# vermashresth/sequential_social_dilemma_games

Measured on AMD Instinct MI355X. Metric: agent-env-steps/sec (random actions), higher is better.
Workload: dtype u8

## Files before the change

sequential_social_dilemma_games_amd/csrc/ssd_internal.hpp:

```cpp
#pragma once
#include <stdint.h>
#include <stddef.h>
#include <stdlib.h>

namespace ssd {

inline int knob_int(const char *name, int dflt) { const char *v = getenv(name); return v ? atoi(v) : dflt; }
#define SSD_KNOB(name, dflt) ::ssd::knob_int(name, dflt)
#ifdef SSD_TESTHOOKS
#define SSD_HOOK(name, dflt) ::ssd::knob_int(name, dflt)
#else
#define SSD_HOOK(name, dflt) (dflt)
#endif

constexpr int kWave = 64;
constexpr int kMaxEnvsPerBlock = 16;
constexpr int kMaxAgents = 64;
constexpr int kMaxCells = 4096;
constexpr int kMaxBeamLen = 21;

constexpr int kListRegsHarvest = 3, kListRegsCleanup = 8;

enum Mode : int32_t {
    kModeStep = 0, kModeReset = 1, kModeObserve = 2,
    kModeRollout = 3,
    kModeStepAuto = 4,
    kModeStepPair = 5
};

enum Stream : uint32_t {
    kSpawnPoint = 1, kSpawnRot = 2, kMove = 3, kApple = 4, kWasteCoin = 5, kWasteOrder = 6, kAction = 7
};

struct Params {
    int32_t E, N, H, W;
    int32_t e_begin;
    int32_t WP, S;
    int32_t A0, A1;
    int32_t view_len, V, beam_len;
    int32_t mode, rotate, keep_beams, num_actions_random;
    int32_t obs_wt;
    int32_t obs_nt;
    int32_t obs_f32;
    int32_t n_steps, reset_every, step0, ring, E_total;
    int32_t horizon;
    uint32_t v_magic16;
    uint32_t seed_lo, seed_hi, env_base;
    int32_t n_spawn, n_thr, n_apple, n_waste;
    int32_t n_waste_reset;
    uint8_t *world;
    uint8_t *beam;
    uint32_t *agents;
    uint4 *hdr;
    uint32_t *status;
    const uint8_t *reset_world;
    const uint32_t *spawn_cells;
    const uint32_t *apple_cells;
    const uint32_t *waste_cells;
    const uint32_t *lut;
    const float *f32lut;
    const uint32_t *view_tab;
    const uint64_t *thr_ca;
    const uint64_t *thr_cw;
    uint32_t thr_h32[4];
    uint32_t thr_h_always;
    const int32_t *actions;
    const uint8_t *order;
    const uint8_t *mask;
    int32_t *actions_out;
    uint8_t *obs;
    int32_t *rew;
    uint8_t *done;
    uint32_t dbg_skip;
    unsigned long long *stamps;
    int32_t action_ring;
    uint32_t coherent;
    int32_t snap_mode, blocks_a;
    uint8_t *world_out;
    uint32_t *agents_out;
    uint32_t *beam_list;
    const uint32_t *beam_list_in;
    uint8_t *snap;
    const uint8_t *snap_in;
    uint8_t *obs_b;
};

constexpr int kMaxRun = 4;
struct PassRec {
    uint8_t *world; uint32_t *agents;
    uint32_t *beam_list; uint8_t *snap;
    int32_t *rew; uint8_t *done;
    const int32_t *actions;
};
struct MidIn { const uint8_t *world; const uint32_t *agents; const uint32_t *beam_list; const uint8_t *snap; };
struct PairParams {
    PassRec pass[kMaxRun];
    int32_t n_pass, n_render;
    MidIn mid_in[kMaxRun - 1];
    uint8_t *obs_b0[kMaxRun - 1];
};

struct KernArgs {
    uint4 *hdr; uint32_t *agents; uint8_t *world;
    int32_t E, e_begin, epb, n_apple;
    const uint32_t *apple_cells; const uint32_t *lut;
    Params p;
};
static_assert(sizeof(KernArgs) == 56 + sizeof(Params), "kernarg layout");
struct PairKernArgs { KernArgs k; PairParams q; };
static_assert(sizeof(PairKernArgs) == sizeof(KernArgs) + sizeof(PairParams), "kernarg layout");

struct Launch {
    const void *fn = nullptr;
    uint32_t grid_x = 0, block_x = 0, lds = 0;
    KernArgs args;
    PairParams pair{};
    size_t args_bytes() const { return args.p.mode == kModeStepPair ? sizeof(PairKernArgs) : sizeof(KernArgs); }
};
static_assert(offsetof(Launch, pair) == offsetof(Launch, args) + sizeof(KernArgs), "Launch::args + Launch::pair == PairKernArgs");

struct AgentOrder { uint8_t sorted[kMaxAgents]; uint8_t rank[kMaxAgents]; };
void launch_agent_action_obs(const int32_t *actions, const uint8_t *done_mask, long long *other_actions, long long *visible,
                             const AgentOrder &order, int E, int N, void *stream);

size_t lds_bytes(const Params &p, int envs_per_block, bool f32);
int envs_per_block(const Params &p, bool f32);
int fast_profile(const Params &p, int game);
int pair_profile(const Params &p, int game);
bool select(const Params &p, int game, Launch *out, const PairParams *pair = nullptr);
void launch(const Launch &L, void *stream);
void launch(const Params &p, int game, void *stream);
const void *flag_kernel_fn();
const void *wait_kernel_fn();
void launch_flag_kernel(unsigned long long *counter, void *stream);
struct WaitArgs { const unsigned long long *counter; unsigned long long target; const uint32_t *abort; unsigned long long timeout_ticks; uint32_t *status; uint32_t *timed_out; };
void launch_wait_counter_kernel(const unsigned long long *counter, unsigned long long target, const uint32_t *abort,
                                unsigned long long timeout_ticks, uint32_t *status, uint32_t *timed_out, void *stream);
#ifdef SSD_STAMPS
void launch_clock_kernel(unsigned long long *out, int iters, void *stream);
#endif
void launch_signal_kernel(long long *signal_value, void *stream);
void launch_render_full(const Params &p, int e0, int count, uint8_t *rgb_dev, void *stream);

}
```

sequential_social_dilemma_games_amd/csrc/ssd_kernels.hip:

```cpp
#include <hip/hip_runtime.h>

#include "ssd_internal.hpp"
#include <type_traits>

#define SSD_OBS_STRIDE 675

namespace ssd {

constexpr uint32_t kStBadAction = 1u << 0;
constexpr uint32_t kStNoSpawn = 1u << 1;
constexpr uint32_t kStMoveLookup = 1u << 2;
constexpr uint32_t kStWaitTimeout = 1u << 3;

__device__ __forceinline__ uint32_t mix32(uint32_t x) {
    x ^= x >> 17; x *= 0xED5AD4BBu;
    x ^= x >> 11; x *= 0xAC4C1B51u;
    x ^= x >> 15; x *= 0x31848BABu;
    x ^= x >> 14;
    return x;
}
__device__ __forceinline__ uint32_t env_key(uint32_t seed_lo, uint32_t seed_hi, uint32_t env, uint32_t episode) {
    uint32_t h = 0x243F6A88u;
    h = mix32(h ^ seed_lo);
    h = mix32(h ^ seed_hi);
    h = mix32(h ^ env);
    h = mix32(h ^ episode);
    return h;
}
__device__ __forceinline__ uint32_t phase_key(uint32_t key, uint32_t t, uint32_t stream) {
    return mix32(mix32(key ^ t) ^ stream);
}
__device__ __forceinline__ uint32_t step_key(uint32_t key, uint32_t t) { return mix32(key ^ t); }
__device__ __forceinline__ uint32_t stream_key(uint32_t skey, uint32_t stream) { return mix32(skey ^ stream); }
__device__ __forceinline__ uint32_t draw(uint32_t pkey, uint32_t index) { return mix32(pkey ^ index); }
__device__ __forceinline__ uint32_t randint(uint32_t u, uint32_t n) { return __umulhi(u, n); }

__device__ __forceinline__ uint32_t rfl(uint32_t v) { return __builtin_amdgcn_readfirstlane(v); }
__device__ __forceinline__ uint32_t rl(uint32_t v, uint32_t lane) { return __builtin_amdgcn_readlane(v, lane); }
__device__ __forceinline__ uint64_t ballot(bool p) { return __builtin_amdgcn_ballot_w64(p); }
__device__ __forceinline__ uint64_t bit(uint32_t i) { return 1ull << i; }
__device__ __forceinline__ uint32_t umin(uint32_t a, uint32_t b) { return a < b ? a : b; }

__device__ __forceinline__ void wave_sync() {
    __builtin_amdgcn_fence(__ATOMIC_RELEASE, "wavefront");
    __builtin_amdgcn_wave_barrier();
    __builtin_amdgcn_fence(__ATOMIC_ACQUIRE, "wavefront");
}

#define SSD_DPP(old, v, ctrl, bc) ((uint32_t)__builtin_amdgcn_update_dpp((int)(old), (int)(v), ctrl, 0xF, 0xF, bc))
__device__ __forceinline__ uint32_t wave_min_u32(uint32_t v) {
    v = umin(v, SSD_DPP(0xFFFFFFFFu, v, 0x111, false));
    v = umin(v, SSD_DPP(0xFFFFFFFFu, v, 0x112, false));
    v = umin(v, SSD_DPP(0xFFFFFFFFu, v, 0x114, false));
    v = umin(v, SSD_DPP(0xFFFFFFFFu, v, 0x118, false));
    return umin(umin(rl(v, 15), rl(v, 31)), umin(rl(v, 47), rl(v, 63)));
}
__device__ __forceinline__ bool wave_argmin_pair(bool has, uint32_t hi, uint32_t lo, uint32_t &out_hi, uint32_t &out_lo) {
    if (!ballot(has)) return false;
    const uint32_t mh = wave_min_u32(has ? hi : 0xFFFFFFFFu);
    const uint32_t ml = wave_min_u32((has && hi == mh) ? lo : 0xFFFFFFFFu);
    out_hi = mh; out_lo = ml;
    return true;
}

__device__ __forceinline__ uint8_t agent_glyph(uint32_t i) {
    uint32_t d = i % 10u;
    return d == 9u ? (uint8_t)'1' : (uint8_t)('1' + d);
}

__device__ __forceinline__ uint32_t turn(int act, uint32_t o) {
    const uint32_t cw = (2u << 0) | (3u << 2) | (1u << 4) | (0u << 6);
    const uint32_t ccw = (3u << 0) | (2u << 2) | (0u << 4) | (1u << 6);
    return ((act == 5 ? cw : ccw) >> (2u * o)) & 3u;
}

__device__ __forceinline__ void unit_vec(int code, int &dr, int &dc) {
    dr = code == 0 ? -1 : (code == 1 ? 1 : 0);
    dc = code == 2 ? -1 : (code == 3 ? 1 : 0);
}

typedef __amdgpu_buffer_rsrc_t rsrc_t;
constexpr int kAuxSc1 = 16, kAuxNt = 2, kAuxSc1Nt = 18;
__device__ __forceinline__ rsrc_t make_rsrc(const void *base, uint32_t bytes) {
    const uint64_t a = reinterpret_cast<uint64_t>(base);
    const uint32_t lo = __builtin_amdgcn_readfirstlane((uint32_t)a), hi = __builtin_amdgcn_readfirstlane((uint32_t)(a >> 32));
    return __builtin_amdgcn_make_buffer_rsrc(reinterpret_cast<void *>(((uint64_t)hi << 32) | lo), 0, (int)bytes, 0x00020000);
}
typedef uint32_t u32x3_t __attribute__((ext_vector_type(3)));
typedef float f32x4_t __attribute__((ext_vector_type(4)));
typedef uint32_t u32x4_t __attribute__((ext_vector_type(4)));
__device__ __forceinline__ void store12_wt(rsrc_t r, uint32_t soff, uint32_t off, u32x3_t d, int wt) {
    if (wt == 1) __builtin_amdgcn_raw_buffer_store_b96(d, r, (int)off, (int)soff, kAuxSc1);
    else if (wt == 3) __builtin_amdgcn_raw_buffer_store_b96(d, r, (int)off, (int)soff, kAuxNt);
    else if (wt == 2) __builtin_amdgcn_raw_buffer_store_b96(d, r, (int)off, (int)soff, kAuxSc1Nt);
    else __builtin_amdgcn_raw_buffer_store_b96(d, r, (int)off, (int)soff, 0);
}
__device__ __forceinline__ void store16_wt(rsrc_t r, uint32_t soff, uint32_t off, f32x4_t f, int wt) {
    const u32x4_t d = __builtin_bit_cast(u32x4_t, f);
    if (wt >= 2) __builtin_amdgcn_raw_buffer_store_b128(d, r, (int)off, (int)soff, kAuxSc1Nt);
    else if (wt) __builtin_amdgcn_raw_buffer_store_b128(d, r, (int)off, (int)soff, kAuxSc1);
    else __builtin_amdgcn_raw_buffer_store_b128(d, r, (int)off, (int)soff, 0);
}
__device__ __forceinline__ u32x4_t load16_sc1(rsrc_t r, uint32_t off) { return __builtin_amdgcn_raw_buffer_load_b128(r, (int)off, 0, kAuxSc1); }
__device__ __forceinline__ void store16_sc1(rsrc_t r, uint32_t off, u32x4_t d) { __builtin_amdgcn_raw_buffer_store_b128(d, r, (int)off, 0, kAuxSc1); }

__device__ __forceinline__ uint32_t nonzero_bytes(uint32_t x) {
    uint32_t m = (((x & 0x7F7F7F7Fu) + 0x7F7F7F7Fu) | x) & 0x80808080u;
    return (m >> 7) * 0xFFu;
}
template <int NA, bool TAB = false>
__device__ __forceinline__ void render_views_std(const int lane, const int WP, const uint32_t a_k, const uint32_t a_s0, const uint32_t view_lds,
                                                 const uint32_t *s_lut, uint8_t *out_env, const int wt, const uint4 tab0 = uint4{0, 0, 0, 0},
                                                 const uint4 tab1 = uint4{0, 0, 0, 0}) {
    typedef __attribute__((address_space(3))) const uint8_t lds_u8;
    constexpr int V = 15, VV = 225, kB = 5;
    const int pp_raw = 4 * lane;
    const bool lane_on = pp_raw < VV;
    const int pp0 = pp_raw > VV - 4 ? VV - 4 : pp_raw;
    int L0[4], L1[4];
    if constexpr (TAB) {
        L0[0] = (int)tab0.x; L0[1] = (int)tab0.y; L0[2] = (int)tab0.z; L0[3] = (int)tab0.w;
        L1[0] = (int)tab1.x; L1[1] = (int)tab1.y; L1[2] = (int)tab1.z; L1[3] = (int)tab1.w;
    } else {
#pragma unroll
    for (int q = 0; q < 4; ++q) {
        const int pp = pp0 + q;
        const int i = pp / 15, j = pp - i * V;
        asm("v_mad_u32_u24 %0, %1, %2, %3" : "=v"(L0[q]) : "v"(i), "s"(WP), "v"(j));
        asm("v_mad_u32_u24 %0, %1, %2, %3" : "=v"(L1[q]) : "v"(j), "s"(WP), "v"(V - 1 - i));
    }
    }
    uint32_t off3 = (uint32_t)pp0 * 3u;
    asm volatile("" : "+v"(off3));
    const rsrc_t out_r = make_rsrc(out_env, (uint32_t)NA * SSD_OBS_STRIDE);
    const uint32_t a_s0v = TAB ? a_s0 + view_lds : a_s0;
    for (int ag0 = 0; ag0 < NA; ag0 += kB) {
        uint32_t addr[kB][4], px[kB][4];
#pragma unroll
        for (int u = 0; u < kB; ++u) {
            const uint32_t k = rl(a_k, ag0 + u);
            const uint32_t s0 = TAB ? rl(a_s0v, ag0 + u) : rl(a_s0, ag0 + u) + view_lds;
            const int sgn = k >= 2 ? -1 : 1;
            if (k & 1) {
#pragma unroll
                for (int q = 0; q < 4; ++q) asm volatile("v_mad_i32_i24 %0, %1, %2, %3" : "=v"(addr[u][q]) : "v"(L1[q]), "v"(sgn), "s"(s0));
            } else {
#pragma unroll
                for (int q = 0; q < 4; ++q) asm volatile("v_mad_i32_i24 %0, %1, %2, %3" : "=v"(addr[u][q]) : "v"(L0[q]), "v"(sgn), "s"(s0));
            }
        }
        uint32_t gl[kB][4];
#pragma unroll
        for (int u = 0; u < kB; ++u)
#pragma unroll
            for (int q = 0; q < 4; ++q) gl[u][q] = *(lds_u8 *)(uintptr_t)addr[u][q];
#pragma unroll
        for (int u = 0; u < kB; ++u)
#pragma unroll
            for (int q = 0; q < 4; ++q) px[u][q] = s_lut[gl[u][q]];
        if (lane_on) {
            u32x3_t d[kB];
#pragma unroll
            for (int u = 0; u < kB; ++u) {
                d[u].x = __builtin_amdgcn_perm(px[u][1], px[u][0], 0x04020100u);
                d[u].y = __builtin_amdgcn_perm(px[u][2], px[u][1], 0x05040201u);
                d[u].z = __builtin_amdgcn_perm(px[u][3], px[u][2], 0x06050402u);
            }
            auto stores = [&](auto policy) {
#pragma unroll
                for (int u = 0; u < kB; ++u) store12_wt(out_r, (uint32_t)(ag0 + u) * SSD_OBS_STRIDE, off3, d[u], decltype(policy)::value);
            };
            if constexpr (TAB) {
                if (__builtin_expect(wt != 3, 1)) stores(std::integral_constant<int, 1>{});
                else stores(std::integral_constant<int, 3>{});
            } else {
                if (wt == 1) stores(std::integral_constant<int, 1>{});
                else if (wt == 3) stores(std::integral_constant<int, 3>{});
                else if (wt == 2) stores(std::integral_constant<int, 2>{});
                else stores(std::integral_constant<int, 0>{});
            }
        }
    }
}

#ifdef SSD_STAMPS
#define SSD_STAMP(i)                                                                               \
    do {                                                                                           \
        if (p.stamps && lane == 0 && e < p.E) p.stamps[(size_t)e * 16 + (i)] = __builtin_readcyclecounter(); \
    } while (0)
#define SSD_STAMP_RT(i)                        \
    do {                                                                                           \
        if (p.stamps && lane == 0 && e < p.E) p.stamps[(size_t)e * 16 + (i)] = __builtin_amdgcn_s_memrealtime(); \
    } while (0)
#define SSD_NOTE(i, v)                                                                             \
    do {                                                                                           \
        if (p.stamps && lane == 0 && e < p.E) p.stamps[(size_t)e * 16 + (i)] = (unsigned long long)(v); \
    } while (0)
#define SSD_SKIP(bit) ((p.dbg_skip >> (bit)) & 1u)
#else
#define SSD_NOTE(i, v)
#define SSD_STAMP(i)
#define SSD_STAMP_RT(i)
#define SSD_SKIP(bit) false
#endif

__host__ size_t lds_bytes(const Params &p, int envs_per_block, bool f32) {
    const int layers = p.mode == kModeRollout ? 4 : 3;
    return (size_t)envs_per_block * (128 * 4 + 256 + (f32 ? 128 * 16 : 0) + (size_t)p.A0 + (size_t)p.A1 + layers * (size_t)p.S);
}

static int forced_epb_early() {
    static const int forced = SSD_KNOB("SSD_ENVS_PER_BLOCK", 0);
    return forced;
}
__host__ int envs_per_block(const Params &p, bool f32) {
    const int E = p.E - p.e_begin;
    static const int forced = SSD_KNOB("SSD_ENVS_PER_BLOCK", 0);
    auto pow2floor = [](int x) { int p = 1; while (p * 2 <= x) p *= 2; return p; };
    int fill = pow2floor(E / 256 > 0 ? E / 256 : 1);
    int rounds = pow2floor(65536 / E > 2 ? 65536 / E : 2);
    int epb = fill < rounds ? fill : rounds;
    if (epb > kMaxEnvsPerBlock) epb = kMaxEnvsPerBlock;
    if (forced >= 1 && forced <= kMaxEnvsPerBlock) epb = forced;
    while (epb > 1 && lds_bytes(p, epb, f32) > 64 * 1024) epb /= 2;
    return epb;
}

struct FastMap { int H, W, WP, S, A0, A1, n_apple, n_waste; };
constexpr FastMap kFastMap[2][3] = {
    {{0, 0, 0, 0, 0, 0, 0, 0}, {16, 38, 45, 720, 336, 320, 155, 0}, {25, 38, 45, 1136, 336, 320, 252, 0}},
    {{0, 0, 0, 0, 0, 0, 0, 0}, {25, 18, 25, 640, 192, 176, 103, 119}, {48, 36, 43, 2064, 320, 304, 412, 476}}};

template <int GAME, int NA, int FAST>
constexpr int run_max() { return (GAME == 0 || NA == 5) ? kMaxRun : 2; }

template <int GAME, int MODE, bool F32, int NA, bool STD, int FAST, bool COH = false, bool ACTS = false>
__global__ __launch_bounds__(64 * kMaxEnvsPerBlock) __attribute__((amdgpu_waves_per_eu(MODE == kModeStepPair ? 8 : 0, MODE == kModeStepPair ? 8 : 0)))
void ssd_env_kernel(uint4 *const a_hdr, uint32_t *const a_agents, uint8_t *const a_world,
                                                                        const int a_E, const int a_e_begin, const int a_epb, const int a_n_apple,
                                                                        const uint32_t *const a_apple_cells, const uint32_t *const a_lut,
                                                                        const Params p) {
    typedef const __attribute__((address_space(4))) uint64_t karg_u64;
    [[maybe_unused]] karg_u64 *const qargs = (karg_u64 *)((const __attribute__((address_space(4))) char *)__builtin_amdgcn_kernarg_segment_ptr() + sizeof(KernArgs));
    [[maybe_unused]] auto qptr = [&](size_t at, auto *like) { return reinterpret_cast<decltype(like)>(qargs[at / 8]); };
    [[maybe_unused]] auto load_rec = [&](int k) {
        const size_t at = offsetof(PairParams, pass) + (size_t)k * sizeof(PassRec);
        PassRec r;
        r.world = qptr(at + offsetof(PassRec, world), r.world); r.agents = qptr(at + offsetof(PassRec, agents), r.agents);
        r.beam_list = qptr(at + offsetof(PassRec, beam_list), r.beam_list); r.snap = qptr(at + offsetof(PassRec, snap), r.snap);
        r.rew = qptr(at + offsetof(PassRec, rew), r.rew); r.done = qptr(at + offsetof(PassRec, done), r.done);
        return r;
    };
    uint8_t *const a_obs = p.obs;
    extern __shared__ __align__(16) uint8_t smem[];
#ifdef SSD_STAMPS
    const unsigned long long t_entry = __builtin_amdgcn_s_memrealtime();
#endif
    const int tid = threadIdx.x, lane = tid & 63;
    const int wv = (int)rfl((uint32_t)tid >> 6);
    constexpr FastMap fm = kFastMap[GAME][FAST];
    const int WP = FAST ? fm.WP : p.WP;
    const int S = FAST ? fm.S : p.S;
    const int A0 = FAST ? fm.A0 : p.A0, A1 = FAST ? fm.A1 : p.A1;
    const int N = NA > 0 ? NA : p.N;
    constexpr int kLR = GAME == 1 ? kListRegsCleanup : (FAST == 2 ? 4 : kListRegsHarvest);
    const int n_apple = FAST ? fm.n_apple : a_n_apple, n_waste = FAST ? fm.n_waste : p.n_waste;
    const bool has_order = !FAST && p.order != nullptr, keep_beams = !FAST && p.keep_beams != 0;
    constexpr bool roll = MODE == kModeRollout;
    constexpr bool auto_mode = MODE == kModeStepAuto;
    constexpr bool pair = MODE == kModeStepPair;
    constexpr bool stepping = MODE == kModeStep || auto_mode || pair;
    uint32_t *s_lut = reinterpret_cast<uint32_t *>(smem + (size_t)wv * (512 + 256 + (F32 ? 2048 : 0) + (size_t)A0 + (size_t)A1 +
                                                                            (roll ? 4 : 3) * (size_t)S));
    uint32_t *s_tmp = s_lut + 128;
    float *s_f32 = reinterpret_cast<float *>(s_lut + 192);
    uint8_t *s_world = reinterpret_cast<uint8_t *>(s_lut + 192 + (F32 ? 512 : 0)) + (roll ? 0 : A0);
    uint8_t *s_beam = s_world + S + (roll ? 0 : A1);
    uint8_t *s_occ = s_beam + S;
    uint8_t *s_view = roll ? s_occ + S + A0 : s_world;

    constexpr bool kCoh = COH;
    const int blk = blockIdx.x;
    if constexpr (MODE == kModeStep && COH && STD && NA > 0 && NA % 5 == 0 && !F32 && FAST != 0) {
        if ((p.snap_mode & 2) && blk >= p.blocks_a) {
            const int eb = a_e_begin + (blk - p.blocks_a) * a_epb + wv;
#ifdef SSD_STAMPS
#define SSD_BSTAMP(i, v) do { if (p.stamps && lane == 0 && eb < a_E) p.stamps[((size_t)p.E_total + eb) * 16 + (i)] = (v); } while (0)
#else
#define SSD_BSTAMP(i, v)
#endif
            SSD_BSTAMP(10, __builtin_amdgcn_s_memrealtime());
            SSD_BSTAMP(0, __builtin_readcyclecounter());
            if (eb < a_E) {
                typedef __attribute__((address_space(3))) const uint8_t lds_u8;
                const uint32_t lut_a = a_lut[lane], lut_b = a_lut[lane + 64];
                const uint4 vt0 = reinterpret_cast<const uint4 *>(p.view_tab)[2 * lane], vt1 = reinterpret_cast<const uint4 *>(p.view_tab)[2 * lane + 1];
                constexpr int kGridLoads = (fm.S + 1023) / 1024;
                u32x4_t g0[kGridLoads];
                const rsrc_t grid_r = make_rsrc(a_world + (size_t)eb * S, (uint32_t)S);
#pragma unroll
                for (int j = 0; j < kGridLoads; ++j) g0[j] = load16_sc1(grid_r, (uint32_t)(lane * 16 + j * 1024));
                uint32_t areg = 0;
                if (lane < N) areg = __hip_atomic_load(a_agents + (size_t)eb * N + lane, __ATOMIC_RELAXED, __HIP_MEMORY_SCOPE_AGENT);
                const uint32_t entry = __hip_atomic_load(p.beam_list_in + (size_t)eb * 64 + lane, __ATOMIC_RELAXED, __HIP_MEMORY_SCOPE_AGENT);
                {
                    const uint4 z = make_uint4(0x30303030u, 0x30303030u, 0x30303030u, 0x30303030u);
                    const int n0 = A0 >> 4, n1 = A1 >> 4;
                    for (int i = lane; i < n0 + n1; i += 64)
                        *reinterpret_cast<uint4 *>(i < n0 ? s_world - A0 + i * 16 : s_world + S + (i - n0) * 16) = z;
                }
                s_lut[lane] = lut_a; s_lut[lane + 64] = lut_b;
                const uint32_t flags = rfl(areg) >> 20;
                const bool snapshot = (flags & 2u) != 0, marks = (flags & 1u) != 0;
                uint32_t entry2 = 0;
                constexpr bool kTwoLists = GAME == 1 && NA > 5;
                if (kTwoLists && (flags & 4u)) entry2 = __hip_atomic_load(p.beam_list_in + ((size_t)p.E_total + eb) * 64 + lane, __ATOMIC_RELAXED, __HIP_MEMORY_SCOPE_AGENT);
                if (snapshot) {
                    const rsrc_t snap_r = make_rsrc(p.snap_in + (size_t)eb * S, (uint32_t)S);
#pragma unroll
                    for (int j = 0; j < kGridLoads; ++j) g0[j] = load16_sc1(snap_r, (uint32_t)(lane * 16 + j * 1024));
                }
#pragma unroll
                for (int j = 0; j < kGridLoads; ++j) {
                    if (lane * 16 + j * 1024 < S) *reinterpret_cast<uint4 *>(s_world + lane * 16 + j * 1024) = make_uint4(g0[j].x, g0[j].y, g0[j].z, g0[j].w);
                }
                wave_sync();
                const uint32_t cellb = areg & 0xFFFFu, orientb = (areg >> 16) & 3u;
                if (!snapshot) {
                    if (lane < N && (areg & (1u << 19))) s_world[cellb] = agent_glyph((uint32_t)lane);
                    wave_sync();
                    if (marks) {
                        if (entry) s_world[entry & 0xFFFFu] = (uint8_t)(entry >> 16);
                        wave_sync();
                        if constexpr (kTwoLists) {
                            if (entry2) s_world[entry2 & 0xFFFFu] = (uint8_t)(entry2 >> 16);
                            wave_sync();
                        }
                    }
                }
                SSD_BSTAMP(1, __builtin_readcyclecounter());
                const uint32_t kq = (0x8Du >> (2u * orientb)) & 3u;
                const uint32_t s0 = (uint32_t)((int)cellb - 7 * (WP + 1) + (kq >= 2 ? 14 * (WP + 1) : 0));
                render_views_std<NA, true>(lane, WP, kq, s0, (uint32_t)(uintptr_t)(lds_u8 *)s_world, s_lut, p.obs_b + (size_t)eb * N * SSD_OBS_STRIDE, p.obs_wt,
                                           vt0, vt1);
                SSD_BSTAMP(2, __builtin_readcyclecounter());
                asm volatile("s_waitcnt vmcnt(0)" ::: "memory");
                SSD_BSTAMP(3, __builtin_readcyclecounter());
            }
            SSD_BSTAMP(11, __builtin_amdgcn_s_memrealtime());
            return;
        }
    }
    if constexpr (pair && COH && STD && NA > 0 && NA % 5 == 0 && !F32 && FAST != 0) {
        if ((p.snap_mode & 2) && blk >= p.blocks_a) {
            const int eb = a_e_begin + (blk - p.blocks_a) * a_epb + wv;
            if (eb < a_E) {
                typedef __attribute__((address_space(3))) const uint8_t lds_u8;
                constexpr int kGridLoads = (fm.S + 1023) / 1024;
                constexpr bool kTwoLists = GAME == 1 && NA > 5;
                constexpr int kRun = run_max<GAME, NA, FAST>();
                static_assert(kMaxRun == 4 && (kRun == 2 || kRun == 4), "two rounds of two layers");
                const int n_render = (int)(uint32_t)(qargs[offsetof(PairParams, n_pass) / 8] >> 32);
                auto used = [&](int t) { return t >= kMaxRun - n_render; };
                struct MidPtr { const uint8_t *world; const uint32_t *agents; const uint32_t *list; const uint8_t *snap; uint8_t *obs; };
                auto mid_ptr = [&](int t) {
                    const size_t at = offsetof(PairParams, mid_in) + (size_t)t * sizeof(MidIn);
                    MidPtr m;
                    m.world = qptr(at + offsetof(MidIn, world), m.world); m.agents = qptr(at + offsetof(MidIn, agents), m.agents);
                    m.list = qptr(at + offsetof(MidIn, beam_list), m.list); m.snap = qptr(at + offsetof(MidIn, snap), m.snap);
                    m.obs = qptr(offsetof(PairParams, obs_b0) + (size_t)t * sizeof(uint8_t *), m.obs);
                    return m;
                };
                struct StepIn { u32x4_t g[kGridLoads]; uint32_t areg, entry, entry2; };
                auto fetch = [&](const uint8_t *world, const uint32_t *agents, const uint32_t *list) {
                    StepIn s;
                    const rsrc_t grid_r = make_rsrc(world + (size_t)eb * S, (uint32_t)S);
#pragma unroll
                    for (int j = 0; j < kGridLoads; ++j) s.g[j] = load16_sc1(grid_r, (uint32_t)(lane * 16 + j * 1024));
                    s.areg = 0; s.entry2 = 0;
                    if (lane < N) s.areg = __hip_atomic_load(agents + (size_t)eb * N + lane, __ATOMIC_RELAXED, __HIP_MEMORY_SCOPE_AGENT);
                    s.entry = __hip_atomic_load(list + (size_t)eb * 64 + lane, __ATOMIC_RELAXED, __HIP_MEMORY_SCOPE_AGENT);
                    return s;
                };
                auto fetch_rare = [&](StepIn &s, const uint32_t *list, const uint8_t *snap) {
                    const uint32_t flags = rfl(s.areg) >> 20;
                    if (kTwoLists && (flags & 4u)) s.entry2 = __hip_atomic_load(list + ((size_t)p.E_total + eb) * 64 + lane, __ATOMIC_RELAXED, __HIP_MEMORY_SCOPE_AGENT);
                    if (flags & 2u) {
                        const rsrc_t snap_r = make_rsrc(snap + (size_t)eb * S, (uint32_t)S);
#pragma unroll
                        for (int j = 0; j < kGridLoads; ++j) s.g[j] = load16_sc1(snap_r, (uint32_t)(lane * 16 + j * 1024));
                    }
                };
                const uint32_t lut_a = a_lut[lane], lut_b = a_lut[lane + 64];
                const uint4 vt0 = reinterpret_cast<const uint4 *>(p.view_tab)[2 * lane], vt1 = reinterpret_cast<const uint4 *>(p.view_tab)[2 * lane + 1];
                static_assert(fm.S >= fm.A0 + fm.A1, "the renderer's second layer fits the beam and occupancy layers");
                uint8_t *const s_world2 = s_world + S + A1 + A0;
                constexpr int kFirst = kMaxRun - kRun;
                StepIn sm[kMaxRun - 1];
                MidPtr mp[kMaxRun - 1];
                StepIn sb = fetch(a_world, a_agents, p.beam_list_in);
#pragma unroll
                for (int t = kMaxRun - 2; t >= kFirst; --t) {
                    sm[t] = sb; mp[t] = MidPtr{};
                    if (used(t)) { mp[t] = mid_ptr(t); sm[t] = fetch(mp[t].world, mp[t].agents, mp[t].list); }
                }
                {
                    const uint4 z = make_uint4(0x30303030u, 0x30303030u, 0x30303030u, 0x30303030u);
                    const int n0 = A0 >> 4, n1 = A1 >> 4;
                    for (int i = lane; i < n0 + n1; i += 64) {
                        const int at = i < n0 ? i * 16 - A0 : S + (i - n0) * 16;
                        *reinterpret_cast<uint4 *>(s_world + at) = z;
                        if (used(kMaxRun - 2)) *reinterpret_cast<uint4 *>(s_world2 + at) = z;
                    }
                }
                s_lut[lane] = lut_a; s_lut[lane + 64] = lut_b;
                fetch_rare(sb, p.beam_list_in, p.snap_in);
#pragma unroll
                for (int t = kMaxRun - 2; t >= kFirst; --t)
                    if (used(t)) fetch_rare(sm[t], mp[t].list, mp[t].snap);
                auto fill = [&](const StepIn &s, uint8_t *layer) {
                    const uint32_t flags = rfl(s.areg) >> 20;
#pragma unroll
                    for (int j = 0; j < kGridLoads; ++j) {
                        if (lane * 16 + j * 1024 < S) *reinterpret_cast<uint4 *>(layer + lane * 16 + j * 1024) = make_uint4(s.g[j].x, s.g[j].y, s.g[j].z, s.g[j].w);
                    }
                    wave_sync();
                    if (!(flags & 2u)) {
                        if (lane < N && (s.areg & (1u << 19))) layer[s.areg & 0xFFFFu] = agent_glyph((uint32_t)lane);
                        wave_sync();
                        if (flags & 1u) {
                            if (s.entry) layer[s.entry & 0xFFFFu] = (uint8_t)(s.entry >> 16);
                            wave_sync();
                            if constexpr (kTwoLists) {
                                if (s.entry2) layer[s.entry2 & 0xFFFFu] = (uint8_t)(s.entry2 >> 16);
                                wave_sync();
                            }
                        }
                    }
                };
                auto views = [&](const uint32_t areg, const uint8_t *layer, uint8_t *obs_to) {
                    const uint32_t cellb = areg & 0xFFFFu, orientb = (areg >> 16) & 3u;
                    const uint32_t kq = (0x8Du >> (2u * orientb)) & 3u;
                    const uint32_t s0 = (uint32_t)((int)cellb - 7 * (WP + 1) + (kq >= 2 ? 14 * (WP + 1) : 0));
                    render_views_std<NA, true>(lane, WP, kq, s0, (uint32_t)(uintptr_t)(lds_u8 *)layer, s_lut, obs_to + (size_t)eb * N * SSD_OBS_STRIDE, p.obs_wt,
                                               vt0, vt1);
                };
                if constexpr (kRun > 2) {
                    if (used(1)) {
                        fill(sm[1], s_world);
                        if (used(0)) { fill(sm[0], s_world2); views(sm[0].areg, s_world2, mp[0].obs); }
                        views(sm[1].areg, s_world, mp[1].obs);
                        wave_sync();
                    }
                }
                fill(sb, s_world);
                if (used(kMaxRun - 2)) { fill(sm[kMaxRun - 2], s_world2); views(sm[kMaxRun - 2].areg, s_world2, mp[kMaxRun - 2].obs); }
                views(sb.areg, s_world, p.obs_b);
                asm volatile("s_waitcnt vmcnt(0)" ::: "memory");
            }
            return;
        }
    }
    const int e = a_e_begin + blk * a_epb + wv;
    constexpr int mode = pair ? (int)kModeStep : MODE;
    bool active = e < a_E;
    if (active && mode == kModeReset && p.mask) active = p.mask[e] != 0;
    SSD_STAMP_RT(10);
    SSD_NOTE(14, t_entry);
    SSD_STAMP(0);

    if (active) {
        const bool is_agent = lane < N;
        auto cload = [](const uint32_t *ptr) -> uint32_t {
            return kCoh ? __hip_atomic_load(ptr, __ATOMIC_RELAXED, __HIP_MEMORY_SCOPE_AGENT) : *ptr;
        };
        constexpr bool kPre = GAME == 1 && (MODE == kModeStep || pair) && COH && FAST != 0;
        constexpr int kPreUp = pair ? kMaxRun - 1 : 0;
        uint4 hdr;
        [[maybe_unused]] PassRec rec{};
        [[maybe_unused]] int n_pass = 1;
        if (kCoh) {
            const uint32_t hv = cload(reinterpret_cast<const uint32_t *>(a_hdr + e) + (lane & 3));
            if constexpr (pair) {
                rec = load_rec(0);
                n_pass = (int)(uint32_t)qargs[offsetof(PairParams, n_pass) / 8];
                asm volatile("" ::"s"(rec.world), "s"(rec.agents), "s"(rec.beam_list), "s"(rec.snap), "s"(rec.rew), "s"(rec.done), "s"(n_pass));
            }
            if constexpr (kPre) asm volatile("" ::"s"(p.waste_cells), "s"(p.thr_ca), "s"(p.thr_cw), "s"(p.n_thr));
            asm volatile("" ::"s"(p.actions), "s"(p.order), "s"(p.num_actions_random), "s"(p.obs));
            if (GAME == 1) asm volatile("" ::"s"(p.waste_cells), "s"(n_waste), "s"(p.thr_ca), "s"(p.thr_cw), "s"(p.n_thr), "s"(p.rew), "s"(p.done), "s"(p.horizon));
            else asm volatile("" ::"s"(p.thr_h32[0]), "s"(p.thr_h32[1]), "s"(p.thr_h32[2]), "s"(p.thr_h32[3]), "s"(p.thr_h_always));
            hdr = make_uint4(rl(hv, 0), rl(hv, 1), rl(hv, 2), rl(hv, 3));
        } else {
            hdr = a_hdr[e];
        }
        uint32_t areg = 0;
        int act_in = -1;
        int act_next = -1;
        [[maybe_unused]] auto next_actions = [&](int k) {
            return qptr(offsetof(PairParams, pass) + (size_t)k * sizeof(PassRec) + offsetof(PassRec, actions), (const uint32_t *)nullptr);
        };
        uint32_t ord_in = 0xFFu;
        uint32_t eN32 = rfl((uint32_t)e * (uint32_t)N);
        asm volatile("" : "+s"(eN32));
        size_t eN = eN32;
        if (mode != kModeReset && is_agent) areg = cload(a_agents + eN + lane);
        const uint8_t *gsrc = mode == kModeReset ? p.reset_world : a_world + (size_t)e * S;
        constexpr int kGridLoads = FAST ? (fm.S + 1023) / 1024 : 1;
        uint4 w0[kGridLoads], b0 = make_uint4(0, 0, 0, 0);
        const rsrc_t grid_r = make_rsrc(gsrc, (uint32_t)S);
        auto issue_grid = [&]() {
#pragma unroll
            for (int j = 0; j < kGridLoads; ++j) {
                w0[j] = make_uint4(0, 0, 0, 0);
                const int off = lane * 16 + j * 1024;
                if constexpr (kCoh) {
                    const u32x4_t v = load16_sc1(grid_r, (uint32_t)off);
                    w0[j] = make_uint4(v.x, v.y, v.z, v.w);
                } else if (off < S) {
                    w0[j] = *reinterpret_cast<const uint4 *>(gsrc + off);
                }
            }
        };
        issue_grid();
        if (lane * 16 < S && mode == kModeObserve && keep_beams) b0 = *reinterpret_cast<const uint4 *>(p.beam + (size_t)e * S + lane * 16);
        uint32_t lut_a = 0, lut_b = 0;
        if (a_obs) { lut_a = a_lut[lane]; lut_b = a_lut[lane + 64]; }
        const bool obs_f32 = F32 && a_obs;
        float4 flut = make_float4(0.f, 0.f, 0.f, 0.f), flut_b = flut;
        if (obs_f32) { flut = reinterpret_cast<const float4 *>(p.f32lut)[lane]; flut_b = reinterpret_cast<const float4 *>(p.f32lut)[lane + 64]; }
        uint32_t alist[kLR], wlist[kLR];
#pragma unroll
        for (int j = 0; j < kLR; ++j) {
            const int idx = lane + 64 * j;
            alist[j] = 0u;
            if (kLR <= 3 || 64 * j < n_apple) alist[j] = (mode != kModeObserve && idx < n_apple) ? a_apple_cells[idx] : 0u;
        }
        asm volatile("" ::"s"(p.actions), "s"(p.order), "s"(p.num_actions_random), "s"(p.obs));
        if (GAME == 1) asm volatile("" ::"s"(p.waste_cells), "s"(n_waste), "s"(p.thr_ca), "s"(p.thr_cw), "s"(p.n_thr), "s"(p.rew), "s"(p.done), "s"(p.horizon));
        else asm volatile("" ::"s"(p.thr_h32[0]), "s"(p.thr_h32[1]), "s"(p.thr_h32[2]), "s"(p.thr_h32[3]), "s"(p.thr_h_always));
        if (stepping && is_agent) {
            if (p.num_actions_random <= 0) act_in = (int)cload(reinterpret_cast<const uint32_t *>(p.actions) + eN + lane);
            if (has_order) ord_in = p.order[eN + lane];
            if constexpr (pair)
                if (p.num_actions_random <= 0 && n_pass > 1) act_next = (int)cload(next_actions(1) + eN + lane);
        }
#pragma unroll
        for (int j = 0; j < kLR; ++j) {
            const int idx = lane + 64 * j;
            wlist[j] = 0u;
            if (GAME == 1 && 64 * j < n_waste) wlist[j] = (mode != kModeObserve && idx < n_waste) ? p.waste_cells[idx] : 0u;
        }
        uint64_t thr_pa = 0, thr_pw = 0;
        if constexpr (kPre) {
            int ti = (int)((rfl(hdr.w) >> 16) & 0x7FFFu) + kPreUp - lane;
            ti = ti < 0 ? 0 : ti;
            ti = ti < p.n_thr ? ti : p.n_thr - 1;
            thr_pa = p.thr_ca[ti]; thr_pw = p.thr_cw[ti];
        }
        uint32_t key = rfl(hdr.x), t = rfl(hdr.y), episode = rfl(hdr.z);
        if (a_obs) { s_lut[lane] = lut_a; s_lut[lane + 64] = lut_b; }
        if (obs_f32) { reinterpret_cast<float4 *>(s_f32)[lane] = flut; reinterpret_cast<float4 *>(s_f32)[lane + 64] = flut_b; }
        uint32_t status = 0u;
        uint32_t cell = areg & 0xFFFFu, orient = mode == kModeReset ? 2u : (areg >> 16) & 3u;
        int rew = 0;
#pragma unroll
        for (int j = 0; j < kGridLoads; ++j)
            if (lane * 16 + j * 1024 < S) {
                *reinterpret_cast<uint4 *>(s_world + lane * 16 + j * 1024) = w0[j];
                *reinterpret_cast<uint4 *>(s_beam + lane * 16 + j * 1024) = j == 0 ? b0 : make_uint4(0, 0, 0, 0);
                *reinterpret_cast<uint4 *>(s_occ + lane * 16 + j * 1024) = make_uint4(0, 0, 0, 0);
            }
        if (a_obs) {
            const uint4 z = make_uint4(0x30303030u, 0x30303030u, 0x30303030u, 0x30303030u);
            const int n0 = A0 >> 4, n1 = A1 >> 4;
            for (int i = lane; i < n0 + n1; i += 64)
                *reinterpret_cast<uint4 *>(i < n0 ? s_view - A0 + i * 16 : s_view + S + (i - n0) * 16) = z;
        }
        for (int i = lane * 16 + 1024 * kGridLoads; i < S; i += 1024) {
            uint4 bv = make_uint4(0, 0, 0, 0);
            if (mode == kModeObserve && keep_beams) bv = *reinterpret_cast<const uint4 *>(p.beam + (size_t)e * S + i);
            if constexpr (kCoh) {
                const u32x4_t wv = load16_sc1(grid_r, (uint32_t)i);
                *reinterpret_cast<uint4 *>(s_world + i) = make_uint4(wv.x, wv.y, wv.z, wv.w);
            } else {
                *reinterpret_cast<uint4 *>(s_world + i) = *reinterpret_cast<const uint4 *>(gsrc + i);
            }
            *reinterpret_cast<uint4 *>(s_beam + i) = bv;
            *reinterpret_cast<uint4 *>(s_occ + i) = make_uint4(0, 0, 0, 0);
        }
        wave_sync();

        uint32_t waste_last = 0;
        uint32_t waste_cur = GAME == 1 ? (rfl(hdr.w) >> 16) & 0x7FFFu : 0u;
        [[maybe_unused]] const uint32_t waste0 = waste_cur;
        bool share = (rfl(hdr.w) >> 31) != 0u;
        [[maybe_unused]] int pass_k = 0;
        auto write_state = [&](const uint32_t render_flags, const uint32_t top_bit = 0u) {
            uint8_t *gw = a_world + (size_t)e * S;
            if constexpr (kCoh) {
                uint32_t *ga = a_agents;
                if constexpr (pair) { gw = rec.world + (size_t)e * S; ga = rec.agents; }
                else if (p.world_out) { gw = p.world_out + (size_t)e * S; ga = p.agents_out; }
                auto cstore = [](uint32_t *ptr, uint32_t v) { __hip_atomic_store(ptr, v, __ATOMIC_RELAXED, __HIP_MEMORY_SCOPE_AGENT); };
                const rsrc_t out_r = make_rsrc(gw, (uint32_t)S);
                if constexpr (FAST != 0) {
                    uint4 v4[kGridLoads];
#pragma unroll
                    for (int j = 0; j < kGridLoads; ++j) {
                        const int off = lane * 16 + j * 1024;
                        v4[j] = *reinterpret_cast<const uint4 *>(s_world + (off < S ? off : 0));
                    }
#pragma unroll
                    for (int j = 0; j < kGridLoads; ++j) {
                        const int off = lane * 16 + j * 1024;
                        const u32x4_t v = {v4[j].x, v4[j].y, v4[j].z, v4[j].w};
                        store16_sc1(out_r, (uint32_t)off, v);
                    }
                } else
                for (int i = lane * 16; i < S; i += 64 * 16) {
                    const uint4 v4 = *reinterpret_cast<const uint4 *>(s_world + i);
                    const u32x4_t v = {v4.x, v4.y, v4.z, v4.w};
                    store16_sc1(out_r, (uint32_t)i, v);
                }
                if (is_agent) cstore(ga + eN + lane, cell | (orient << 16) | top_bit | (lane == 0 ? render_flags : 0u));
                if (!pair || pass_k + 1 >= n_pass)
                {
                    uint32_t hw = waste_last | (waste_cur << 16) | (share ? 1u << 31 : 0u);
                    asm("v_writelane_b32 %0, %1, 0" : "+v"(hw) : "s"(key));
                    asm("v_writelane_b32 %0, %1, 1" : "+v"(hw) : "s"(t));
                    asm("v_writelane_b32 %0, %1, 2" : "+v"(hw) : "s"(episode));
                    if (lane < 4) cstore(reinterpret_cast<uint32_t *>(a_hdr + e) + lane, hw);
                }
                if (status && lane == 0) atomicOr(p.status, status);
                return;
            }
            for (int i = lane * 16; i < S; i += 64 * 16) {
                *reinterpret_cast<uint4 *>(gw + i) = *reinterpret_cast<const uint4 *>(s_world + i);
                if (keep_beams)
                    *reinterpret_cast<uint4 *>(p.beam + (size_t)e * S + i) = *reinterpret_cast<const uint4 *>(s_beam + i);
            }
            if (is_agent) a_agents[eN + lane] = cell | (orient << 16);
            if (lane == 0) a_hdr[e] = make_uint4(key, t, episode, waste_last | (waste_cur << 16) | (share ? 1u << 31 : 0u));
            if (status && lane == 0) atomicOr(p.status, status);
        };
        int k_step = 0;
        int to_reset = -1;
        uint32_t slot = 0;
        if (roll) {
            if (p.reset_every > 0) to_reset = (p.reset_every - p.step0 % p.reset_every) % p.reset_every;
            slot = (uint32_t)(p.step0 % p.ring);
        }
        bool in_reset = roll && to_reset == 0;
        constexpr bool roll_acts = roll && ACTS;
        uint32_t aslot = 0;
        uint32_t ord_next = 0xFFu;
        auto fetch_action = [&]() {
            if (is_agent) {
                const size_t at = ((size_t)aslot * (size_t)p.E_total + (size_t)e) * N + lane;
                act_next = p.actions[at];
                if (has_order) ord_next = p.order[at];
            }
            aslot = aslot + 1 == (uint32_t)p.action_ring ? 0u : aslot + 1;
        };
        if constexpr (roll_acts) { aslot = (uint32_t)(p.step0 % p.action_ring); fetch_action(); }
        const size_t en_stride = (size_t)p.E_total * N;
        size_t slot_en_run = roll ? (size_t)slot * en_stride : 0;
        for (;;) {
            if constexpr (pair) { asm volatile("" : "+s"(eN32)); eN = eN32; }
            const bool is_reset = (roll || auto_mode) ? in_reset : (mode == kModeReset);
            const bool is_step = (roll || auto_mode) ? !in_reset : (mode == kModeStep);
            const size_t slot_en = roll ? slot_en_run : 0;
            if (roll || (auto_mode && in_reset) || (pair && pass_k > 0)) {
                __builtin_amdgcn_s_setprio(0);
                rew = 0;
                if constexpr (pair) { rec = load_rec(pass_k); act_in = act_next; }
                for (int i = lane * 16; i < S; i += 64 * 16) {
                    if (is_reset) *reinterpret_cast<uint4 *>(s_world + i) = *reinterpret_cast<const uint4 *>(p.reset_world + i);
                    *reinterpret_cast<uint4 *>(s_beam + i) = make_uint4(0, 0, 0, 0);
                    *reinterpret_cast<uint4 *>(s_occ + i) = make_uint4(0, 0, 0, 0);
                }
                wave_sync();
                if constexpr (pair) asm volatile("" ::"s"(rec.world), "s"(rec.agents), "s"(rec.beam_list), "s"(rec.snap), "s"(rec.rew), "s"(rec.done));
            }
            if constexpr (pair && run_max<GAME, NA, FAST>() > 2) {
                if (pass_k > 0 && p.num_actions_random <= 0 && pass_k + 1 < n_pass && is_agent)
                    act_next = (int)cload(next_actions(pass_k + 1) + eN + lane);
            }
            uint32_t cleaned = 0;
            if (is_reset) {
                episode += 1; t = 0;
                waste_cur = (uint32_t)p.n_waste_reset;
                key = env_key(p.seed_lo, p.seed_hi, p.env_base + (uint32_t)e, episode);
                const uint32_t pk_pt = phase_key(key, 0, kSpawnPoint), pk_rot = phase_key(key, 0, kSpawnRot);
                for (int i = 0; i < N; ++i) {
                    bool has = false;
                    uint32_t bh = 0, bl = 0;
                    for (int s = lane; s < p.n_spawn; s += 64) {
                        const uint32_t ce = p.spawn_cells[s], c = ce & 0xFFFFu;
                        if (s_occ[c] == 0) {
                            const uint32_t kh = ~draw(pk_pt, ((uint32_t)i << 16) | (ce >> 16)), kl = ~c;
                            if (!has || kh < bh || (kh == bh && kl < bl)) { bh = kh; bl = kl; has = true; }
                        }
                    }
                    uint32_t oh, ol, chosen;
                    if (wave_argmin_pair(has, bh, bl, oh, ol)) chosen = ~ol;
                    else { status |= kStNoSpawn; chosen = p.n_spawn ? (p.spawn_cells[0] & 0xFFFFu) : (uint32_t)(WP + 1); }
                    if (lane == i) { cell = chosen; orient = randint(draw(pk_rot, (uint32_t)i), 4); }
                    s_occ[chosen] = agent_glyph((uint32_t)i);
                    wave_sync();
                }
                share = (status & kStNoSpawn) != 0u;
            }

            SSD_STAMP(1);
            int act = -1;
            uint32_t ordv = (uint32_t)lane;
            int nord = N;
            bool all_apart = false;
            if (is_step) t += 1;
            const uint32_t skey = step_key(key, t);
            uint32_t vkeys = 0;
            if constexpr (roll) vkeys = stream_key(skey, (uint32_t)lane);
            auto stream_key_of = [&](uint32_t stream) -> uint32_t {
                if constexpr (roll) return rl(vkeys, stream);
                else return stream_key(skey, stream);
            };
            if (is_step) {
                constexpr int kNumActions = GAME == 0 ? 8 : 9;
                if constexpr (roll_acts) {
                    act = act_next; ord_in = ord_next;
                    fetch_action();
                    const bool bad = is_agent && (act < -1 || act >= kNumActions);
                    if (ballot(bad)) { status |= kStBadAction; if (bad) act = -1; }
                } else if (roll || p.num_actions_random > 0) {
                    const uint32_t pk = stream_key_of(kAction);
                    if (is_agent) {
                        act = (int)randint(draw(pk, (uint32_t)lane), (uint32_t)p.num_actions_random);
                        if (!roll && p.actions_out) {
                            int32_t *actions_out = p.actions_out;
                            if constexpr (pair && GAME == 1) asm volatile("" : "+s"(actions_out));
                            actions_out[eN + lane] = act;
                        }
                    }
                } else {
                    act = act_in;
                    const bool bad = is_agent && (act < -1 || act >= kNumActions);
                    if (ballot(bad)) { status |= kStBadAction; if (bad) act = -1; }
                }
                if (has_order) {
                    ordv = ord_in;
                    if (ordv != 0xFFu && ordv >= (uint32_t)N) { ordv = 0xFFu; status |= kStBadAction; }
                    const uint64_t endm = ballot(ordv == 0xFFu);
                    nord = endm ? __builtin_ctzll(endm) : 64;
                    uint64_t acting = 0;
                    for (int k = 0; k < nord; ++k) acting |= bit(rl(ordv, k));
                    if (!((acting >> lane) & 1)) act = -1;
                }

                const bool mover = !SSD_SKIP(0) && is_agent && act >= 0 && act <= 4;
                if (is_agent && (act == 5 || act == 6)) orient = turn(act, orient);
                uint32_t tcell = cell;
                {
                    constexpr uint32_t kMoveIdx8 = (0u << 0) | (16u << 5) | (24u << 10) | (8u << 15);
                    constexpr uint32_t kTurns8 = (8u << 0) | (24u << 5) | (0u << 10) | (16u << 15);
                    const uint32_t sum = __builtin_amdgcn_ubfe(kMoveIdx8, (uint32_t)act * 5u, 5u) + __builtin_amdgcn_ubfe(kTurns8, orient * 5u, 5u);
                    int step;
                    if (FAST) {
                        const uint32_t off4 = ((uint32_t)(-WP) & 0xFFu) | (1u << 8) | ((uint32_t)WP << 16) | (0xFFu << 24);
                        step = __builtin_amdgcn_sbfe(off4, sum, 8u);
                    } else {
                        step = __builtin_amdgcn_sbfe(0x000100FFu, sum, 8u) * WP + __builtin_amdgcn_sbfe(0xFF000100u, sum, 8u);
                    }
                    const uint32_t cand = (uint32_t)((int)cell + ((mover & (act < 4)) ? step : 0));
                    tcell = (mover & (s_world[cand] != '@')) ? cand : cell;
                }
                uint32_t mvcell = tcell;
                const uint64_t M = ballot(mover);
                const uint64_t agents_m = N >= 64 ? ~0ull : bit((uint32_t)N) - 1;
                uint64_t clashm = 0, dupm = 0;
                bool exact_loop = !roll || (NA == 0 && N > 16);
                if (!exact_loop) {
                    const uint32_t cellx = is_agent ? cell : 0xFFFFFFFEu, tcellm = mover ? tcell : 0xFFFFFFFFu;
                    uint32_t nearest = 0xFFFFFFFFu;
                    constexpr int kN = NA > 0 ? NA : 16;
#define SSD_LOOK(k)                                                                                                            \
    if constexpr ((k) < kN || 16 - (k) < kN) {                                                                                  \
        const uint32_t pc = SSD_DPP(0, cellx, 0x120 + (k), false), pt = SSD_DPP(0, tcellm, 0x120 + (k), false);                \
        nearest = umin(nearest, umin(tcell ^ pc, tcell ^ pt));                                                                  \
    }
                    SSD_LOOK(1) SSD_LOOK(2) SSD_LOOK(3) SSD_LOOK(4) SSD_LOOK(5) SSD_LOOK(6) SSD_LOOK(7) SSD_LOOK(8)
                    SSD_LOOK(9) SSD_LOOK(10) SSD_LOOK(11) SSD_LOOK(12) SSD_LOOK(13) SSD_LOOK(14) SSD_LOOK(15)
#undef SSD_LOOK
                    clashm = ballot(is_agent & (nearest == 0u));
                    exact_loop = (clashm & M) != 0;
                }
                constexpr bool kFold = !roll && NA > 0;
                int occ_fold = -1;
                if (exact_loop) {
                    const uint32_t tcellm = mover ? tcell : 0xFFFFFFFFu;
                    clashm = 0;
                    if constexpr (kFold) {
                        for (int j = 0; j < N; ++j) {
// ... 473 lines not shown
                            const uint32_t c = ce & 0xFFFFu;
                            const bool cand = valid & (s_world[c] != 'H') & ((uint64_t)draw(pk_coin, ce >> 16) < thr_w);
                            const uint32_t kh = draw(pk_ord, ce >> 16);
                            const bool better = cand & (!has | (kh < bh) | ((kh == bh) & (c < bl)));
                            bh = better ? kh : bh; bl = better ? c : bl; has = has | cand;
                        };
                        const int w_iters = (n_waste + 63) >> 6;
#pragma unroll
                        for (int j = 0; j < kLR; ++j)
                            if (64 * j < n_waste) waste(wlist[j], lane + 64 * j < n_waste);
                        for (int j = kLR; j < w_iters; ++j) {
                            const int idx = lane + 64 * j;
                            waste(idx < n_waste ? p.waste_cells[idx] : 0u, idx < n_waste);
                        }
                        uint32_t oh, ol;
                        if (wave_argmin_pair(has, bh, bl, oh, ol)) waste_cell = ol;
                    }
                }
                }
                wave_sync();
#pragma unroll
                for (int j = 0; j < kLR; ++j)
                    if ((kLR <= 3 || 64 * j < n_apple) && ((spawn_bits >> j) & 1)) s_world[alist[j] & 0xFFFFu] = 'A';
                for (int j = kLR; j < a_iters; ++j)
                    if ((spawn_bits >> j) & 1) s_world[a_apple_cells[lane + 64 * j] & 0xFFFFu] = 'A';
                if (waste_cell != 0xFFFFFFFFu) s_world[waste_cell] = 'H';
                if (GAME == 1) waste_cur = waste_count + (waste_cell != 0xFFFFFFFFu ? 1u : 0u);
                wave_sync();

                SSD_STAMP(5);
                waste_last = waste_count;
                if constexpr (pair) asm volatile("" : "+v"(act_next));
                if (!roll) {
                    uint32_t render_flags = 0;
                    if constexpr (stepping && COH) {
                        if ((pair || (p.snap_mode & 1)) && is_step) {
                            render_flags = (!keep_beams && beams_in_regs) ? (ballot(b_cov | (kTwoPasses & b_cov0)) ? 1u << 20 : 0u) : 1u << 21;
                            if constexpr (kTwoPasses)
                                if (!keep_beams && beams_in_regs && ballot(b_cov0)) render_flags |= 1u << 22;
                        }
                    }
                    write_state(render_flags, __builtin_amdgcn_inverse_ballot_w64(highest) ? 1u << 19 : 0u);
                }
                if (is_agent && is_step) {
                    const uint8_t dn = (p.horizon > 0 && t >= (uint32_t)p.horizon) ? 1 : 0;
                    if constexpr (pair) {
                        int32_t *const rew_to = rec.rew;
                        uint8_t *const done_to = rec.done;
                        if (rew_to) __hip_atomic_store(rew_to + eN + lane, rew, __ATOMIC_RELAXED, __HIP_MEMORY_SCOPE_AGENT);
                        if (done_to) __hip_atomic_store(done_to + eN + lane, dn, __ATOMIC_RELAXED, __HIP_MEMORY_SCOPE_AGENT);
                    } else if constexpr (COH) {
                        if (p.rew) __hip_atomic_store(p.rew + slot_en + eN + lane, rew, __ATOMIC_RELAXED, __HIP_MEMORY_SCOPE_AGENT);
                        if (p.done) __hip_atomic_store(p.done + slot_en + eN + lane, dn, __ATOMIC_RELAXED, __HIP_MEMORY_SCOPE_AGENT);
                    } else {
                        if (p.rew) p.rew[slot_en + eN + lane] = rew;
                        if (p.done) p.done[slot_en + eN + lane] = dn;
                    }
                }
                wave_sync();
            }

            SSD_STAMP(6);
            const bool patch = is_step && !keep_beams && beams_in_regs;
            bool leave_overlay = false;
            if constexpr (stepping && COH) {
                if ((pair || (p.snap_mode & 1)) && is_step) {
                    leave_overlay = patch;
                    const bool two = kTwoPasses && ballot(b_cov0) != 0;
                    const uint32_t ent = b_cov ? ((uint32_t)b_idx | (b_chr << 16)) : 0u, ent0 = b_cov0 ? ((uint32_t)b_idx0 | (b_chr0 << 16)) : 0u;
                    uint32_t *list_to = p.beam_list;
                    if constexpr (pair) list_to = rec.beam_list;
                    if (patch && ballot(b_cov | b_cov0))
                        __hip_atomic_store(list_to + (size_t)e * 64 + lane, two ? ent0 : ent, __ATOMIC_RELAXED, __HIP_MEMORY_SCOPE_AGENT);
                    if (patch && two)
                        __hip_atomic_store(list_to + ((size_t)p.E_total + e) * 64 + lane, ent, __ATOMIC_RELAXED, __HIP_MEMORY_SCOPE_AGENT);
                }
            }
            if (leave_overlay) {
            } else if (patch && !SSD_SKIP(5)) {
                if (roll)
                    for (int i = lane * 16; i < S; i += 64 * 16)
                        *reinterpret_cast<uint4 *>(s_view + i) = *reinterpret_cast<const uint4 *>(s_world + i);
                if (__builtin_amdgcn_inverse_ballot_w64(highest)) s_view[cell] = agent_glyph((uint32_t)lane);
                if (kTwoPasses && b_cov0) s_view[b_idx0] = (uint8_t)b_chr0;
                if (b_cov) s_view[b_idx] = (uint8_t)b_chr;
            } else if ((!roll || is_step) && !SSD_SKIP(5))
            for (int i = lane * 4; i < S; i += 64 * 4) {
                const uint32_t w = *reinterpret_cast<const uint32_t *>(s_world + i);
                const uint32_t o = *reinterpret_cast<const uint32_t *>(s_occ + i);
                const uint32_t b = *reinterpret_cast<const uint32_t *>(s_beam + i);
                const uint32_t mo = nonzero_bytes(o), mb = nonzero_bytes(b);
                uint32_t v = (w & ~mo) | (o & mo);
                v = (v & ~mb) | (b & mb);
                *reinterpret_cast<uint32_t *>((pair ? s_beam : s_view) + i) = v;
            }
            wave_sync();
            if constexpr (stepping && COH) {
                if ((pair || (p.snap_mode & 1)) && is_step && !patch) {
                    uint8_t *snap_to = p.snap;
                    if constexpr (pair) snap_to = rec.snap;
                    const rsrc_t snap_r = make_rsrc(snap_to + (size_t)e * S, (uint32_t)S);
                    for (int i = lane * 16; i < S; i += 64 * 16) {
                        const uint4 v4 = *reinterpret_cast<const uint4 *>((pair ? s_beam : s_view) + i);
                        store16_sc1(snap_r, (uint32_t)i, u32x4_t{v4.x, v4.y, v4.z, v4.w});
                    }
                }
            }
            SSD_STAMP(7);
            SSD_STAMP(8);

            if (!pair && a_obs && (!roll || is_step)) {
                typedef __attribute__((address_space(3))) const uint8_t lds_u8;
                const int V = STD ? 15 : p.V, v = STD ? 7 : p.view_len, VV = V * V;
                uint8_t *out_env = a_obs + (slot_en + (size_t)(SSD_SKIP(4) ? (e & 63) : e) * N) * VV * 3;
                if constexpr (roll) {
                    const uint64_t ob = reinterpret_cast<uint64_t>(out_env);
                    out_env = reinterpret_cast<uint8_t *>(((uint64_t)rfl((uint32_t)(ob >> 32)) << 32) | (uint64_t)rfl((uint32_t)ob));
                }
                uint32_t a_s0 = 0, a_k = 0;
                if (is_agent) {
                    a_k = (is_step || (!roll && !auto_mode && p.rotate)) ? ((0x8Du >> (2u * orient)) & 3u) : 0u;
                    a_s0 = (uint32_t)((int)cell - v * (WP + 1) + (a_k >= 2 ? (V - 1) * (WP + 1) : 0));
                }
                const uint32_t world_lds = (uint32_t)(uintptr_t)(lds_u8 *)s_view;
                if (F32 && a_obs && VV * 3 >= 4) {
                    const int nf = VV * 3, n_st = (nf + 255) >> 8;
                    float *base_env = reinterpret_cast<float *>(a_obs) + (slot_en + (size_t)e * N) * (size_t)nf;
                    const rsrc_t f32_r = make_rsrc(base_env, (uint32_t)(N * nf * 4));
                    for (int k4 = 0; k4 < n_st; ++k4) {
                        const int f_raw = k4 * 256 + 4 * lane;
                        const bool on = f_raw < nf;
                        const int f0 = f_raw > nf - 4 ? nf - 4 : f_raw;
                        const int c0 = (int)(((uint32_t)f0 * 21846u) >> 16);
                        const int r = f0 - 3 * c0;
                        int M0[2], M1[2];
#pragma unroll
                        for (int q = 0; q < 2; ++q) {
                            const int pp = c0 + q;
                            const int i = STD ? pp / 15 : (int)(((uint32_t)pp * p.v_magic16) >> 16), j = pp - i * V;
                            M0[q] = i * WP + j;
                            M1[q] = j * WP + (V - 1 - i);
                        }
                        const bool r0 = r == 0, r1 = r == 1;
                        for (int ag = 0; ag < N; ++ag) {
                            const uint32_t k = rl(a_k, ag);
                            const int s0 = (int)(rl(a_s0, ag) + world_lds);
                            const int sgn = k >= 2 ? -1 : 1;
                            float4 t[2];
#pragma unroll
                            for (int q = 0; q < 2; ++q) {
                                const uint32_t ad = (uint32_t)(s0 + sgn * ((k & 1) ? M1[q] : M0[q]));
                                t[q] = reinterpret_cast<const float4 *>(s_f32)[*(lds_u8 *)(uintptr_t)ad];
                            }
                            f32x4_t o;
                            o.x = r0 ? t[0].x : r1 ? t[0].y : t[0].z;
                            o.y = r0 ? t[0].y : r1 ? t[0].z : t[1].x;
                            o.z = r0 ? t[0].z : r1 ? t[1].x : t[1].y;
                            o.w = r0 ? t[1].x : r1 ? t[1].y : t[1].z;
                            if (on) store16_wt(f32_r, (uint32_t)(ag * nf * 4), (uint32_t)f0 * 4u, o, p.obs_wt);
                        }
                    }
                } else if constexpr (STD && NA > 0 && NA % 5 == 0 && !F32) {
                    render_views_std<NA>(lane, WP, a_k, a_s0, world_lds, s_lut, out_env, p.obs_wt);
                } else {
                const rsrc_t gen_r = obs_f32 ? make_rsrc(reinterpret_cast<float *>(a_obs) + (slot_en + (size_t)e * N) * VV * 3, (uint32_t)(N * VV * 12))
                                             : make_rsrc(out_env, (uint32_t)(N * VV * 3));
                for (int base = 0; base < VV; base += 256) {
                    const int pp_raw = base + 4 * lane;
                    const bool lane_on = pp_raw < VV;
                    const int pp0 = (VV >= 4 && pp_raw > VV - 4) ? VV - 4 : pp_raw;
                    int L0[4], L1[4];
#pragma unroll
                    for (int q = 0; q < 4; ++q) {
                        const int pp = pp0 + q;
                        const int i = STD ? pp / 15 : (int)(((uint32_t)pp * p.v_magic16) >> 16), j = pp - i * V;
                        asm("v_mad_u32_u24 %0, %1, %2, %3" : "=v"(L0[q]) : "v"(i), "s"(WP), "v"(j));
                        asm("v_mad_u32_u24 %0, %1, %2, %3" : "=v"(L1[q]) : "v"(j), "s"(WP), "v"(V - 1 - i));
                    }
                    uint32_t off3 = (uint32_t)pp0 * 3u;
                    asm volatile("" : "+v"(off3));
                    const int ncell = lane_on ? VV - pp0 : 0;
                    for (int ag = 0; ag < N; ++ag) {
                        const uint32_t k = rl(a_k, ag);
                        const uint32_t s0 = rl(a_s0, ag) + world_lds;
                        const int sgn = k >= 2 ? -1 : 1;
                        uint32_t addr[4], px[4];
                        if (k & 1) {
#pragma unroll
                            for (int q = 0; q < 4; ++q) asm volatile("v_mad_i32_i24 %0, %1, %2, %3" : "=v"(addr[q]) : "v"(L1[q]), "v"(sgn), "s"(s0));
                        } else {
#pragma unroll
                            for (int q = 0; q < 4; ++q) asm volatile("v_mad_i32_i24 %0, %1, %2, %3" : "=v"(addr[q]) : "v"(L0[q]), "v"(sgn), "s"(s0));
                        }
                        uint32_t gl[4];
#pragma unroll
                        for (int q = 0; q < 4; ++q) gl[q] = *(lds_u8 *)(uintptr_t)addr[q];
                        const size_t cell0 = (size_t)ag * VV + pp0;
                        if (obs_f32) {
                            float *dstf = reinterpret_cast<float *>(a_obs) + ((slot_en + (size_t)e * N) * VV + cell0) * 3;
                            float f[12];
#pragma unroll
                            for (int q = 0; q < 4; ++q) {
                                const float4 v = reinterpret_cast<const float4 *>(s_f32)[gl[q]];
                                f[q * 3 + 0] = v.x; f[q * 3 + 1] = v.y; f[q * 3 + 2] = v.z;
                            }
                            if (VV >= 4) {
                                if (lane_on) {
#pragma unroll
                                    for (int k4 = 0; k4 < 3; ++k4) {
                                        f32x4_t v4 = {f[4 * k4], f[4 * k4 + 1], f[4 * k4 + 2], f[4 * k4 + 3]};
                                        store16_wt(gen_r, (uint32_t)(ag * VV * 12), (uint32_t)pp0 * 12u + 16u * k4, v4, p.obs_wt);
                                    }
                                }
                            } else {
#pragma unroll
                                for (int q = 0; q < 3; ++q)
                                    if (q < ncell) { dstf[q * 3] = f[q * 3]; dstf[q * 3 + 1] = f[q * 3 + 1]; dstf[q * 3 + 2] = f[q * 3 + 2]; }
                            }
                            continue;
                        }
#pragma unroll
                        for (int q = 0; q < 4; ++q) px[q] = s_lut[gl[q]];
                        uint8_t *dst = out_env + (size_t)ag * VV * 3 + off3;
                        if (VV >= 4) {
                            if (lane_on) {
                                u32x3_t d;
                                d.x = __builtin_amdgcn_perm(px[1], px[0], 0x04020100u);
                                d.y = __builtin_amdgcn_perm(px[2], px[1], 0x05040201u);
                                d.z = __builtin_amdgcn_perm(px[3], px[2], 0x06050402u);
                                store12_wt(gen_r, (uint32_t)(ag * VV * 3), off3, d, p.obs_wt);
                            }
                        } else {
#pragma unroll
                            for (int q = 0; q < 3; ++q)
                                if (q < ncell) {
                                    dst[q * 3 + 0] = (uint8_t)px[q];
                                    dst[q * 3 + 1] = (uint8_t)(px[q] >> 8);
                                    dst[q * 3 + 2] = (uint8_t)(px[q] >> 16);
                                }
                        }
                    }
                }
                }
            }
            if (auto_mode) {
                if (is_step && p.horizon > 0 && t >= (uint32_t)p.horizon) { in_reset = true; continue; }
                break;
            }
            if constexpr (pair) {
                if (++pass_k >= n_pass) break;
                continue;
            }
            if (!roll) break;
            if (in_reset) { in_reset = false; continue; }
            if (++k_step >= p.n_steps) break;
            slot = slot + 1 == (uint32_t)p.ring ? 0u : slot + 1;
            slot_en_run = slot == 0u ? 0 : slot_en_run + en_stride;
            if (to_reset >= 0) to_reset = (to_reset == 0 ? p.reset_every : to_reset) - 1;
            in_reset = to_reset == 0;
        }
        if (roll) write_state(0u);
        if constexpr (COH) asm volatile("s_waitcnt vmcnt(0)" ::: "memory");
    }
    SSD_STAMP(9);
    SSD_STAMP_RT(11);
}

__global__ void ssd_render_full_kernel(const Params p, int e0, uint8_t *rgb) {
    const int hw = p.H * p.W;
    const int e = e0 + (int)blockIdx.y;
    uint8_t *out = rgb + (size_t)blockIdx.y * hw * 3;
    for (int c = blockIdx.x * blockDim.x + threadIdx.x; c < hw; c += gridDim.x * blockDim.x) {
        const int g = (c / p.W) * p.WP + c % p.W;
        uint32_t ch = p.world[(size_t)e * p.S + g];
        for (int i = 0; i < p.N; ++i)
            if ((p.agents[(size_t)e * p.N + i] & 0xFFFFu) == (uint32_t)g) ch = agent_glyph((uint32_t)i);
        if (p.keep_beams) { const uint32_t b = p.beam[(size_t)e * p.S + g]; if (b) ch = b; }
        const uint32_t px = p.lut[ch & 127u];
        out[c * 3 + 0] = (uint8_t)px; out[c * 3 + 1] = (uint8_t)(px >> 8); out[c * 3 + 2] = (uint8_t)(px >> 16);
    }
}

template <int GAME, int MODE, bool F32, int NA, bool STD, int FAST, bool COH = false, bool ACTS = false>
static const void *kernel_fn() {
    return reinterpret_cast<const void *>(&ssd_env_kernel<GAME, MODE, F32, NA, STD, FAST, COH, ACTS>);
}

template <int GAME, bool F32, int NA, bool STD, int FAST>
static const void *select_step(const Params &p) {
    if (p.mode == kModeRollout) {
        if constexpr (!F32) {
            if (p.action_ring > 0) return kernel_fn<GAME, kModeRollout, false, NA, STD, FAST, false, true>();
            return kernel_fn<GAME, kModeRollout, false, NA, STD, FAST>();
        }
        return nullptr;
    } else if (p.mode == kModeStepAuto) {
        if constexpr (!F32) return kernel_fn<GAME, kModeStepAuto, false, NA, STD, FAST>();
        return nullptr;
    } else if (p.mode == kModeStepPair) {
        if constexpr ((GAME == 0 || FAST == 1) && !F32 && FAST != 0 && STD && NA > 0) {
            if (p.coherent) return kernel_fn<GAME, kModeStepPair, false, NA, STD, FAST, true>();
        }
        return nullptr;
    } else {
        if constexpr (!F32 && FAST != 0) {
            if (p.coherent) return kernel_fn<GAME, kModeStep, false, NA, STD, FAST, true>();
        }
        return kernel_fn<GAME, kModeStep, F32, NA, STD, FAST>();
    }
}

int fast_profile(const Params &p, int game) {
    const bool std_view = p.view_len == 7 && p.beam_len == 5;
    int fast = 0;
    for (int f = 1; f <= 2; ++f) {
        const FastMap &m = kFastMap[game][f];
        if (std_view && !p.order && !p.keep_beams && p.H == m.H && p.W == m.W && p.WP == m.WP && p.S == m.S && p.A0 == m.A0 &&
            p.A1 == m.A1 && p.n_apple == m.n_apple && (game == 0 || p.n_waste == m.n_waste))
            fast = f;
    }
    if (p.N != 5 && p.N != 10) fast = 0;
    if (fast == 2 && ((p.N == 5 && game != 0) || (p.N == 10 && game != 1))) fast = 0;
    return fast;
}

int pair_profile(const Params &p, int game) {
    const int fast = fast_profile(p, game);
    if (p.obs_f32 || fast <= 0 || !(game == 0 || fast == 1)) return 1;
    if (game == 0) return p.N == 5 ? (fast == 1 ? run_max<0, 5, 1>() : run_max<0, 5, 2>()) : run_max<0, 10, 1>();
    return p.N == 5 ? run_max<1, 5, 1>() : run_max<1, 10, 1>();
}

template <int GAME, bool F32>
static const void *select_game(const Params &p) {
    if (p.mode == kModeStep || p.mode == kModeRollout || p.mode == kModeStepAuto || p.mode == kModeStepPair) {
        const bool std_view = p.view_len == 7 && p.beam_len == 5;
        const int fast = fast_profile(p, GAME);
        if (std_view && p.N == 5) {
            if (fast == 1) return select_step<GAME, F32, 5, true, 1>(p);
            if (GAME == 0 && fast == 2) { if constexpr (GAME == 0) return select_step<GAME, F32, 5, true, 2>(p); }
            return select_step<GAME, F32, 5, true, 0>(p);
        } else if (std_view && p.N == 10) {
            if (fast == 1) return select_step<GAME, F32, 10, true, 1>(p);
            if (GAME == 1 && fast == 2) { if constexpr (GAME == 1) return select_step<GAME, F32, 10, true, 2>(p); }
            return select_step<GAME, F32, 10, true, 0>(p);
        } else if (std_view) return select_step<GAME, F32, 0, true, 0>(p);
        return select_step<GAME, F32, 0, false, 0>(p);
    } else if (p.mode == kModeReset) {
        if constexpr (!F32) { if (p.coherent) return kernel_fn<GAME, kModeReset, false, 0, false, 0, true>(); }
        return kernel_fn<GAME, kModeReset, F32, 0, false, 0>();
    }
    return kernel_fn<GAME, kModeObserve, F32, 0, false, 0>();
}

bool select(const Params &p_in, int game, Launch *out, const PairParams *pair) {
    Params p = p_in;
    static const int forced_wt = SSD_HOOK("SSD_OBS_WT", -1);
    p.obs_wt = forced_wt >= 0 ? forced_wt : ((p.E - p.e_begin) <= (p.obs_f32 ? 4096 : 16384) ? 1 : 0);
    if (p.coherent) p.obs_wt = 1;
    static const int forced_nt = SSD_HOOK("SSD_OBS_NT", -1);
    if (forced_nt >= 0) p.obs_nt = forced_nt;
    if (p.obs_nt) p.obs_wt = p.obs_f32 ? (p.obs_wt == 1 ? 2 : p.obs_wt) : 3;
    static const int forced_epb = SSD_KNOB("SSD_ENVS_PER_BLOCK", 0);
    const bool f32 = p.obs && p.obs_f32;
    int epb = envs_per_block(p, f32);
    static const int split_epb = SSD_HOOK("SSD_SPLIT_EPB", 4);
    if (p.snap_mode && forced_epb_early() <= 0 && epb > split_epb && split_epb >= 1) epb = split_epb;
    if (p.coherent == 2 && epb > 1 && forced_epb <= 0) epb /= 2;
    out->grid_x = (uint32_t)((p.E - p.e_begin + epb - 1) / epb);
    if (p.snap_mode & 2) {
        p.blocks_a = (p.snap_mode & 4) ? 0 : (int32_t)out->grid_x;
        out->grid_x = (uint32_t)p.blocks_a + out->grid_x;
    }
    out->block_x = (uint32_t)(64 * epb);
    out->lds = (uint32_t)lds_bytes(p, epb, f32);
    if (game == 0) out->fn = f32 ? select_game<0, true>(p) : select_game<0, false>(p);
    else out->fn = f32 ? select_game<1, true>(p) : select_game<1, false>(p);
    KernArgs &k = out->args;
    k.hdr = p.hdr; k.agents = p.agents; k.world = p.world; k.E = p.E; k.e_begin = p.e_begin; k.epb = epb; k.n_apple = p.n_apple;
    k.apple_cells = p.apple_cells; k.lut = p.lut; k.p = p;
    if (p.mode == kModeStepPair) { if (!pair) return false; out->pair = *pair; }
    return out->fn != nullptr;
}

void launch(const Launch &L, void *stream) {
    if (L.args.p.mode == kModeStepPair) return;
    KernArgs &k = const_cast<KernArgs &>(L.args);
    void *args[] = {&k.hdr, &k.agents, &k.world, &k.E, &k.e_begin, &k.epb, &k.n_apple, &k.apple_cells, &k.lut, &k.p};
    (void)hipLaunchKernel(L.fn, dim3(L.grid_x), dim3(L.block_x), args, L.lds, static_cast<hipStream_t>(stream));
}

void launch(const Params &p, int game, void *stream) {
    Launch L;
    if (select(p, game, &L)) launch(L, stream);
}

__global__ void ssd_flag_kernel(unsigned long long *counter) {
    if (threadIdx.x == 0) __hip_atomic_fetch_add(counter, 1ull, __ATOMIC_RELEASE, __HIP_MEMORY_SCOPE_AGENT);
}
__global__ void ssd_wait_counter_kernel(const unsigned long long *counter, unsigned long long target, const volatile uint32_t *abort,
                                        unsigned long long timeout_ticks, uint32_t *status, uint32_t *timed_out) {
    if (threadIdx.x != 0) return;
    uint32_t spins = 0;
    const unsigned long long t0 = __builtin_amdgcn_s_memrealtime();
    while (__hip_atomic_load(counter, __ATOMIC_RELAXED, __HIP_MEMORY_SCOPE_AGENT) < target) {
        __builtin_amdgcn_s_sleep(16);
        if ((++spins & 1023u) == 0) {
            if (abort && *abort) break;
            if (timeout_ticks && __builtin_amdgcn_s_memrealtime() - t0 > timeout_ticks) {
                if (status) atomicOr(status, kStWaitTimeout);
                if (timed_out) __hip_atomic_store(timed_out, 1u, __ATOMIC_RELAXED, __HIP_MEMORY_SCOPE_SYSTEM);
                break;
            }
        }
    }
    __builtin_amdgcn_fence(__ATOMIC_ACQUIRE, "agent");
}
__global__ void ssd_signal_kernel(long long *signal_value) {
    if (threadIdx.x == 0) __hip_atomic_store(signal_value, 0ll, __ATOMIC_RELEASE, __HIP_MEMORY_SCOPE_SYSTEM);
}
#ifdef SSD_STAMPS
__global__ void ssd_clock_kernel(unsigned long long *out, int iters) {
    if (threadIdx.x != 0) return;
    for (int i = 0; i < iters; ++i) {
        __hip_atomic_store(out, (unsigned long long)__builtin_amdgcn_s_memrealtime(), __ATOMIC_RELAXED, __HIP_MEMORY_SCOPE_SYSTEM);
        __builtin_amdgcn_s_sleep(4);
    }
}
void launch_clock_kernel(unsigned long long *out, int iters, void *stream) {
    hipLaunchKernelGGL(ssd_clock_kernel, dim3(1), dim3(64), 0, static_cast<hipStream_t>(stream), out, iters);
}
#endif
const void *flag_kernel_fn() { return reinterpret_cast<const void *>(&ssd_flag_kernel); }
const void *wait_kernel_fn() { return reinterpret_cast<const void *>(&ssd_wait_counter_kernel); }
void launch_flag_kernel(unsigned long long *counter, void *stream) {
    hipLaunchKernelGGL(ssd_flag_kernel, dim3(1), dim3(64), 0, static_cast<hipStream_t>(stream), counter);
}
void launch_wait_counter_kernel(const unsigned long long *counter, unsigned long long target, const uint32_t *abort,
                                unsigned long long timeout_ticks, uint32_t *status, uint32_t *timed_out, void *stream) {
    hipLaunchKernelGGL(ssd_wait_counter_kernel, dim3(1), dim3(64), 0, static_cast<hipStream_t>(stream), counter, target, abort,
                       timeout_ticks, status, timed_out);
}
void launch_signal_kernel(long long *signal_value, void *stream) {
    hipLaunchKernelGGL(ssd_signal_kernel, dim3(1), dim3(64), 0, static_cast<hipStream_t>(stream), signal_value);
}

__global__ void ssd_agent_action_obs_kernel(const int32_t *actions, const uint8_t *done_mask, long long *other_actions, long long *visible,
                                            AgentOrder order, int E, int N) {
    const long long total = (long long)E * N * (N - 1);
    for (long long idx = (long long)blockIdx.x * blockDim.x + threadIdx.x; idx < total; idx += (long long)gridDim.x * blockDim.x) {
        const int j = (int)(idx % (N - 1));
        const long long ei = idx / (N - 1);
        const int i = (int)(ei % N);
        const long long e = ei / N;
        if (other_actions) {
            long long v = 0;
            if (actions && !(done_mask && done_mask[ei])) v = actions[e * N + order.sorted[j + (j >= (int)order.rank[i] ? 1 : 0)]];
            other_actions[idx] = v;
        }
        if (visible) visible[idx] = 1;
    }
}
void launch_agent_action_obs(const int32_t *actions, const uint8_t *done_mask, long long *other_actions, long long *visible,
                             const AgentOrder &order, int E, int N, void *stream) {
    const long long total = (long long)E * N * (N - 1);
    if (total <= 0) return;
    const int blocks = (int)((total + 255) / 256 < 4096 ? (total + 255) / 256 : 4096);
    hipLaunchKernelGGL(ssd_agent_action_obs_kernel, dim3(blocks), dim3(256), 0, static_cast<hipStream_t>(stream), actions, done_mask,
                       other_actions, visible, order, E, N);
}

void launch_render_full(const Params &p, int e0, int count, uint8_t *rgb_dev, void *stream) {
    const int hw = p.H * p.W;
    hipLaunchKernelGGL(ssd_render_full_kernel, dim3((hw + 255) / 256, count), dim3(256), 0, static_cast<hipStream_t>(stream), p, e0, rgb_dev);
}

}
```

sequential_social_dilemma_games_amd/csrc/ssd_rollout.hip:

```cpp
#include <hip/hip_runtime.h>

#include <cstring>
#include <atomic>
#include <chrono>
#include <condition_variable>
#include <memory>
#include <mutex>
#include <string>
#include <thread>
#include <vector>

#include "../../include/ssd.h"
#include "ssd_internal.hpp"
#include "ssd_env.hpp"
#include "ssd_aql.hpp"
#include "ssd_rollout_plan.hpp"

using ssd::Params;
namespace plan = ssd::plan;

struct ChainJob {
    int chain = 0, e_begin = 0, e_end = 0;
    int32_t num_actions = 0, n_steps = 0, reset_every = 0, step0 = 0, ring = 1;
    const int32_t *actions = nullptr; int32_t action_ring = 0;
    const uint8_t *order = nullptr;
    uint8_t *obs = nullptr; int32_t *rew = nullptr; uint8_t *done = nullptr;
    uint32_t flags = 0;
    hipStream_t s = nullptr;
};
struct ChainWorker {
    std::thread th;
    std::mutex mu;
    std::condition_variable cv;
    std::atomic<int> state{0};
    ChainJob job;
    int rc = 0;
};

struct AqlState : plan::SplitBuffers {
    bool tried = false, ok = false;
    ssd::aql::Queue *q[8] = {};
    int nq = 0;
    static constexpr int kForks = 16;
    uint64_t fork_sig[kForks] = {};
    uint64_t fork_used[kForks][8] = {};
    int fork_next = 0;
    unsigned long long *fork_counter = nullptr;
    unsigned long long forks = 0;
    uint8_t *fork_kernarg = nullptr;
    static constexpr size_t kForkBlock = 256;
    ssd::aql::Kernel wait_kernel{};
    unsigned long long *join_counter = nullptr;
    unsigned long long joins = 0;
    void *flag_kernarg = nullptr;
    uint32_t *timed_out_host = nullptr, *timed_out_dev = nullptr;
    using Key = plan::Key;
    struct Geo { ssd::aql::Kernel k; uint32_t grid_x = 0, block_x = 0, lds = 0; };
    struct Set {
        bool valid = false;
        Key key;
        uint8_t *dev = nullptr;
        size_t cap = 0;
        Geo geo[8][plan::kKinds];
        plan::KindTable kinds;
        uint64_t last_use[8] = {};
        uint64_t stamp = 0;
    };
    static constexpr int kSets = 4;
    static constexpr size_t kBlock = 896;
    Set sets[kSets];
    uint64_t clock = 0;
};
static_assert(AqlState::kBlock >= sizeof(ssd::PairKernArgs), "an argument block holds the largest kernarg segment");

void RolloutDelete::operator()(ChainWorker *w) const { delete w; }
void RolloutDelete::operator()(AqlState *a) const { delete a; }

struct ChainCursor : plan::ChainRings {
    Params p;
    hipStream_t s;
    int32_t reset_every, step0, ring;
};
using plan::cursor_actions;
static ChainCursor chain_cursor(const ssd_env *env, const ChainJob &j) {
    ChainCursor c;
    const bool f32 = (j.flags & SSD_OBS_F32) != 0;
    c.p = env->p;
    c.p.obs_f32 = f32 ? 1 : 0;
    c.p.e_begin = j.e_begin; c.p.E = j.e_end;
    c.s = j.s; c.obs = j.obs; c.rew = j.rew; c.done = j.done;
    c.actions = j.actions; c.order = j.order; c.action_ring = j.action_ring;
    c.en = (size_t)env->E * env->N; c.ob = obs_bytes(env, f32);
    c.p.obs_nt = plan::ring_past_cache(j.obs, j.ring, c.ob) ? 1 : 0;
    c.num_actions = j.num_actions; c.reset_every = j.reset_every; c.step0 = j.step0; c.ring = j.ring;
    return c;
}
static inline void chain_launch_step(const ssd_env *env, ChainCursor &c, int k) {
    Params &p = c.p;
    const size_t slot = (size_t)((c.step0 + k) % c.ring);
    p.obs = c.obs ? c.obs + slot * c.ob : nullptr;
    if (c.reset_every > 0 && (c.step0 + k) % c.reset_every == 0) {
        p.mode = ssd::kModeReset; p.rotate = 0; p.num_actions_random = 0; p.actions = nullptr; p.order = nullptr; p.rew = nullptr; p.done = nullptr;
        ssd::launch(p, env->game, c.s);
    }
    p.mode = ssd::kModeStep; p.rotate = 1;
    cursor_actions(c, p, (size_t)(c.step0 + k));
    p.rew = c.rew ? c.rew + slot * c.en : nullptr; p.done = c.done ? c.done + slot * c.en : nullptr;
    ssd::launch(p, env->game, c.s);
}

static int rollout_chain(ssd_env *env, const ChainJob &j) {
    const int32_t n_steps = j.n_steps;
    hipStream_t s = j.s;
    if (j.flags & SSD_ROLLOUT_FUSED) {
        if (n_steps == 0) return SSD_OK;
        Params p = env->p;
        p.obs_f32 = 0;
        p.e_begin = j.e_begin; p.E = j.e_end;
        p.mode = ssd::kModeRollout; p.rotate = 1;
        p.num_actions_random = j.actions ? 0 : j.num_actions;
        p.actions = j.actions; p.order = j.actions ? j.order : nullptr; p.action_ring = j.actions ? j.action_ring : 0;
        p.n_steps = n_steps; p.reset_every = j.reset_every; p.step0 = j.step0; p.ring = j.ring;
        p.obs = j.obs; p.rew = j.rew; p.done = j.done;
        p.obs_nt = plan::ring_past_cache(j.obs, j.ring, obs_bytes(env, false)) ? 1 : 0;
        ssd::launch(p, env->game, s);
        return hipGetLastError() == hipSuccess ? SSD_OK : SSD_E_DEVICE;
    }
    ChainCursor c = chain_cursor(env, j);
    for (int k = 0; k < n_steps; ++k) chain_launch_step(env, c, k);
    return hipGetLastError() == hipSuccess ? SSD_OK : SSD_E_DEVICE;
}

static void chain_worker_main(ssd_env *env, ChainWorker *w) {
    const bool on_device = hipSetDevice(env->device) == hipSuccess;
    static const int spin_us = SSD_HOOK("SSD_WORKER_SPIN_US", 200);
    for (;;) {
        int st = w->state.load(std::memory_order_acquire);
        if (st != 1 && st != 3) {
            const auto t0 = std::chrono::steady_clock::now();
            for (;;) {
                st = w->state.load(std::memory_order_acquire);
                if (st == 1 || st == 3) break;
                __builtin_ia32_pause();
                if (std::chrono::steady_clock::now() - t0 > std::chrono::microseconds(spin_us)) break;
            }
            if (st != 1 && st != 3) {
                std::unique_lock<std::mutex> lk(w->mu);
                w->cv.wait(lk, [&] { const int v = w->state.load(std::memory_order_acquire); return v == 1 || v == 3; });
                st = w->state.load(std::memory_order_acquire);
            }
        }
        if (st == 3) return;
        w->rc = on_device ? rollout_chain(env, w->job) : SSD_E_DEVICE;
        w->state.store(2, std::memory_order_release);
    }
}
static void post_job(ChainWorker *w, const ChainJob &j) {
    w->job = j;
    {
        std::lock_guard<std::mutex> lk(w->mu);
        w->state.store(1, std::memory_order_release);
    }
    w->cv.notify_one();
}
static int wait_job(ChainWorker *w) {
    for (int spins = 0; w->state.load(std::memory_order_acquire) != 2; ++spins) {
        if (spins < 4096) __builtin_ia32_pause();
        else std::this_thread::yield();
    }
    w->state.store(0, std::memory_order_relaxed);
    return w->rc;
}
void stop_workers(ssd_env *env) {
    for (auto &w : env->workers) {
        {
            std::lock_guard<std::mutex> lk(w->mu);
            w->state.store(3, std::memory_order_release);
        }
        w->cv.notify_one();
        if (w->th.joinable()) w->th.join();
    }
    env->workers.clear();
}

static void aql_drain(ssd_env *env) {
    if (!env->aql) return;
    AqlState &A = *env->aql;
    if (!A.ok && !A.nq) return;
    if (!A.joins || !A.flag_kernarg) return;
    std::lock_guard<std::mutex> enqueue_lock(ssd::aql::enqueue_mutex(env->device));
    for (int c = 0; c < A.nq; ++c) {
        if (!A.q[c] || ssd::aql::queue_failed(A.q[c])) continue;
        if (ssd::aql::join_and_wait(A.q[c], A.flag_kernarg)) A.joins += 1;
    }
}

int after_timeout(ssd_env *env) {
    if (!env->aql || !env->aql->timed_out_host) return SSD_OK;
    AqlState &A = *env->aql;
    if (!__atomic_load_n(A.timed_out_host, __ATOMIC_ACQUIRE)) return SSD_OK;
    bool drained = true;
    if (A.joins && A.flag_kernarg) {
        std::lock_guard<std::mutex> enqueue_lock(ssd::aql::enqueue_mutex(env->device));
        for (int c = 0; c < A.nq; ++c) {
            if (!A.q[c] || ssd::aql::queue_failed(A.q[c])) continue;
            if (ssd::aql::join_and_wait(A.q[c], A.flag_kernarg, 10.0)) A.joins += 1; else drained = false;
        }
    }
    __atomic_store_n(A.timed_out_host, 0u, __ATOMIC_RELEASE);
    A.ok = false;
    env->err = drained ? "a rollout call's wait for the library's dispatch queues timed out (the WAIT_TIMEOUT status bit): its outputs may be incomplete; "
                         "the queues have been drained and the handle now steps through hipLaunchKernel"
                       : "a rollout call's wait for the library's dispatch queues timed out (the WAIT_TIMEOUT status bit) and the queues did not "
                         "drain within 10 s: its buffers may still be written to";
    return SSD_E_DEVICE;
}

void aql_teardown(ssd_env *env) {
    if (!env->aql) return;
    AqlState &A = *env->aql;
    aql_drain(env);
    for (uint64_t h : A.fork_sig) ssd::aql::signal_destroy(h);
    if (A.join_counter) (void)hipFree(A.join_counter);
    if (A.fork_counter) (void)hipFree(A.fork_counter);
    ssd::aql::host_kernarg_free(A.flag_kernarg);
    ssd::aql::host_kernarg_free(A.fork_kernarg);
    for (auto &st : A.sets) if (st.dev) (void)hipFree(st.dev);
    for (int i = 0; i < 2; ++i) { if (A.snap_grid[i]) (void)hipFree(A.snap_grid[i]); if (A.beam_list[i]) (void)hipFree(A.beam_list[i]); }
    if (A.world_buf[1]) (void)hipFree(A.world_buf[1]);
    if (A.agents_buf[1]) (void)hipFree(A.agents_buf[1]);
    for (int k = 0; k < plan::kMids; ++k)
        for (int i = 0; i < 2; ++i)
            for (void *m : {(void *)A.mid_world[k][i], (void *)A.mid_snap[k][i], (void *)A.mid_agents[k][i], (void *)A.mid_list[k][i]}) if (m) (void)hipFree(m);
    env->aql.reset();
}

static bool aql_ready(ssd_env *env, int chains) {
    if (!env->aql) env->aql.reset(new AqlState());
    AqlState &A = *env->aql;
    if (A.tried && !A.ok) return false;
    if (!A.tried) {
        A.tried = true;
        if (!ssd::aql::available(env->device)) return false;
        for (int i = 0; i < AqlState::kForks; ++i) {
            A.fork_sig[i] = ssd::aql::signal_create(0);
            if (!A.fork_sig[i]) return false;
        }
        void *ptr = nullptr;
        if (hipMalloc(&ptr, 8) != hipSuccess || hipMemset(ptr, 0, 8) != hipSuccess) { (void)hipGetLastError(); return false; }
        A.join_counter = static_cast<unsigned long long *>(ptr);
        A.flag_kernarg = ssd::aql::host_kernarg_alloc(env->device, 64);
        if (!A.flag_kernarg) return false;
        std::memcpy(A.flag_kernarg, &A.join_counter, sizeof(void *));
        {
            void *h = nullptr, *d = nullptr;
            if (hipHostMalloc(&h, 64, hipHostMallocMapped) != hipSuccess || hipHostGetDevicePointer(&d, h, 0) != hipSuccess) { (void)hipGetLastError(); return false; }
            A.timed_out_host = static_cast<uint32_t *>(h); A.timed_out_dev = static_cast<uint32_t *>(d);
            *A.timed_out_host = 0;
            env->host_allocs.push_back(h);
        }
        ptr = nullptr;
        if (hipMalloc(&ptr, 8) != hipSuccess || hipMemset(ptr, 0, 8) != hipSuccess) { (void)hipGetLastError(); return false; }
        A.fork_counter = static_cast<unsigned long long *>(ptr);
        A.fork_kernarg = static_cast<uint8_t *>(ssd::aql::host_kernarg_alloc(env->device, AqlState::kForks * AqlState::kForkBlock));
        if (!A.fork_kernarg || !ssd::aql::lookup(env->device, ssd::wait_kernel_fn(), &A.wait_kernel) || A.wait_kernel.kernarg_size > AqlState::kForkBlock) return false;
        {
            ssd::aql::signal_set(A.fork_sig[0], 1);
            ssd::launch_signal_kernel(ssd::aql::signal_value_ptr(A.fork_sig[0]), nullptr);
            ssd::launch_wait_counter_kernel(A.join_counter, 0, nullptr, 0, nullptr, nullptr, nullptr);
            ssd::launch_flag_kernel(A.fork_counter, nullptr); A.forks = 1;
            if (hipStreamSynchronize(nullptr) != hipSuccess) { (void)hipGetLastError(); return false; }
        }
        A.q[0] = ssd::aql::pool_queue(env->device, 0);
        if (!A.q[0]) return false;
        A.nq = 1;
        A.ok = true;
    }
    if (chains > ssd::aql::pool_size(env->device)) return false;
    while (A.nq < chains) {
        A.q[A.nq] = ssd::aql::pool_queue(env->device, A.nq);
        if (!A.q[A.nq]) return false;
        A.nq++;
    }
    for (int c = 0; c < A.nq; ++c) if (ssd::aql::queue_failed(A.q[c])) { A.ok = false; return false; }
    return true;
}

static inline void aql_wait_consumed(ssd::aql::Queue *q, uint64_t idx_plus_1) {
    while (idx_plus_1 && ssd::aql::read_index(q) < idx_plus_1 && !ssd::aql::queue_failed(q)) __builtin_ia32_pause();
}

static bool aql_split_buffers(ssd_env *env) {
    AqlState &A = *env->aql;
    if (A.world_buf[1]) return true;
    const size_t grid = (size_t)env->E * env->S, agents = (size_t)env->E * (env->N ? env->N : 1) * 4;
    const size_t lists = (size_t)env->E * 128 * 4;
    constexpr int kBufs = 6 + 8 * plan::kMids;
    size_t sizes[kBufs] = {grid, agents, grid, grid, lists, lists};
    for (int k = 0; k < plan::kMids; ++k) {
        const size_t mids[8] = {grid, grid, grid, grid, agents, agents, lists, lists};
        for (int j = 0; j < 8; ++j) sizes[6 + 8 * k + j] = mids[j];
    }
    void *buf[kBufs] = {};
    for (int i = 0; i < kBufs; ++i)
        if (hipMalloc(&buf[i], sizes[i]) != hipSuccess) {
            (void)hipGetLastError();
            for (int j = 0; j < i; ++j) (void)hipFree(buf[j]);
            return false;
        }
    A.world_buf[0] = env->p.world; A.agents_buf[0] = env->p.agents;
    A.agents_buf[1] = static_cast<uint32_t *>(buf[1]);
    A.snap_grid[0] = static_cast<uint8_t *>(buf[2]); A.snap_grid[1] = static_cast<uint8_t *>(buf[3]);
    A.beam_list[0] = static_cast<uint32_t *>(buf[4]); A.beam_list[1] = static_cast<uint32_t *>(buf[5]);
    for (int k = 0; k < plan::kMids; ++k)
        for (int i = 0; i < 2; ++i) {
            void **b = buf + 6 + 8 * k;
            A.mid_world[k][i] = static_cast<uint8_t *>(b[i]); A.mid_snap[k][i] = static_cast<uint8_t *>(b[2 + i]);
            A.mid_agents[k][i] = static_cast<uint32_t *>(b[4 + i]); A.mid_list[k][i] = static_cast<uint32_t *>(b[6 + i]);
        }
    A.world_buf[1] = static_cast<uint8_t *>(buf[0]);
    return true;
}

static AqlState::Set *aql_set(ssd_env *env, const AqlState::Key &key, int chains, const ChainJob *jobs) {
    AqlState &A = *env->aql;
    A.clock++;
    for (auto &st : A.sets) if (st.valid && st.key == key) { st.stamp = A.clock; return &st; }
    AqlState::Set *victim = &A.sets[0];
    for (auto &st : A.sets) { if (!st.valid) { victim = &st; break; } if (st.stamp < victim->stamp) victim = &st; }
    AqlState::Set &st = *victim;
    if (st.valid) for (int c = 0; c < 8 && c < A.nq; ++c) aql_wait_consumed(A.q[c], st.last_use[c]);
    st.valid = false;
    st.kinds = plan::kind_table(key.split, key.pairs);
    const int n_dense = st.kinds.n_dense;
    const size_t need = (size_t)chains * key.slots * n_dense * AqlState::kBlock;
    if (need > st.cap) {
        if (st.dev) (void)hipFree(st.dev);
        st.dev = nullptr; st.cap = 0;
        void *ptr = nullptr;
        if (hipMalloc(&ptr, need) != hipSuccess) { (void)hipGetLastError(); return nullptr; }
        st.dev = static_cast<uint8_t *>(ptr); st.cap = need;
    }
    if (key.split && !aql_split_buffers(env)) return nullptr;
    std::vector<uint8_t> host(need, 0);
    for (int c = 0; c < chains; ++c) {
        const ChainCursor cur = chain_cursor(env, jobs[c]);
        for (int i = 0; i < key.slots; ++i)
            for (int kind = 0; kind < plan::kKinds; ++kind) {
                if (st.kinds.dense[kind] < 0) continue;
                Params p;
                ssd::PairParams q;
                plan::fill_block(cur.p, cur, key, A, kind, i, p, q);
                ssd::Launch L;
                if (!ssd::select(p, env->game, &L, &q)) return nullptr;
                AqlState::Geo &g = st.geo[c][kind];
                if (i == 0) {
                    if (!ssd::aql::lookup(env->device, L.fn, &g.k) || g.k.kernarg_size > AqlState::kBlock || g.k.kernarg_size < sizeof(ssd::KernArgs)) return nullptr;
                    g.grid_x = L.grid_x; g.block_x = L.block_x; g.lds = L.lds;
                }
                std::memcpy(host.data() + (((size_t)c * key.slots + i) * n_dense + st.kinds.dense[kind]) * AqlState::kBlock, &L.args, L.args_bytes());
            }
    }
    if (hipMemcpy(st.dev, host.data(), need, hipMemcpyHostToDevice) != hipSuccess) { (void)hipGetLastError(); return nullptr; }
    st.key = key; st.valid = true; st.stamp = A.clock;
    for (auto &u : st.last_use) u = 0;
    return &st;
}

static int aql_fork(ssd_env *env, int chains, hipStream_t s, bool sync_mode) {
    AqlState &A = *env->aql;
    static const bool always_fork = SSD_HOOK("SSD_AQL_ALWAYS_FORK", 0) != 0;
    if (sync_mode) { SSD_HIP(env, hipStreamSynchronize(s)); env->last_path |= SSD_PATH_SYNC; }
    bool stream_idle = sync_mode || (!always_fork && hipStreamQuery(s) == hipSuccess);
    if (!stream_idle && !always_fork) {
        static const int spin_us = SSD_HOOK("SSD_AQL_FORK_SPIN_US", 8);
        const auto t0 = std::chrono::steady_clock::now();
        while (!stream_idle && std::chrono::steady_clock::now() - t0 < std::chrono::microseconds(spin_us))
            stream_idle = hipStreamQuery(s) == hipSuccess;
    }
    if (!stream_idle) {
        (void)hipGetLastError();
        const int slot = A.fork_next;
        A.fork_next = (A.fork_next + 1) % AqlState::kForks;
        for (int c = 0; c < A.nq; ++c) { aql_wait_consumed(A.q[c], A.fork_used[slot][c]); A.fork_used[slot][c] = 0; }
        static const int fork_kind = SSD_HOOK("SSD_AQL_FORK_KIND", 1);
        if (fork_kind == 1) {
            A.forks++;
            ssd::launch_flag_kernel(A.fork_counter, s);
            if (hipGetLastError() != hipSuccess) { A.forks--; env->err = "fork kernel launch failed"; return SSD_E_DEVICE; }
            ssd::WaitArgs wa{A.fork_counter, A.forks, ssd::aql::abort_flag_dev(env->device), 6000000000ull, env->p.status, A.timed_out_dev};
            uint8_t *ka = A.fork_kernarg + (size_t)slot * AqlState::kForkBlock;
            std::memcpy(ka, &wa, sizeof wa);
            for (int c = 0; c < chains; ++c) {
                ssd::aql::dispatch(A.q[c], A.wait_kernel, 1, 64, 0, ka, true, 0, 0);
                A.fork_used[slot][c] = ssd::aql::write_index(A.q[c]);
            }
        } else {
            ssd::aql::signal_set(A.fork_sig[slot], 1);
            ssd::launch_signal_kernel(ssd::aql::signal_value_ptr(A.fork_sig[slot]), s);
            if (hipGetLastError() != hipSuccess) { env->err = "fork kernel launch failed"; return SSD_E_DEVICE; }
            for (int c = 0; c < chains; ++c) {
                ssd::aql::barrier_and(A.q[c], A.fork_sig[slot]);
                A.fork_used[slot][c] = ssd::aql::write_index(A.q[c]);
            }
        }
        env->last_path |= SSD_PATH_FORKED;
    }
    return SSD_OK;
}

static int aql_join(ssd_env *env, AqlState::Set *st, int chains, int32_t n_steps, hipStream_t s, bool sync_mode) {
    AqlState &A = *env->aql;
    auto host_join = [&]() -> bool {
        bool ok = true;
        for (int c = 0; c < chains; ++c) ssd::aql::ring(A.q[c]);
        for (int c = 0; c < chains; ++c) { ok = ssd::aql::join_and_wait(A.q[c], A.flag_kernarg) && ok; st->last_use[c] = ssd::aql::write_index(A.q[c]); }
        A.joins += (unsigned long long)chains;
        return ok;
    };
    if (sync_mode) {
        if (!host_join()) { env->err = "the HSA runtime reported an error on a dispatch queue"; A.ok = false; return SSD_E_DEVICE; }
        return SSD_OK;
    }
    for (int c = 0; c < chains; ++c) {
        ssd::aql::join(A.q[c], A.flag_kernarg);
        st->last_use[c] = ssd::aql::write_index(A.q[c]);
    }
    A.joins += (unsigned long long)chains;
    unsigned long long timeout_ticks = (unsigned long long)((2.0 + 0.002 * (double)n_steps) * 1e8);
    static const int test_lost = SSD_HOOK("SSD_AQL_TEST_LOST_JOIN", 0), test_timeout_ms = SSD_HOOK("SSD_AQL_TEST_TIMEOUT_MS", 0);
    if (test_timeout_ms > 0) timeout_ticks = (unsigned long long)test_timeout_ms * 100000ull;
    (void)hipGetLastError();
    ssd::launch_wait_counter_kernel(A.join_counter, A.joins + (test_lost ? 1000000ull : 0ull), ssd::aql::abort_flag_dev(env->device), timeout_ticks,
                                    env->p.status, A.timed_out_dev, s);
    if (hipGetLastError() != hipSuccess) {
        bool ok = true;
        for (int c = 0; c < chains; ++c) ok = ssd::aql::join_and_wait(A.q[c], A.flag_kernarg) && ok;
        A.joins += (unsigned long long)chains;
        env->err = "join kernel launch failed (the call's work was waited for on the host)"; A.ok = false;
        return SSD_E_DEVICE;
    }
    for (int c = 0; c < chains; ++c) if (ssd::aql::queue_failed(A.q[c])) { env->err = "the HSA runtime reported an error on a dispatch queue"; A.ok = false; return SSD_E_DEVICE; }
    return SSD_OK;
}

static int rollout_aql(ssd_env *env, int chains, const ChainJob *jobs, hipStream_t s) {
    if (!aql_ready(env, chains)) return 1;
    AqlState &A = *env->aql;
    const ChainJob &j0 = jobs[0];
    AqlState::Key key;
    key.obs = j0.obs; key.rew = j0.rew; key.done = j0.done; key.ring = j0.ring; key.f32 = (j0.flags & SSD_OBS_F32) ? 1 : 0;
    key.num_actions = j0.num_actions; key.chains = chains; key.horizon = env->p.horizon;
    key.actions = j0.actions; key.order = j0.actions ? j0.order : nullptr; key.action_ring = j0.actions ? j0.action_ring : 0;
    key.slots = plan::block_slots(key.ring, key.action_ring, chains);
    if (!key.slots) return 1;
    key.stamps = env->p.stamps; key.dbg_skip = env->p.dbg_skip;
    static const int env_coh = SSD_KNOB("SSD_AQL_COHERENT", 1);
    static const int env_alternate = SSD_HOOK("SSD_AQL_ALTERNATE", 0);
    static const int env_split = SSD_KNOB("SSD_AQL_SPLIT", 1);
    static const int env_pairs = SSD_HOOK("SSD_AQL_PAIRS", 1);
    static const int env_run = SSD_HOOK("SSD_AQL_RUN", ssd::kMaxRun);
    plan::FormIn in;
    in.per_launch = (env->E + chains - 1) / chains; in.chains = chains;
    in.f32 = key.f32 != 0; in.order = key.order != nullptr; in.obs = j0.obs != nullptr; in.n_steps = j0.n_steps;
    in.fast_profile = ssd::fast_profile(env->p, env->game); in.pair_profile = ssd::pair_profile(env->p, env->game);
    in.aql_coherent = env_coh; in.aql_split = env_split; in.aql_alternate = env_alternate; in.aql_pairs = env_pairs; in.aql_run = env_run;
    const plan::Form form = plan::choose_form(in);
    const bool coherent = form.coherent != 0, split = form.split;
    key.coherent = form.coherent; key.split = form.key_split; key.pairs = form.pairs;
    key.world = key.split ? nullptr : env->p.world;
    AqlState::Set *st = aql_set(env, key, chains, jobs);
    if (!st) return 1;
    env->last_path |= SSD_PATH_AQL | (coherent ? SSD_PATH_COHERENT : 0) | (split ? SSD_PATH_SPLIT : 0);
    if (j0.n_steps == 0) return SSD_OK;
    std::lock_guard<std::mutex> enqueue_lock(ssd::aql::enqueue_mutex(env->device));
    const bool sync_mode = ssd::aql::sync_mode();
    if (const int rc = aql_fork(env, chains, s, sync_mode)) return rc;
    static const int env_acq = SSD_HOOK("SSD_AQL_ACQ", -1);
    static const int env_rel = SSD_HOOK("SSD_AQL_REL", -1);
    const int kAcq = env_acq >= 0 ? env_acq : (coherent ? 0 : 1), kRel = env_rel >= 0 ? env_rel : (coherent ? 0 : 1);
    const bool obs_wb = !key.f32 && plan::ring_past_cache(j0.obs, j0.ring, obs_bytes(env, false));
    const int o = plan::start_orientation(key.split, A.world_buf[1] && env->p.world == A.world_buf[1]);
    plan::Schedule sched(j0.n_steps, j0.step0, j0.reset_every, j0.ring, key.slots, split, form.run_cap, coherent, obs_wb, kAcq, kRel, o);
    plan::Group g;
    while (sched.next(g))
        for (int c = 0; c < chains; ++c) {
            for (int j = 0; j < g.n_packets; ++j) {
                const plan::Packet &pk = g.packet[j];
                const AqlState::Geo &geo = st->geo[c][pk.kind];
                ssd::aql::dispatch(A.q[c], geo.k, geo.grid_x, geo.block_x, geo.lds,
                                   st->dev + (((size_t)c * key.slots + pk.block) * st->kinds.n_dense + st->kinds.dense[pk.kind]) * AqlState::kBlock,
                                   true, pk.acquire, pk.release);
            }
            if (g.ring) ssd::aql::ring(A.q[c]);
        }
    if (sched.longest() > 1) env->last_path |= SSD_PATH_PAIRS;
    env->last_path = (env->last_path & ~(7 << SSD_PATH_RUN_SHIFT)) | (sched.longest() << SSD_PATH_RUN_SHIFT);
    if (split) {
        env->p.world = A.world_buf[sched.orientation()]; env->p.agents = A.agents_buf[sched.orientation()];
    }
    return aql_join(env, st, chains, j0.n_steps, s, sync_mode);
}

static int rollout(ssd_env *env, const int32_t *actions, const uint8_t *order, int32_t action_ring, int32_t num_actions, int32_t n_steps,
                   int32_t reset_every, int32_t step0, void *obs, int32_t *rew, uint8_t *done, int32_t ring, uint32_t flags, void *stream) {
    if (obs && (reinterpret_cast<uintptr_t>(obs) & 3u)) { env->err = "obs must be 4-byte aligned"; return SSD_E_INVALID; }
    if (flags & SSD_ROLLOUT_AUTO) {
        flags &= ~(uint32_t)SSD_ROLLOUT_AUTO;
        if (!(flags & SSD_OBS_F32) && !order && n_steps >= 2) flags |= SSD_ROLLOUT_FUSED;
    }
    if ((flags & SSD_ROLLOUT_FUSED) && (flags & SSD_OBS_F32)) { env->err = "the fused rollout kernel writes uint8 observations"; return SSD_E_INVALID; }
    {
        int cur = -1;
        if (hipGetDevice(&cur) != hipSuccess || cur != env->device) SSD_HIP(env, hipSetDevice(env->device));
    }
    if (const int rc = after_timeout(env)) return rc;
    hipStream_t s = static_cast<hipStream_t>(stream);
    env->last_stream = s; env->last_stream_set = true;
    uint8_t *o = static_cast<uint8_t *>(obs);
    static const int forced = SSD_KNOB("SSD_ROLLOUT_CHAINS", 0);
    auto by_size = [&]() { return env->E < 2048 ? 1 : (env->E >= 6144 && env->E <= 24576) ? 3 : 2; };
    int chains = env->rollout_chains > 0 ? env->rollout_chains : forced > 0 ? forced : by_size();
    if ((flags & SSD_ROLLOUT_FUSED) && env->rollout_chains <= 0 && forced <= 0) chains = 1;
    const bool automatic = env->rollout_chains <= 0 && forced <= 0;
    auto clamp_chains = [&]() {
        if (automatic && ssd::aql::pool_size(env->device) >= 1 && chains > ssd::aql::pool_size(env->device)) chains = ssd::aql::pool_size(env->device);
        if (automatic && ssd::aql::over_the_cliff(env->device)) chains = 1;
        if (chains > 8) chains = 8;
        if (chains > env->E) chains = env->E;
        if (chains < 1) chains = 1;
        env->last_path = (chains << 8) | ((flags & SSD_ROLLOUT_FUSED) ? SSD_PATH_FUSED : 0);
    };
    clamp_chains();
    auto range = [&](int c) { return (int)(((long long)env->E * c) / chains); };
    auto job_of = [&](int c, hipStream_t cs) {
        ChainJob j;
        j.chain = c; j.e_begin = range(c); j.e_end = range(c + 1);
        j.num_actions = num_actions; j.n_steps = n_steps; j.reset_every = reset_every; j.step0 = step0; j.ring = ring;
        j.actions = actions; j.order = order; j.action_ring = action_ring;
        j.obs = o; j.rew = rew; j.done = done; j.flags = flags; j.s = cs;
        return j;
    };
    if (!(flags & SSD_ROLLOUT_FUSED)) {
        for (int attempt = 0; attempt < 2; ++attempt) {
            ChainJob jobs[8];
            for (int c = 0; c < chains; ++c) jobs[c] = job_of(c, s);
            const int pool_before = ssd::aql::pool_size(env->device);
            const int rc = rollout_aql(env, chains, jobs, s);
            env->last_path |= ssd::aql::pool_report(env->device);
            if (rc <= 0) return rc;
            env->last_path &= ~(SSD_PATH_AQL | SSD_PATH_COHERENT | SSD_PATH_SPLIT | SSD_PATH_PAIRS | SSD_PATH_SYNC | SSD_PATH_FORKED | (7 << SSD_PATH_RUN_SHIFT));
            if (!automatic || ssd::aql::pool_size(env->device) >= pool_before) break;
            chains = by_size();
            clamp_chains();
            env->last_path |= ssd::aql::pool_report(env->device);
        }
    }
    if (chains <= 1) {
        int rc = rollout_chain(env, job_of(0, s));
        if (rc) env->err = "kernel launch failed in a rollout call";
        return rc;
    }
    while ((int)env->chain_streams.size() < chains - 1) {
        hipStream_t ns; hipEvent_t ne;
        SSD_HIP(env, hipStreamCreateWithFlags(&ns, hipStreamNonBlocking));
        SSD_HIP(env, hipEventCreateWithFlags(&ne, hipEventDisableTiming));
        env->chain_streams.push_back(ns); env->chain_events.push_back(ne);
    }
    if (!env->fork_event) SSD_HIP(env, hipEventCreateWithFlags(&env->fork_event, hipEventDisableTiming));
    static const int env_threads = SSD_HOOK("SSD_ROLLOUT_THREADS", -1);
    static const int inline_steps = SSD_HOOK("SSD_ROLLOUT_INLINE_STEPS", 256);
    bool threads = !(flags & SSD_ROLLOUT_FUSED) && n_steps > inline_steps;
    if (env_threads == 0) threads = false;
    if (env_threads == 1) threads = true;
    SSD_HIP(env, hipEventRecord(env->fork_event, s));
    for (int c = 1; c < chains; ++c) SSD_HIP(env, hipStreamWaitEvent(env->chain_streams[c - 1], env->fork_event, 0));
    int rc_all = SSD_OK;
    if (threads) {
        while ((int)env->workers.size() < chains - 1) {
            env->workers.emplace_back(new ChainWorker());
            ChainWorker *w = env->workers.back().get();
            w->th = std::thread(chain_worker_main, env, w);
        }
        for (int c = 1; c < chains; ++c) post_job(env->workers[c - 1].get(), job_of(c, env->chain_streams[c - 1]));
        rc_all = rollout_chain(env, job_of(0, s));
        for (int c = 1; c < chains; ++c) { const int rc = wait_job(env->workers[c - 1].get()); if (rc && !rc_all) rc_all = rc; }
    } else if (flags & SSD_ROLLOUT_FUSED) {
        for (int c = 0; c < chains; ++c) { const int rc = rollout_chain(env, job_of(c, c ? env->chain_streams[c - 1] : s)); if (rc && !rc_all) rc_all = rc; }
    } else {
        ChainCursor cur[8];
        for (int c = 0; c < chains; ++c) cur[c] = chain_cursor(env, job_of(c, c ? env->chain_streams[c - 1] : s));
        for (int k = 0; k < n_steps; ++k)
            for (int c = 0; c < chains; ++c) chain_launch_step(env, cur[c], k);
        if (hipGetLastError() != hipSuccess) rc_all = SSD_E_DEVICE;
    }
    for (int c = 1; c < chains; ++c) {
        SSD_HIP(env, hipEventRecord(env->chain_events[c - 1], env->chain_streams[c - 1]));
        SSD_HIP(env, hipStreamWaitEvent(s, env->chain_events[c - 1], 0));
    }
    if (rc_all) env->err = "kernel launch failed in a rollout call";
    return rc_all;
}

extern "C" {

int ssd_rollout_random(ssd_env *env, int32_t num_actions, int32_t n_steps, int32_t reset_every, int32_t step0,
                       void *obs, int32_t *rew, uint8_t *done, int32_t ring, uint32_t flags, void *stream) {
    if (!env || n_steps < 0 || reset_every < 0 || step0 < 0 || ring < 1) return SSD_E_INVALID;
    if (flags & SSD_HOST_PTRS) { env->err = "ssd_rollout_random takes device pointers"; return SSD_E_INVALID; }
    if (num_actions < 1 || num_actions > game_actions(env)) { env->err = "num_actions outside the game's Discrete(n)"; return SSD_E_INVALID; }
    return rollout(env, nullptr, nullptr, 0, num_actions, n_steps, reset_every, step0, obs, rew, done, ring, flags, stream);
}

int ssd_rollout_actions(ssd_env *env, const int32_t *actions, const uint8_t *order, int32_t action_ring, int32_t n_steps, int32_t reset_every,
                        int32_t step0, void *obs, int32_t *rew, uint8_t *done, int32_t ring, uint32_t flags, void *stream) {
    if (!env || n_steps < 0 || reset_every < 0 || step0 < 0 || ring < 1 || action_ring < 1) return SSD_E_INVALID;
    if (flags & SSD_HOST_PTRS) { env->err = "ssd_rollout_actions takes device pointers"; return SSD_E_INVALID; }
    if (!actions && env->N > 0) { env->err = "actions is null"; return SSD_E_INVALID; }
    return rollout(env, actions, order, action_ring, 0, n_steps, reset_every, step0, obs, rew, done, ring, flags, stream);
}

int ssd_profiler_attached(void) { return ssd::aql::tool_attached_now(); }

int ssd_rollout_path(const ssd_env *env) { return env ? env->last_path : SSD_E_INVALID; }

int ssd_set_rollout_chains(ssd_env *env, int32_t chains) {
    if (!env || chains < 0 || chains > 8) return SSD_E_INVALID;
    env->rollout_chains = chains;
    return SSD_OK;
}

}
```

sequential_social_dilemma_games_amd/csrc/ssd_rollout_plan.hpp:

```cpp
#pragma once
#include <stddef.h>
#include <stdint.h>

#include "ssd_internal.hpp"

#ifndef SSD_RING_EVERY
#define SSD_RING_EVERY 4
#endif

namespace ssd {
namespace plan __attribute__((visibility("hidden"))) {

enum Kind { kS = 0, kR = 1, kRn = 2, kA = 3, kAB = 4, kB = 5, kRun = 6, kKindsPerO = kRun + (kMaxRun + 1) * (kMaxRun + 1), kKinds = 2 * kKindsPerO };
constexpr int run_kind(int n, int rendered) { return kRun + n * (kMaxRun + 1) + rendered; }
constexpr bool run_len(int n, int cap) { return n == 1 || (n == 2 && cap >= 2) || (n > 2 && n == cap); }
constexpr bool run_kind_used(int base, int cap) {
    const int n = (base - kRun) / (kMaxRun + 1), rd = (base - kRun) % (kMaxRun + 1);
    if (n > 0 ? !run_len(n, cap) : rd == 0) return false;
    if (rd > 0 && !run_len(rd, cap)) return false;
    return n >= 2 || rd >= 2;
}

struct KindTable { int8_t dense[kKinds]; int n_dense; };
inline KindTable kind_table(int split, int pairs) {
    KindTable t;
    t.n_dense = 0;
    for (int kind = 0; kind < kKinds; ++kind) {
        const int o = kind / kKindsPerO, base = kind % kKindsPerO;
        const bool split_kind = base >= kRn, run = base >= kRun;
        const bool used = !(split_kind && !split) && !(run && !run_kind_used(base, pairs)) && !(!split && o == 1);
        t.dense[kind] = used ? (int8_t)t.n_dense++ : (int8_t)-1;
    }
    return t;
}

struct Key {
    const void *obs = nullptr, *rew = nullptr, *done = nullptr;
    int32_t ring = 0, f32 = 0, num_actions = 0, chains = 0, horizon = 0, coherent = 0, split = 0, pairs = 0;
    const void *actions = nullptr, *order = nullptr; int32_t action_ring = 0;
    int32_t slots = 0;
    const void *stamps = nullptr; uint32_t dbg_skip = 0;
    const void *world = nullptr;
    bool operator==(const Key &o) const {
        return stamps == o.stamps && dbg_skip == o.dbg_skip && world == o.world && obs == o.obs && rew == o.rew && done == o.done && ring == o.ring && f32 == o.f32 && num_actions == o.num_actions &&
               chains == o.chains && horizon == o.horizon && coherent == o.coherent && split == o.split && pairs == o.pairs && actions == o.actions && order == o.order &&
               action_ring == o.action_ring && slots == o.slots;
    }
};

inline int32_t block_slots(int32_t ring, int32_t action_ring, int chains) {
    const long long ar = action_ring > 0 ? action_ring : 1;
    long long a = ring, b = ar;
    while (b) { const long long t = a % b; a = b; b = t; }
    const long long l = (long long)ring / a * ar;
    if (l * chains > 2048) return 0;
    return (int32_t)l;
}

struct FormIn {
    int per_launch, chains;
    bool f32, order, obs;
    int n_steps;
    int fast_profile, pair_profile;
    int aql_coherent, aql_split, aql_alternate, aql_pairs, aql_run;
};
struct Form {
    int coherent;
    int key_split;
    bool split;
    int pairs;
    int run_cap;
};
inline Form choose_form(const FormIn &in) {
    Form f;
    const bool coherent = in.aql_coherent != 0 && !in.f32 && !in.order && in.fast_profile > 0 && in.per_launch <= 4096;
    f.coherent = coherent ? (in.aql_alternate != 0 ? 2 : 1) : 0;
    const int split_cap = in.chains == 1 ? 3072 : 2304;
    f.key_split = (coherent && in.aql_split != 0 && in.obs && in.per_launch <= split_cap) ? 1 : 0;
    f.split = f.key_split && in.n_steps >= 4;
    int cap = (f.key_split && in.aql_pairs != 0) ? in.pair_profile : 1;
    if (in.aql_run >= 1 && in.aql_run < cap) cap = in.aql_run;
    f.pairs = cap >= 2 ? cap : 0;
    f.run_cap = f.split ? f.pairs : 0;
    return f;
}

inline bool ring_past_cache(const void *obs, int32_t ring, size_t obs_bytes) { return obs && (size_t)ring * obs_bytes > ((size_t)232 << 20); }

struct ChainRings {
    uint8_t *obs; int32_t *rew; uint8_t *done;
    const int32_t *actions; const uint8_t *order; int32_t action_ring;
    size_t en, ob;
    int32_t num_actions;
};
inline void cursor_actions(const ChainRings &c, Params &p, size_t step_index) {
    if (c.actions) {
        const size_t at = (step_index % (size_t)c.action_ring) * c.en;
        p.actions = c.actions + at; p.order = c.order ? c.order + at : nullptr; p.num_actions_random = 0;
    } else { p.actions = nullptr; p.order = nullptr; p.num_actions_random = c.num_actions; }
}

constexpr int kMids = kMaxRun - 1;
struct SplitBuffers {
    uint8_t *world_buf[2] = {};
    uint32_t *agents_buf[2] = {};
    uint32_t *beam_list[2] = {};
    uint8_t *snap_grid[2] = {};
    uint8_t *mid_world[kMids][2] = {}, *mid_snap[kMids][2] = {};
    uint32_t *mid_agents[kMids][2] = {}, *mid_list[kMids][2] = {};
};

inline void fill_block(const Params &base, const ChainRings &cur, const Key &key, const SplitBuffers &A, int kind, int i, Params &p, PairParams &q) {
    const int r = i % key.ring;
    const int o = kind / kKindsPerO, kb = kind % kKindsPerO;
    const bool pair_kind = kb >= kRun;
    p = base;
    q = PairParams{};
    if (key.split) { p.world = A.world_buf[o]; p.agents = A.agents_buf[o]; }
    p.obs = cur.obs ? cur.obs + (size_t)r * cur.ob : nullptr;
    p.coherent = key.coherent ? ((key.coherent == 2 && o == 1) ? 2u : 1u) : 0u;
    if (kb == kR || kb == kRn) {
        p.mode = kModeReset; p.rotate = 0; p.num_actions_random = 0; p.actions = nullptr; p.order = nullptr; p.rew = nullptr; p.done = nullptr;
        if (kb == kRn) p.obs = nullptr;
        return;
    }
    p.mode = kModeStep; p.rotate = 1;
    cursor_actions(cur, p, (size_t)i);
    p.rew = cur.rew ? cur.rew + (size_t)r * cur.en : nullptr; p.done = cur.done ? cur.done + (size_t)r * cur.en : nullptr;
    if (pair_kind) {
        constexpr int kMax = kMaxRun;
        const int n = (kb - kRun) / (kMax + 1), rd = (kb - kRun) % (kMax + 1);
        auto ring_slot = [&](int d) { return ((r + d) % key.ring + key.ring) % key.ring; };
        auto slot_obs = [&](int sl) { return cur.obs ? cur.obs + (size_t)sl * cur.ob : nullptr; };
        p.mode = kModeStepPair;
        p.obs = nullptr;
        p.snap_mode = (n == 0 ? 4 : 1) | (rd > 0 ? 2 : 0);
        p.world_out = A.world_buf[1 - o]; p.agents_out = A.agents_buf[1 - o];
        p.beam_list = A.beam_list[o]; p.snap = A.snap_grid[o];
        p.beam_list_in = A.beam_list[1 - o]; p.snap_in = A.snap_grid[1 - o];
        q.n_pass = n; q.n_render = rd;
        for (int k = 0; k < n; ++k) {
            const int rk = ring_slot(k);
            PassRec &rec = q.pass[k];
            if (k + 1 < n) rec = PassRec{A.mid_world[k][o], A.mid_agents[k][o], A.mid_list[k][o], A.mid_snap[k][o], nullptr, nullptr, nullptr};
            else rec = PassRec{p.world_out, p.agents_out, p.beam_list, p.snap, nullptr, nullptr, nullptr};
            rec.rew = cur.rew ? cur.rew + (size_t)rk * cur.en : nullptr;
            rec.done = cur.done ? cur.done + (size_t)rk * cur.en : nullptr;
            rec.actions = cur.actions ? cur.actions + ((size_t)(i + k) % (size_t)cur.action_ring) * cur.en : nullptr;
        }
        const int first = n == 0 ? 0 : -rd;
        for (int t = kMax - rd; t < kMax - 1; ++t) {
            if (t < 0) continue;
            const int j = t - (kMax - rd);
            q.mid_in[t] = MidIn{A.mid_world[j][1 - o], A.mid_agents[j][1 - o], A.mid_list[j][1 - o], A.mid_snap[j][1 - o]};
            q.obs_b0[t] = slot_obs(ring_slot(first + j));
        }
        p.obs_b = slot_obs(ring_slot(first + rd - 1));
    } else if (kb >= kA) {
        uint8_t *obs_r = p.obs;
        uint8_t *obs_prev = cur.obs ? cur.obs + (size_t)((r + key.ring - 1) % key.ring) * cur.ob : nullptr;
        p.obs = nullptr;
        p.snap_mode = 1;
        p.world_out = A.world_buf[1 - o]; p.agents_out = A.agents_buf[1 - o];
        p.beam_list = A.beam_list[o]; p.snap = A.snap_grid[o];
        if (kb != kA) {
            p.snap_mode = kb == kB ? (2 | 4) : (1 | 2);
            p.beam_list_in = A.beam_list[1 - o]; p.snap_in = A.snap_grid[1 - o];
            p.obs_b = kb == kB ? obs_r : obs_prev;
        }
    }
}

inline int start_orientation(int key_split, bool state_in_second_buffer) { return key_split && state_in_second_buffer ? 1 : 0; }

struct Packet {
    size_t block;
    int kind;
    int acquire, release;
};
struct Group {
    Packet packet[4]; int n_packets;
    int step, steps;
    bool reset;
    bool ring;
};
class Schedule {
public:
    Schedule(int n_steps, int step0, int reset_every, int ring, int slots, bool split, int run_cap, bool coherent, bool obs_wb, int acq, int rel, int o)
        : n_steps_(n_steps), step0_(step0), reset_every_(reset_every), ring_(ring), slots_(slots), split_(split), run_cap_(split ? run_cap : 0),
          coherent_(coherent), obs_wb_(obs_wb), kAcq(acq), kRel(rel), o_(o) {}
    __attribute__((always_inline)) bool next(Group &g) {
        const int k = k_;
        if (k >= n_steps_) return false;
        const int KO = kKindsPerO;
        const size_t i = (size_t)((step0_ + k) % slots_);
        const bool reset = reset_every_ > 0 && (step0_ + k) % reset_every_ == 0;
        int avail = n_steps_ - k;
        if (reset_every_ > 0) { const int to_reset = reset_every_ - (step0_ + k) % reset_every_; if (to_reset < avail) avail = to_reset; }
        const int n = (run_cap_ > 2 && avail >= run_cap_) ? run_cap_ : (run_cap_ >= 2 && avail >= 2) ? 2 : 1;
        const bool last = k + n >= n_steps_;
        const int acq = k == 0 ? 1 : kAcq;
        Packet *pk = g.packet;
        if (reset) {
            if (split_ && pending_) *pk++ = Packet{i_prev_, o_ * KO + render_only(pending_), kAcq, kRel};
            *pk++ = Packet{i, o_ * KO + (split_ ? kRn : kR), acq, kRel};
        }
        const int rendered = reset ? 0 : pending_;
        const int base = !split_ ? (int)kS
                         : (n == 1 && rendered <= 1) ? (rendered == 1 ? (int)kAB : (int)kA)
                                                     : run_kind(n, rendered);
        bool round = false;
        for (int j = 0; j < n; ++j) round = round || (step0_ + k + j) % ring_ == 0;
        const int rel = (obs_wb_ && round) ? 1 : kRel;
        *pk++ = Packet{i, o_ * KO + base, reset ? kAcq : acq, rel};
        if (split_ && last) *pk++ = Packet{i, (1 - o_) * KO + render_only(n), kAcq, kRel};
        g.n_packets = (int)(pk - g.packet);
        g.step = k; g.steps = n; g.reset = reset;
#if SSD_RING_EVERY > 1
        g.ring = !coherent_ || launches_ < 2 || run_cap_ > 2 || (launches_ % SSD_RING_EVERY) == SSD_RING_EVERY - 1;
#else
        g.ring = true;
#endif
        if (split_) { o_ = 1 - o_; pending_ = n; i_prev_ = i; }
        if (n > longest_) longest_ = n;
        launches_++;
        k_ = k + n;
        return true;
    }
    int orientation() const { return o_; }
    int longest() const { return longest_; }
    static constexpr int render_only(int rendered) { return rendered == 1 ? (int)kB : run_kind(0, rendered); }

private:
    int n_steps_, step0_, reset_every_, ring_, slots_;
    bool split_; int run_cap_; bool coherent_, obs_wb_;
    int kAcq, kRel;
    int o_;
    int k_ = 0;
    int pending_ = 0;
    size_t i_prev_ = 0;
    int launches_ = 0;
    int longest_ = 0;
};

}
}
```

sequential_social_dilemma_games_amd/engine.py:

```python
import ctypes as C

import numpy as np

from . import _capi
from . import config as cfgmod
from . import constants as K


def _ptr(a):
    return None if a is None else a.ctypes.data_as(C.c_void_p)


class VecEngine(object):
    def __init__(self, game, ascii_map=None, num_envs=1, num_agents=1, view_len=K.VIEW_LEN, beam_len=K.BEAM_LEN,
                 seed=0, env_index_base=0, device=0, keep_beams=False, color_map=None, harvest_thresholds=None,
                 cleanup_thresholds=None, library_tables=False):
        self.game = int(game)
        if ascii_map is None:
            ascii_map = K.HARVEST_MAP if self.game == K.GAME_HARVEST else K.CLEANUP_MAP
        self.ascii_map = [str(r) for r in ascii_map]
        flat, self.H, self.W = cfgmod.ascii_to_bytes(self.ascii_map)
        self.E, self.N = int(num_envs), int(num_agents)
        self.view_len, self.V, self.beam_len = int(view_len), 2 * int(view_len) + 1, int(beam_len)
        self.seed, self.env_index_base, self.device = int(seed), int(env_index_base), int(device)
# ... 153 lines not shown
        if rc:
            _capi.check(rc, self._h)
        self._count_after_step(auto_reset)
        return obs, rew, done

    def _count_steps(self, n):
        if self.steps_since_full_reset is not None:
            self.steps_since_full_reset += n

    def set_rollout_chains(self, chains):
        _capi.check(self._L.ssd_set_rollout_chains(self._h, int(chains)), self._h)

    def _rollout_args(self, obs, rew, done):
        cache = getattr(self, "_roll_cache", None)
        if cache is not None and cache[0] is obs and cache[1] is rew and cache[2] is done:
            return cache[3]
        torch, dev = self._torch()
        first = obs if obs is not None else rew if rew is not None else done
        if first is None:
            raise ValueError("a rollout needs at least one of obs / rew / done (their leading dimension is the output ring)")
        ring = int(first.shape[0])
        if obs is not None:
            if obs.dtype not in (torch.uint8, torch.float32):
                raise ValueError("obs must be uint8 or float32")
            self._check_tensor(obs, (ring, self.E, self.N, self.V, self.V, 3), obs.dtype, "obs")
        if rew is not None:
            self._check_tensor(rew, (ring, self.E, self.N), torch.int32, "rew")
        if done is not None:
            self._check_tensor(done, (ring, self.E, self.N), torch.uint8, "done")
        args = (self._dp(obs), self._dp(rew), self._dp(done), ring, (_capi.SSD_OBS_F32 if obs is not None and obs.dtype == torch.float32 else 0))
        self._roll_cache = (obs, rew, done, args)
        return args

    def _count_rollout(self, n_steps, reset_every, step0):
        n_steps, reset_every, step0 = int(n_steps), int(reset_every), int(step0)
        last = None
        if reset_every > 0 and n_steps > 0:
            k = (n_steps - 1) - ((step0 + n_steps - 1) % reset_every)
            last = k if k >= 0 else None
        if last is not None:
            self.steps_since_full_reset = n_steps - last
        else:
            self._count_steps(n_steps)

    def _check_stats(self, stats, rew, n_steps):
        if stats is None:
            return
        if rew is None:
            raise ValueError("stats need the call's rewards: pass rew")
        if stats.E != self.E or stats.N != self.N or stats.device != self.device:
            raise ValueError("stats were made for %d envs x %d agents on device %d, the engine has %d x %d on device %d"
                             % (stats.E, stats.N, stats.device, self.E, self.N, self.device))
        if int(rew.shape[0]) < int(n_steps):
            raise ValueError("stats need every step's rewards: the rew ring (%d) is shorter than n_steps (%d)"
                             % (int(rew.shape[0]), int(n_steps)))

    def rollout_random(self, n_steps, obs, rew=None, done=None, reset_every=0, step0=0, num_actions=None, fused=False, stats=None):
        self._check_stats(stats, rew, n_steps)
        po, pr, pd, ring, f32 = self._rollout_args(obs, rew, done)
        na = self.num_actions if num_actions is None else int(num_actions)
        rc = self._L.ssd_rollout_random(self._h, na, int(n_steps), int(reset_every), int(step0), po, pr, pd, ring,
                                        f32 | self._fused_flag(fused), self._stream())
        if rc:
            _capi.check(rc, self._h)
        self._count_rollout(n_steps, reset_every, step0)
        if stats is not None:
            stats.fold(rew, None, step0=step0, n_steps=n_steps, reset_every=reset_every)

    def rollout_actions(self, actions, n_steps, obs, rew=None, done=None, reset_every=0, step0=0, fused=False, order=None,
                        stats=None):
        torch, dev = self._torch()
        self._check_stats(stats, rew, n_steps)
        cache = getattr(self, "_act_cache", None)
        if cache is not None and cache[0] is actions and cache[1] is order:
            pa, pord, aring = cache[2]
        else:
            aring = int(actions.shape[0])
            self._check_tensor(actions, (aring, self.E, self.N), torch.int32, "actions")
            if order is not None:
                self._check_tensor(order, (aring, self.E, self.N), torch.uint8, "order")
            pa, pord = self._dp(actions), self._dp(order)
            self._act_cache = (actions, order, (pa, pord, aring))
        po, pr, pd, ring, f32 = self._rollout_args(obs, rew, done)
        rc = self._L.ssd_rollout_actions(self._h, pa, pord, aring, int(n_steps), int(reset_every), int(step0), po, pr, pd, ring,
                                         f32 | self._fused_flag(fused), self._stream())
        if rc:
            _capi.check(rc, self._h)
        self._count_rollout(n_steps, reset_every, step0)
        if stats is not None:
            stats.fold(rew, None, step0=step0, n_steps=n_steps, reset_every=reset_every)

    @staticmethod
    def _fused_flag(fused):
        if isinstance(fused, str):
            if fused != "auto":
                raise ValueError("fused must be True, False or 'auto'")
            return _capi.SSD_ROLLOUT_AUTO
        return _capi.SSD_ROLLOUT_FUSED if fused else 0

    def _policy_weights(self, policy):
        from .policy import ConvFCPolicy, ConvLSTMPolicy, ConvMOAPolicy
        torch, dev = self._torch()
        if not isinstance(policy, (ConvFCPolicy, ConvLSTMPolicy, ConvMOAPolicy)):
            raise ValueError("policy must be a ConvFCPolicy, a ConvLSTMPolicy or a ConvMOAPolicy")
        if policy.TAKES_PREV_ACTIONS and policy.num_agents != self.N:
            raise ValueError("the MOA policy is built for %d agents, the engine has %d" % (policy.num_agents, self.N))
        if self.V != _capi.SSD_POL_VIEW:
            raise ValueError("the policy network takes 15 x 15 views (view_len 7); this engine has V = %d" % self.V)
        if policy.num_actions != self.num_actions:
            raise ValueError("the policy has %d actions, the game Discrete(%d)" % (policy.num_actions, self.num_actions))
        if policy.num_sets not in (1, self.N):
            raise ValueError("the policy has %d weight sets: 1 (shared) or %d (one per agent) expected" % (policy.num_sets, self.N))
        if policy.conv_w.device != dev:
            raise ValueError("the policy's parameters are on %s, the engine on %s" % (policy.conv_w.device, dev))
        if self.N < 1:
            raise ValueError("a policy needs at least one agent")
        return policy.num_sets

    def _scratch(self, key, shape, dtype):
        flat, t = self._scratch_bufs.get(key, (None, None))
        if t is None or tuple(t.shape) != shape:
            torch, dev = self._torch()
            n = int(np.prod(shape))
            if flat is None or flat.numel() < n:
                flat = torch.empty(n, dtype=dtype, device=dev)
            t = flat[:n].view(shape)
            self._scratch_bufs[key] = (flat, t)
        return t

    def _check_actions_like(self, t, shape, name):
        torch, dev = self._torch()
        if not isinstance(t, torch.Tensor):
            raise ValueError("%s must be an int32 tensor of shape %s" % (name, tuple(shape)))
        self._check_tensor(t, tuple(shape), torch.int32, name)

    def _check_state(self, state, shape, who, shown):
        torch, dev = self._torch()
        if not isinstance(state, torch.Tensor):
            raise ValueError("%s needs state: a float32 tensor %s" % (who, shown))
        self._check_tensor(state, shape, torch.float32, "state")

    def _check_starts(self, starts, lead):
        torch, dev = self._torch()
        if starts is None:
            return None
        if not isinstance(starts, torch.Tensor) or starts.dtype not in (torch.bool, torch.uint8):
            raise ValueError("starts must be a bool or uint8 tensor of shape %s" % (lead,))
        self._check_tensor(starts, lead, starts.dtype, "starts")
        return starts.view(torch.uint8)

    @staticmethod
    def _check_clip(influence_clip):
        clip = float(influence_clip)
        if not (0.0 <= clip < float("inf")):
            raise ValueError("influence_clip must be finite and >= 0")
        return clip

    def policy_forward(self, policy, obs, state=None, starts=None, prev_actions=None, actions=None, influence_clip=10.0):
        torch, dev = self._torch()
        P = self._policy_weights(policy)
        V, N, A = self.V, self.N, self.num_actions
        if not isinstance(obs, torch.Tensor) or obs.dtype != torch.uint8 or obs.device != dev or not obs.is_contiguous() \
                or obs.dim() < 4 or tuple(obs.shape[-4:]) != (N, V, V, 3):
            raise ValueError("obs must be a contiguous uint8 tensor of shape [..., %d, %d, %d, 3] on %s" % (N, V, V, dev))
        B = obs.numel() // (N * V * V * 3)
        if B < 1:
            raise ValueError("obs holds no observation")
        lead = tuple(obs.shape[:-3])
        rows, moa = policy.STATE_ROWS, policy.TAKES_PREV_ACTIONS
        if not moa and (prev_actions is not None or actions is not None):
            raise ValueError("prev_actions and actions belong to a ConvMOAPolicy")
        if not rows:
            if state is not None or starts is not None:
                raise ValueError("state and starts belong to a ConvLSTMPolicy; a ConvFCPolicy has no state")
        else:
            C = policy.cell_size
            self._check_state(state, lead + (rows, C), "a " + type(policy).__name__, lead + (rows, C))
        if moa:
            self._check_actions_like(prev_actions, lead, "prev_actions")
            if actions is not None:
                self._check_actions_like(actions, lead, "actions")
        starts = self._check_starts(starts, lead)
        clip = self._check_clip(influence_clip) if moa else None
        e = lambda shape: torch.empty(lead + shape, dtype=torch.float32, device=dev)
        dp = self._dp
        logits, value = e((A,)), e(())
        out, net, inp, res, extra = (logits, value), [], [], [], []
        if rows:
            new_state = torch.empty_like(state)
            scratch = self._scratch("policy", policy.scratch_shape(B * N), torch.float32)
            net, inp, res = [C], [dp(state), dp(starts)], [dp(scratch), dp(new_state)]
            out += (new_state,)
        if moa:
            pred, cf, infl = e((N - 1, A)), e((A, N - 1, A)), e(()) if actions is not None else None
            inp.insert(0, dp(prev_actions))
            extra = [dp(pred), dp(cf), dp(actions), dp(infl), clip]
            out = (logits, value, pred, cf, new_state, infl)
        w = policy.packed()
        _capi.policy_check(getattr(self._L, policy.C_FORWARD)(dp(w), P, A, *net, dp(obs), *inp, B, N, *res, dp(logits), dp(value),
                                                               *extra, self.device, 0, self._stream()))
        return out

    def rollout_policy(self, policy, obs_in, n_steps, obs, actions=None, logp=None, value=None, logits=None, rew=None, done=None,
                       last_value=None, step0=0, greedy=False, stats=None, state=None, state_ring=None, state_every=1,
                       prev_actions=None, prev_actions_ring=None, influence=None, influence_clip=10.0):
        torch, dev = self._torch()
        P = self._policy_weights(policy)
        SR, moa = policy.STATE_ROWS, policy.TAKES_PREV_ACTIONS
        n_steps, step0 = int(n_steps), int(step0)
        if n_steps < 1:
            raise ValueError("n_steps must be >= 1")
        if step0 < 0:
            raise ValueError("step0 must be >= 0")
        E, N, V, A = self.E, self.N, self.V, self.num_actions
        if not isinstance(obs, torch.Tensor) or obs.dim() != 6:
            raise ValueError("obs must be a uint8 ring [R,%d,%d,%d,%d,3]" % (E, N, V, V))
        R = int(obs.shape[0])
        if R < 1:
            raise ValueError("the ring length must be >= 1")
        self._check_tensor(obs, (R, E, N, V, V, 3), torch.uint8, "obs")
        if not isinstance(obs_in, torch.Tensor):
            raise ValueError("obs_in must be a uint8 tensor [%d,%d,%d,%d,3]" % (E, N, V, V))
        self._check_tensor(obs_in, (E, N, V, V, 3), torch.uint8, "obs_in")
        if R > 1 and (E * N) % 4:
            raise ValueError("an observation ring of more than one slot needs num_envs * num_agents to be a multiple of 4")
        for t, dt, shape, name in ((actions, torch.int32, (R, E, N), "actions"), (logp, torch.float32, (R, E, N), "logp"),
                                   (value, torch.float32, (R, E, N), "value"), (logits, torch.float32, (R, E, N, A), "logits"),
                                   (rew, torch.int32, (R, E, N), "rew"), (done, torch.uint8, (R, E, N), "done"),
                                   (last_value, torch.float32, (E, N), "last_value")):
            if t is not None:
                if not isinstance(t, torch.Tensor):
                    raise ValueError("%s must be a tensor" % name)
                self._check_tensor(t, shape, dt, name)
        if stats is not None:
            self._check_stats(stats, rew, n_steps)
            if done is None:
                raise ValueError("stats need the call's done flags: pass done")
        if not SR:
            if state is not None or state_ring is not None:
                raise ValueError("state and state_ring belong to a ConvLSTMPolicy; a ConvFCPolicy has no state")
        else:
            C = policy.cell_size
            self._check_state(state, (E, N, SR, C), "a recurrent policy", "[%d,%d,%d,%d]" % (E, N, SR, C))
            state_every = int(state_every)
            S = 0
            if state_ring is not None:
                if state_every < 1:
                    raise ValueError("state_every must be >= 1")
                if not isinstance(state_ring, torch.Tensor) or state_ring.dim() != 5:
                    raise ValueError("state_ring must be a float32 ring [S,%d,%d,%d,%d]" % (E, N, SR, C))
                S = int(state_ring.shape[0])
                self._check_tensor(state_ring, (S, E, N, SR, C), torch.float32, "state_ring")
                if S < -(-n_steps // state_every):
                    raise ValueError("state_ring needs ceil(n_steps / state_every) = %d slots, has %d" % (-(-n_steps // state_every), S))
                if state_ring.data_ptr() < state.data_ptr() + state.numel() * 4 and state.data_ptr() < state_ring.data_ptr() + state_ring.numel() * 4:
                    raise ValueError("state_ring must not overlap state")
        if moa:
            self._check_actions_like(prev_actions, (E, N), "prev_actions")
            if prev_actions_ring is not None:
                self._check_actions_like(prev_actions_ring, (R, E, N), "prev_actions_ring")
            if influence is not None:
                if not isinstance(influence, torch.Tensor):
                    raise ValueError("influence must be a float32 ring [R,%d,%d]" % (E, N))
                self._check_tensor(influence, (R, E, N), torch.float32, "influence")
            clip = self._check_clip(influence_clip)
        elif prev_actions is not None or prev_actions_ring is not None or influence is not None:
            raise ValueError("prev_actions, prev_actions_ring and influence belong to a ConvMOAPolicy")
        if actions is None:
            actions = self._scratch("actions", (R, E, N), torch.int32)
        w = policy.packed()
        dp = self._dp
        head = [self._h, dp(w), P, dp(obs_in), n_steps, step0]
        if SR:
            head.insert(3, C)
            head += [dp(state), dp(state_ring), S, state_every]
            if moa:
                head += [dp(prev_actions), dp(prev_actions_ring), dp(influence), clip]
            head.append(dp(self._scratch("policy", policy.scratch_shape(E * N), torch.float32)))
        rc = getattr(self._L, policy.C_ROLLOUT)(*head, dp(obs), dp(actions), dp(logp), dp(value), dp(logits), dp(rew), dp(done), R,
                                                dp(last_value), _capi.SSD_POLICY_GREEDY if greedy else 0, self._stream())
        if rc:
            _capi.check(rc, self._h)
        self._count_auto_steps(n_steps)
        if stats is not None:
            stats.fold(rew, done, step0=step0, n_steps=n_steps)
        return actions

    def _count_auto_steps(self, n):
        s, h = self.steps_since_full_reset, getattr(self, "horizon", 0)
        if s is None:
            return
        if h <= 0:
            self.steps_since_full_reset = s + n
            return
        first = max(h - s, 1)
        self.steps_since_full_reset = s + n if n < first else (n - first) % h

    def rollout_path(self):
        m = self._L.ssd_rollout_path(self._h)
        return {"aql": bool(m & _capi.SSD_PATH_AQL), "coherent": bool(m & _capi.SSD_PATH_COHERENT), "split": bool(m & _capi.SSD_PATH_SPLIT),
                "pairs": bool(m & _capi.SSD_PATH_PAIRS),
                "fused": bool(m & _capi.SSD_PATH_FUSED), "sync": bool(m & _capi.SSD_PATH_SYNC), "forked": bool(m & _capi.SSD_PATH_FORKED),
                "queue_dropped": bool(m & _capi.SSD_PATH_QUEUE_DROPPED), "chains": (m >> 8) & 15, "pool": (m >> 12) & 7,
                "agent_match": ("none", "pci", "uuid", "ordinal")[(m >> 16) & 3], "run": (m >> _capi.SSD_PATH_RUN_SHIFT) & 7}

    def observe(self, rotate=True, obs=None):
        torch, dev = self._torch()
        if obs is None:
            obs = torch.empty((self.E, self.N, self.V, self.V, 3), dtype=torch.uint8, device=dev)
        _capi.check(self._L.ssd_observe(self._h, self._dp(obs), (0 if rotate else _capi.SSD_NO_ROTATE) | self._obs_flags(obs),
                                        self._stream()), self._h)
        return obs

    def _host_out(self):
        return (np.zeros((self.E, self.N, self.V, self.V, 3), np.uint8), np.zeros((self.E, self.N), np.int32),
                np.zeros((self.E, self.N), np.uint8))

    def reset_host(self, mask=None):
        obs = np.zeros((self.E, self.N, self.V, self.V, 3), np.uint8)
        m = None if mask is None else np.ascontiguousarray(mask, dtype=np.uint8).reshape(self.E)
        _capi.check(self._L.ssd_reset(self._h, _ptr(m), _ptr(obs), _capi.SSD_HOST_PTRS, None), self._h)
        self.steps_since_full_reset = 0 if mask is None else None
        return obs

    def step_host(self, actions, order=None):
        actions = np.ascontiguousarray(actions, dtype=np.int32).reshape(self.E, self.N)
        if order is not None:
            order = np.ascontiguousarray(order, dtype=np.uint8).reshape(self.E, self.N)
        obs, rew, done = self._host_out()
        _capi.check(self._L.ssd_step(self._h, _ptr(actions), _ptr(order), _ptr(obs), _ptr(rew), _ptr(done),
                                     _capi.SSD_HOST_PTRS, None), self._h)
        self._count_steps(1)
        return obs, rew, done

    def step_random_host(self):
        act = np.zeros((self.E, self.N), np.int32)
        obs, rew, done = self._host_out()
        _capi.check(self._L.ssd_step_random(self._h, self.num_actions, _ptr(act), _ptr(obs), _ptr(rew), _ptr(done),
                                            _capi.SSD_HOST_PTRS, None), self._h)
        self._count_steps(1)
        return act, obs, rew, done

    def observe_host(self, rotate=True):
        obs = np.zeros((self.E, self.N, self.V, self.V, 3), np.uint8)
        flags = _capi.SSD_HOST_PTRS | (0 if rotate else _capi.SSD_NO_ROTATE)
        _capi.check(self._L.ssd_observe(self._h, _ptr(obs), flags, None), self._h)
        return obs

    def get_state(self):
        E, N, H, W = self.E, self.N, self.H, self.W
        s = dict(world=np.zeros((E, H, W), np.int8), beam=np.zeros((E, H, W), np.int8) if self.keep_beams else None,
                 pos=np.zeros((E, N, 2), np.int16), orient=np.zeros((E, N), np.uint8),
                 episode=np.zeros(E, np.uint32), t=np.zeros(E, np.uint32))
        _capi.check(self._L.ssd_get_state(self._h, _ptr(s["world"]), _ptr(s["beam"]), _ptr(s["pos"]), _ptr(s["orient"]),
                                          _ptr(s["episode"]), _ptr(s["t"])), self._h)
        return s

    def set_state(self, world=None, beam=None, pos=None, orient=None, episode=None, t=None):
        E, N, H, W = self.E, self.N, self.H, self.W

        def prep(a, dt, shape, name):
            if a is None:
                return None
            a = np.ascontiguousarray(a, dtype=dt)
            if a.shape != shape:
                raise ValueError("%s must have shape %s, got %s" % (name, shape, a.shape))
            return a
        world, beam = prep(world, np.int8, (E, H, W), "world"), prep(beam, np.int8, (E, H, W), "beam")
        pos, orient = prep(pos, np.int16, (E, N, 2), "pos"), prep(orient, np.uint8, (E, N), "orient")
        episode, t = prep(episode, np.uint32, (E,), "episode"), prep(t, np.uint32, (E,), "t")
        _capi.check(self._L.ssd_set_state(self._h, _ptr(world), _ptr(beam), _ptr(pos), _ptr(orient), _ptr(episode),
                                          _ptr(t)), self._h)
        if t is not None:
            self.steps_since_full_reset = None

    def set_horizon(self, horizon):
        _capi.check(self._L.ssd_set_horizon(self._h, int(horizon)), self._h)
        self.horizon = int(horizon)

    def waste_count(self):
        out = np.zeros(self.E, np.uint32)
        _capi.check(self._L.ssd_get_waste_count(self._h, _ptr(out)), self._h)
        return out

    def render_full(self, e=0):
        rgb = np.zeros((self.H, self.W, 3), np.uint8)
        _capi.check(self._L.ssd_render_full(self._h, int(e), _ptr(rgb)), self._h)
        return rgb

    def render_frames(self, e_begin=0, count=None, out=None, host=False):
        count = self.E - e_begin if count is None else int(count)
        if e_begin < 0 or count < 0 or e_begin + count > self.E:
            raise ValueError("env range [%d, %d) outside the batch of %d" % (e_begin, e_begin + count, self.E))
        shape = (count, self.H, self.W, 3)
        if host:
            rgb = np.zeros(shape, np.uint8) if out is None else out
            if rgb.dtype != np.uint8 or rgb.shape != shape or not rgb.flags.c_contiguous:
                raise ValueError("out must be a C-contiguous uint8 array of shape %s" % (shape,))
            if count:
                _capi.check(self._L.ssd_render_frames(self._h, int(e_begin), count, _ptr(rgb), _capi.SSD_HOST_PTRS, None), self._h)
            return rgb
        torch, dev = self._torch()
        if out is None:
            out = torch.empty(shape, dtype=torch.uint8, device=dev)
        elif out.dtype != torch.uint8 or tuple(out.shape) != shape or not out.is_contiguous():
            raise ValueError("out must be a contiguous uint8 tensor of shape %s" % (shape,))
        if count:
            _capi.check(self._L.ssd_render_frames(self._h, int(e_begin), count, self._dp(out), 0, self._stream()), self._h)
        return out

    def agent_action_obs(self, actions=None, done=None, out=None):
        torch, dev = self._torch()
        shape = (self.E, self.N, max(self.N - 1, 0))
        if actions is not None:
            self._check_tensor(actions, (self.E, self.N), torch.int32, "actions")
        if done is not None:
            self._check_tensor(done, (self.E, self.N), torch.uint8, "done")
        oaa, vis = out if out is not None else (torch.empty(shape, dtype=torch.int64, device=dev), torch.empty(shape, dtype=torch.int64, device=dev))
        for t, name in ((oaa, "other_agent_actions"), (vis, "visible_agents")):
            self._check_tensor(t, shape, torch.int64, name)
        _capi.check(self._L.ssd_agent_action_obs(self._h, self._dp(actions), self._dp(done), self._dp(oaa), self._dp(vis), 0,
                                                 self._stream()), self._h)
        return oaa, vis

    def agent_action_obs_host(self, actions=None, done=None):
        shape = (self.E, self.N, max(self.N - 1, 0))
        oaa, vis = np.zeros(shape, np.int64), np.zeros(shape, np.int64)
        a = None if actions is None else np.ascontiguousarray(actions, dtype=np.int32).reshape(self.E, self.N)
        d = None if done is None else np.ascontiguousarray(done, dtype=np.uint8).reshape(self.E, self.N)
        _capi.check(self._L.ssd_agent_action_obs(self._h, _ptr(a), _ptr(d), _ptr(oaa), _ptr(vis), _capi.SSD_HOST_PTRS, None), self._h)
        return oaa, vis

    def status(self, clear=True):
        st = C.c_uint32(0)
        _capi.check(self._L.ssd_device_status(self._h, C.byref(st), int(clear)), self._h)
        return st.value

    def synchronize(self):
        _capi.check(self._L.ssd_synchronize(self._h), self._h)

    def algorithmic_bytes_per_env_step(self):
        return cfgmod.algorithmic_bytes_per_env_step(self.H, self.W, self.N, self.V)
```

Baseline: 5.324 billion.

## Add eight-step long-run kernel mode to batch more steps per launch

Adds a kModeStepLong kernel mode and LongParams kernarg block so one dispatch runs up to eight environment steps instead of the four used by the pair mode. The split renderer processes two halves of four layers each. The schedule picks the long run when enough steps remain, which cuts the number of AQL packets and dispatches per step. In exchange the kernarg blocks get larger, the schedule kinds and dense tables get more complex, and the bigger fused kernel may hurt register pressure or latency.

```diff
diff --git a/sequential_social_dilemma_games_amd/csrc/ssd_internal.hpp b/sequential_social_dilemma_games_amd/csrc/ssd_internal.hpp
--- a/sequential_social_dilemma_games_amd/csrc/ssd_internal.hpp
+++ b/sequential_social_dilemma_games_amd/csrc/ssd_internal.hpp
@@ -25,7 +25,8 @@
     kModeStep = 0, kModeReset = 1, kModeObserve = 2,
     kModeRollout = 3,
     kModeStepAuto = 4,
-    kModeStepPair = 5
+    kModeStepPair = 5,
+    kModeStepLong = 6
 };
 
 enum Stream : uint32_t {
@@ -100,6 +101,14 @@
     uint8_t *obs_b0[kMaxRun - 1];
 };
 
+constexpr int kLongRun = 8;
+struct LongParams {
+    PassRec pass[kLongRun];
+    int32_t n_pass, n_render;
+    MidIn mid_in[kLongRun - 1];
+    uint8_t *obs_b0[kLongRun - 1];
+};
+
 struct KernArgs {
     uint4 *hdr; uint32_t *agents; uint8_t *world;
     int32_t E, e_begin, epb, n_apple;
@@ -109,6 +118,8 @@
 static_assert(sizeof(KernArgs) == 56 + sizeof(Params), "kernarg layout");
 struct PairKernArgs { KernArgs k; PairParams q; };
 static_assert(sizeof(PairKernArgs) == sizeof(KernArgs) + sizeof(PairParams), "kernarg layout");
+struct LongKernArgs { KernArgs k; LongParams q; };
+static_assert(sizeof(LongKernArgs) == sizeof(KernArgs) + sizeof(LongParams), "kernarg layout");
 
 struct Launch {
     const void *fn = nullptr;
@@ -127,6 +138,7 @@
 int envs_per_block(const Params &p, bool f32);
 int fast_profile(const Params &p, int game);
 int pair_profile(const Params &p, int game);
+int long_profile(const Params &p, int game);
 bool select(const Params &p, int game, Launch *out, const PairParams *pair = nullptr);
 void launch(const Launch &L, void *stream);
 void launch(const Params &p, int game, void *stream);
diff --git a/sequential_social_dilemma_games_amd/csrc/ssd_kernels.hip b/sequential_social_dilemma_games_amd/csrc/ssd_kernels.hip
--- a/sequential_social_dilemma_games_amd/csrc/ssd_kernels.hip
+++ b/sequential_social_dilemma_games_amd/csrc/ssd_kernels.hip
@@ -235,16 +235,18 @@
 constexpr int run_max() { return (GAME == 0 || NA == 5) ? kMaxRun : 2; }
 
 template <int GAME, int MODE, bool F32, int NA, bool STD, int FAST, bool COH = false, bool ACTS = false>
-__global__ __launch_bounds__(64 * kMaxEnvsPerBlock) __attribute__((amdgpu_waves_per_eu(MODE == kModeStepPair ? 8 : 0, MODE == kModeStepPair ? 8 : 0)))
+__global__ __launch_bounds__(64 * kMaxEnvsPerBlock) __attribute__((amdgpu_waves_per_eu((MODE == kModeStepPair || MODE == kModeStepLong) ? 8 : 0, (MODE == kModeStepPair || MODE == kModeStepLong) ? 8 : 0)))
 void ssd_env_kernel(uint4 *const a_hdr, uint32_t *const a_agents, uint8_t *const a_world,
                                                                         const int a_E, const int a_e_begin, const int a_epb, const int a_n_apple,
                                                                         const uint32_t *const a_apple_cells, const uint32_t *const a_lut,
                                                                         const Params p) {
+    constexpr bool lng = MODE == kModeStepLong;
+    using QP = std::conditional_t<lng, LongParams, PairParams>;
     typedef const __attribute__((address_space(4))) uint64_t karg_u64;
     [[maybe_unused]] karg_u64 *const qargs = (karg_u64 *)((const __attribute__((address_space(4))) char *)__builtin_amdgcn_kernarg_segment_ptr() + sizeof(KernArgs));
     [[maybe_unused]] auto qptr = [&](size_t at, auto *like) { return reinterpret_cast<decltype(like)>(qargs[at / 8]); };
     [[maybe_unused]] auto load_rec = [&](int k) {
-        const size_t at = offsetof(PairParams, pass) + (size_t)k * sizeof(PassRec);
+        const size_t at = offsetof(QP, pass) + (size_t)k * sizeof(PassRec);
         PassRec r;
         r.world = qptr(at + offsetof(PassRec, world), r.world); r.agents = qptr(at + offsetof(PassRec, agents), r.agents);
         r.beam_list = qptr(at + offsetof(PassRec, beam_list), r.beam_list); r.snap = qptr(at + offsetof(PassRec, snap), r.snap);
@@ -268,7 +270,7 @@
     const bool has_order = !FAST && p.order != nullptr, keep_beams = !FAST && p.keep_beams != 0;
     constexpr bool roll = MODE == kModeRollout;
     constexpr bool auto_mode = MODE == kModeStepAuto;
-    constexpr bool pair = MODE == kModeStepPair;
+    constexpr bool pair = MODE == kModeStepPair || lng;
     constexpr bool stepping = MODE == kModeStep || auto_mode || pair;
     uint32_t *s_lut = reinterpret_cast<uint32_t *>(smem + (size_t)wv * (512 + 256 + (F32 ? 2048 : 0) + (size_t)A0 + (size_t)A1 +
                                                                             (roll ? 4 : 3) * (size_t)S));
@@ -351,7 +353,7 @@
             return;
         }
     }
-    if constexpr (pair && COH && STD && NA > 0 && NA % 5 == 0 && !F32 && FAST != 0) {
+    if constexpr (pair && !lng && COH && STD && NA > 0 && NA % 5 == 0 && !F32 && FAST != 0) {
         if ((p.snap_mode & 2) && blk >= p.blocks_a) {
             const int eb = a_e_begin + (blk - p.blocks_a) * a_epb + wv;
             if (eb < a_E) {
@@ -461,6 +463,120 @@
             return;
         }
     }
+    if constexpr (lng && COH && STD && NA > 0 && NA % 5 == 0 && !F32 && FAST != 0) {
+        if ((p.snap_mode & 2) && blk >= p.blocks_a) {
+            const int eb = a_e_begin + (blk - p.blocks_a) * a_epb + wv;
+            if (eb < a_E) {
+                typedef __attribute__((address_space(3))) const uint8_t lds_u8;
+                constexpr int kGridLoads = (fm.S + 1023) / 1024;
+                constexpr bool kTwoLists = GAME == 1 && NA > 5;
+                constexpr int kHalf = kLongRun / 2;
+                static_assert(kHalf == 4, "a half is the step-pair kernels' two rounds of two layers");
+                const int n_render = (int)(uint32_t)(qargs[offsetof(LongParams, n_pass) / 8] >> 32);
+                struct MidPtr { const uint8_t *world; const uint32_t *agents; const uint32_t *list; const uint8_t *snap; uint8_t *obs; };
+                auto mid_ptr = [&](int t) {
+                    const size_t at = offsetof(LongParams, mid_in) + (size_t)t * sizeof(MidIn);
+                    MidPtr m;
+                    m.world = qptr(at + offsetof(MidIn, world), m.world); m.agents = qptr(at + offsetof(MidIn, agents), m.agents);
+                    m.list = qptr(at + offsetof(MidIn, beam_list), m.list); m.snap = qptr(at + offsetof(MidIn, snap), m.snap);
+                    m.obs = qptr(offsetof(LongParams, obs_b0) + (size_t)t * sizeof(uint8_t *), m.obs);
+                    return m;
+                };
+                struct StepIn { u32x4_t g[kGridLoads]; uint32_t areg, entry, entry2; };
+                auto fetch = [&](const uint8_t *world, const uint32_t *agents, const uint32_t *list) {
+                    StepIn s;
+                    const rsrc_t grid_r = make_rsrc(world + (size_t)eb * S, (uint32_t)S);
+#pragma unroll
+                    for (int j = 0; j < kGridLoads; ++j) s.g[j] = load16_sc1(grid_r, (uint32_t)(lane * 16 + j * 1024));
+                    s.areg = 0; s.entry2 = 0;
+                    if (lane < N) s.areg = __hip_atomic_load(agents + (size_t)eb * N + lane, __ATOMIC_RELAXED, __HIP_MEMORY_SCOPE_AGENT);
+                    s.entry = __hip_atomic_load(list + (size_t)eb * 64 + lane, __ATOMIC_RELAXED, __HIP_MEMORY_SCOPE_AGENT);
+                    return s;
+                };
+                auto fetch_rare = [&](StepIn &s, const uint32_t *list, const uint8_t *snap) {
+                    const uint32_t flags = rfl(s.areg) >> 20;
+                    if (kTwoLists && (flags & 4u)) s.entry2 = __hip_atomic_load(list + ((size_t)p.E_total + eb) * 64 + lane, __ATOMIC_RELAXED, __HIP_MEMORY_SCOPE_AGENT);
+                    if (flags & 2u) {
+                        const rsrc_t snap_r = make_rsrc(snap + (size_t)eb * S, (uint32_t)S);
+#pragma unroll
+                        for (int j = 0; j < kGridLoads; ++j) s.g[j] = load16_sc1(snap_r, (uint32_t)(lane * 16 + j * 1024));
+                    }
+                };
+                const uint32_t lut_a = a_lut[lane], lut_b = a_lut[lane + 64];
+                const uint4 vt0 = reinterpret_cast<const uint4 *>(p.view_tab)[2 * lane], vt1 = reinterpret_cast<const uint4 *>(p.view_tab)[2 * lane + 1];
+                static_assert(fm.S >= fm.A0 + fm.A1, "the renderer's second layer fits the beam and occupancy layers");
+                uint8_t *const s_world2 = s_world + S + A1 + A0;
+                {
+                    const uint4 z = make_uint4(0x30303030u, 0x30303030u, 0x30303030u, 0x30303030u);
+                    const int n0 = A0 >> 4, n1 = A1 >> 4;
+                    for (int i = lane; i < n0 + n1; i += 64) {
+                        const int at = i < n0 ? i * 16 - A0 : S + (i - n0) * 16;
+                        *reinterpret_cast<uint4 *>(s_world + at) = z;
+                        if (n_render > 1) *reinterpret_cast<uint4 *>(s_world2 + at) = z;
+                    }
+                }
+                s_lut[lane] = lut_a; s_lut[lane + 64] = lut_b;
+                auto fill = [&](const StepIn &s, uint8_t *layer) {
+                    const uint32_t flags = rfl(s.areg) >> 20;
+#pragma unroll
+                    for (int j = 0; j < kGridLoads; ++j) {
+                        if (lane * 16 + j * 1024 < S) *reinterpret_cast<uint4 *>(layer + lane * 16 + j * 1024) = make_uint4(s.g[j].x, s.g[j].y, s.g[j].z, s.g[j].w);
+                    }
+                    wave_sync();
+                    if (!(flags & 2u)) {
+                        if (lane < N && (s.areg & (1u << 19))) layer[s.areg & 0xFFFFu] = agent_glyph((uint32_t)lane);
+                        wave_sync();
+                        if (flags & 1u) {
+                            if (s.entry) layer[s.entry & 0xFFFFu] = (uint8_t)(s.entry >> 16);
+                            wave_sync();
+                            if constexpr (kTwoLists) {
+                                if (s.entry2) layer[s.entry2 & 0xFFFFu] = (uint8_t)(s.entry2 >> 16);
+                                wave_sync();
+                            }
+                        }
+                    }
+                };
+                auto views = [&](const uint32_t areg, const uint8_t *layer, uint8_t *obs_to) {
+                    const uint32_t cellb = areg & 0xFFFFu, orientb = (areg >> 16) & 3u;
+                    const uint32_t kq = (0x8Du >> (2u * orientb)) & 3u;
+                    const uint32_t s0 = (uint32_t)((int)cellb - 7 * (WP + 1) + (kq >= 2 ? 14 * (WP + 1) : 0));
+                    render_views_std<NA, true>(lane, WP, kq, s0, (uint32_t)(uintptr_t)(lds_u8 *)layer, s_lut, obs_to + (size_t)eb * N * SSD_OBS_STRIDE, p.obs_wt,
+                                               vt0, vt1);
+                };
+#pragma nounroll
+                for (int h = n_render > kHalf ? 0 : 1; h < 2; ++h) {
+                    const int t0 = kHalf * h;
+                    auto used = [&](int t) { return t0 + t >= kLongRun - n_render; };
+                    MidPtr last = MidPtr{a_world, a_agents, p.beam_list_in, p.snap_in, p.obs_b};
+                    if (h == 0) last = mid_ptr(kHalf - 1);
+                    StepIn sm[kHalf - 1];
+                    MidPtr mp[kHalf - 1];
+                    StepIn sb = fetch(last.world, last.agents, last.list);
+#pragma unroll
+                    for (int t = kHalf - 2; t >= 0; --t) {
+                        sm[t] = sb; mp[t] = MidPtr{};
+                        if (used(t)) { mp[t] = mid_ptr(t0 + t); sm[t] = fetch(mp[t].world, mp[t].agents, mp[t].list); }
+                    }
+                    fetch_rare(sb, last.list, last.snap);
+#pragma unroll
+                    for (int t = kHalf - 2; t >= 0; --t)
+                        if (used(t)) fetch_rare(sm[t], mp[t].list, mp[t].snap);
+                    if (used(1)) {
+                        fill(sm[1], s_world);
+                        if (used(0)) { fill(sm[0], s_world2); views(sm[0].areg, s_world2, mp[0].obs); }
+                        views(sm[1].areg, s_world, mp[1].obs);
+                        wave_sync();
+                    }
+                    fill(sb, s_world);
+                    if (used(2)) { fill(sm[2], s_world2); views(sm[2].areg, s_world2, mp[2].obs); }
+                    views(sb.areg, s_world, last.obs);
+                    wave_sync();
+                }
+                asm volatile("s_waitcnt vmcnt(0)" ::: "memory");
+            }
+            return;
+        }
+    }
     const int e = a_e_begin + blk * a_epb + wv;
     constexpr int mode = pair ? (int)kModeStep : MODE;
     bool active = e < a_E;
@@ -475,7 +591,7 @@
             return kCoh ? __hip_atomic_load(ptr, __ATOMIC_RELAXED, __HIP_MEMORY_SCOPE_AGENT) : *ptr;
         };
         constexpr bool kPre = GAME == 1 && (MODE == kModeStep || pair) && COH && FAST != 0;
-        constexpr int kPreUp = pair ? kMaxRun - 1 : 0;
+        constexpr int kPreUp = lng ? kLongRun - 1 : pair ? kMaxRun - 1 : 0;
         uint4 hdr;
         [[maybe_unused]] PassRec rec{};
         [[maybe_unused]] int n_pass = 1;
@@ -483,7 +599,7 @@
             const uint32_t hv = cload(reinterpret_cast<const uint32_t *>(a_hdr + e) + (lane & 3));
             if constexpr (pair) {
                 rec = load_rec(0);
-                n_pass = (int)(uint32_t)qargs[offsetof(PairParams, n_pass) / 8];
+                n_pass = (int)(uint32_t)qargs[offsetof(QP, n_pass) / 8];
                 asm volatile("" ::"s"(rec.world), "s"(rec.agents), "s"(rec.beam_list), "s"(rec.snap), "s"(rec.rew), "s"(rec.done), "s"(n_pass));
             }
             if constexpr (kPre) asm volatile("" ::"s"(p.waste_cells), "s"(p.thr_ca), "s"(p.thr_cw), "s"(p.n_thr));
@@ -498,7 +614,7 @@
         int act_in = -1;
         int act_next = -1;
         [[maybe_unused]] auto next_actions = [&](int k) {
-            return qptr(offsetof(PairParams, pass) + (size_t)k * sizeof(PassRec) + offsetof(PassRec, actions), (const uint32_t *)nullptr);
+            return qptr(offsetof(QP, pass) + (size_t)k * sizeof(PassRec) + offsetof(PassRec, actions), (const uint32_t *)nullptr);
         };
         uint32_t ord_in = 0xFFu;
         uint32_t eN32 = rfl((uint32_t)e * (uint32_t)N);
@@ -1578,6 +1694,11 @@
             if (p.coherent) return kernel_fn<GAME, kModeStepPair, false, NA, STD, FAST, true>();
         }
         return nullptr;
+    } else if (p.mode == kModeStepLong) {
+        if constexpr (GAME == 0 && FAST == 1 && NA == 5 && !F32 && STD) {
+            if (p.coherent) return kernel_fn<GAME, kModeStepLong, false, NA, STD, FAST, true>();
+        }
+        return nullptr;
     } else {
         if constexpr (!F32 && FAST != 0) {
             if (p.coherent) return kernel_fn<GAME, kModeStep, false, NA, STD, FAST, true>();
@@ -1607,9 +1728,13 @@
     return p.N == 5 ? run_max<1, 5, 1>() : run_max<1, 10, 1>();
 }
 
+int long_profile(const Params &p, int game) {
+    return (game == 0 && p.N == 5 && !p.obs_f32 && fast_profile(p, game) == 1 && pair_profile(p, game) == kMaxRun) ? kLongRun : 0;
+}
+
 template <int GAME, bool F32>
 static const void *select_game(const Params &p) {
-    if (p.mode == kModeStep || p.mode == kModeRollout || p.mode == kModeStepAuto || p.mode == kModeStepPair) {
+    if (p.mode == kModeStep || p.mode == kModeRollout || p.mode == kModeStepAuto || p.mode == kModeStepPair || p.mode == kModeStepLong) {
         const bool std_view = p.view_len == 7 && p.beam_len == 5;
         const int fast = fast_profile(p, GAME);
         if (std_view && p.N == 5) {
@@ -1660,7 +1785,7 @@
 }
 
 void launch(const Launch &L, void *stream) {
-    if (L.args.p.mode == kModeStepPair) return;
+    if (L.args.p.mode == kModeStepPair || L.args.p.mode == kModeStepLong) return;
     KernArgs &k = const_cast<KernArgs &>(L.args);
     void *args[] = {&k.hdr, &k.agents, &k.world, &k.E, &k.e_begin, &k.epb, &k.n_apple, &k.apple_cells, &k.lut, &k.p};
     (void)hipLaunchKernel(L.fn, dim3(L.grid_x), dim3(L.block_x), args, L.lds, static_cast<hipStream_t>(stream));
diff --git a/sequential_social_dilemma_games_amd/csrc/ssd_rollout.hip b/sequential_social_dilemma_games_amd/csrc/ssd_rollout.hip
--- a/sequential_social_dilemma_games_amd/csrc/ssd_rollout.hip
+++ b/sequential_social_dilemma_games_amd/csrc/ssd_rollout.hip
@@ -61,17 +61,27 @@
         Key key;
         uint8_t *dev = nullptr;
         size_t cap = 0;
-        Geo geo[8][plan::kKinds];
+        Geo geo[8][plan::kAllKinds];
         plan::KindTable kinds;
+        plan::LongKindTable long_kinds;
+        size_t long_at = 0;
+        uint8_t *block_of(int c, size_t block, int kind) const {
+            if (plan::is_long_kind(kind))
+                return dev + long_at + (((size_t)c * key.slots + block) * long_kinds.n_dense + long_kinds.dense[kind - plan::kKinds]) * kLongBlock;
+            return dev + (((size_t)c * key.slots + block) * kinds.n_dense + kinds.dense[kind]) * kBlock;
+        }
         uint64_t last_use[8] = {};
         uint64_t stamp = 0;
     };
     static constexpr int kSets = 4;
     static constexpr size_t kBlock = 896;
+    static constexpr size_t kLongBlock = 1216;
+    bool long_tried = false;
     Set sets[kSets];
     uint64_t clock = 0;
 };
 static_assert(AqlState::kBlock >= sizeof(ssd::PairKernArgs), "an argument block holds the largest kernarg segment");
+static_assert(AqlState::kLongBlock >= sizeof(ssd::LongKernArgs) && AqlState::kLongBlock % 64 == 0, "a long block holds a long launch's kernarg segment");
 
 void RolloutDelete::operator()(ChainWorker *w) const { delete w; }
 void RolloutDelete::operator()(AqlState *a) const { delete a; }
@@ -232,6 +242,9 @@
     for (int k = 0; k < plan::kMids; ++k)
         for (int i = 0; i < 2; ++i)
             for (void *m : {(void *)A.mid_world[k][i], (void *)A.mid_snap[k][i], (void *)A.mid_agents[k][i], (void *)A.mid_list[k][i]}) if (m) (void)hipFree(m);
+    for (int k = 0; k < plan::kLongMids - plan::kMids; ++k)
+        for (int i = 0; i < 2; ++i)
+            for (void *m : {(void *)A.long_world[k][i], (void *)A.long_snap[k][i], (void *)A.long_agents[k][i], (void *)A.long_list[k][i]}) if (m) (void)hipFree(m);
     env->aql.reset();
 }
 
@@ -322,6 +335,29 @@
     return true;
 }
 
+static bool aql_long_buffers(ssd_env *env) {
+    AqlState &A = *env->aql;
+    constexpr int kSets = plan::kLongMids - plan::kMids;
+    if (A.long_tried) return A.long_world[0][0] != nullptr;
+    A.long_tried = true;
+    const size_t grid = (size_t)env->E * env->S, agents = (size_t)env->E * (env->N ? env->N : 1) * 4, lists = (size_t)env->E * 128 * 4;
+    const size_t mids[8] = {grid, grid, grid, grid, agents, agents, lists, lists};
+    void *buf[8 * kSets] = {};
+    for (int i = 0; i < 8 * kSets; ++i)
+        if (hipMalloc(&buf[i], mids[i % 8]) != hipSuccess) {
+            (void)hipGetLastError();
+            for (int j = 0; j < i; ++j) (void)hipFree(buf[j]);
+            return false;
+        }
+    for (int k = 0; k < kSets; ++k)
+        for (int i = 0; i < 2; ++i) {
+            void **b = buf + 8 * k;
+            A.long_world[k][i] = static_cast<uint8_t *>(b[i]); A.long_snap[k][i] = static_cast<uint8_t *>(b[2 + i]);
+            A.long_agents[k][i] = static_cast<uint32_t *>(b[4 + i]); A.long_list[k][i] = static_cast<uint32_t *>(b[6 + i]);
+        }
+    return true;
+}
+
 static AqlState::Set *aql_set(ssd_env *env, const AqlState::Key &key, int chains, const ChainJob *jobs) {
     AqlState &A = *env->aql;
     A.clock++;
@@ -331,9 +367,12 @@
     AqlState::Set &st = *victim;
     if (st.valid) for (int c = 0; c < 8 && c < A.nq; ++c) aql_wait_consumed(A.q[c], st.last_use[c]);
     st.valid = false;
+    st.key = key;
     st.kinds = plan::kind_table(key.split, key.pairs);
+    st.long_kinds = plan::long_kind_table(key.long_cap);
     const int n_dense = st.kinds.n_dense;
-    const size_t need = (size_t)chains * key.slots * n_dense * AqlState::kBlock;
+    st.long_at = (size_t)chains * key.slots * n_dense * AqlState::kBlock;
+    const size_t need = st.long_at + (size_t)chains * key.slots * st.long_kinds.n_dense * AqlState::kLongBlock;
     if (need > st.cap) {
         if (st.dev) (void)hipFree(st.dev);
         st.dev = nullptr; st.cap = 0;
@@ -359,6 +398,23 @@
                     g.grid_x = L.grid_x; g.block_x = L.block_x; g.lds = L.lds;
                 }
                 std::memcpy(host.data() + (((size_t)c * key.slots + i) * n_dense + st.kinds.dense[kind]) * AqlState::kBlock, &L.args, L.args_bytes());
+            }
+        for (int i = 0; i < key.slots; ++i)
+            for (int kind = plan::kKinds; kind < plan::kAllKinds; ++kind) {
+                if (st.long_kinds.dense[kind - plan::kKinds] < 0) continue;
+                Params p;
+                ssd::LongParams q;
+                plan::fill_long_block(cur.p, cur, key, A, kind, i, p, q);
+                ssd::Launch L;
+                if (!ssd::select(p, env->game, &L)) return nullptr;
+                AqlState::Geo &g = st.geo[c][kind];
+                if (i == 0) {
+                    if (!ssd::aql::lookup(env->device, L.fn, &g.k) || g.k.kernarg_size > AqlState::kLongBlock || g.k.kernarg_size < sizeof(ssd::KernArgs)) return nullptr;
+                    g.grid_x = L.grid_x; g.block_x = L.block_x; g.lds = L.lds;
+                }
+                uint8_t *at = host.data() + (st.block_of(c, (size_t)i, kind) - st.dev);
+                std::memcpy(at, &L.args, sizeof(ssd::KernArgs));
+                std::memcpy(at + sizeof(ssd::KernArgs), &q, sizeof q);
             }
     }
     if (hipMemcpy(st.dev, host.data(), need, hipMemcpyHostToDevice) != hipSuccess) { (void)hipGetLastError(); return nullptr; }
@@ -459,15 +515,17 @@
     static const int env_alternate = SSD_HOOK("SSD_AQL_ALTERNATE", 0);
     static const int env_split = SSD_KNOB("SSD_AQL_SPLIT", 1);
     static const int env_pairs = SSD_HOOK("SSD_AQL_PAIRS", 1);
-    static const int env_run = SSD_HOOK("SSD_AQL_RUN", ssd::kMaxRun);
+    static const int env_run = SSD_HOOK("SSD_AQL_RUN", ssd::kLongRun);
     plan::FormIn in;
     in.per_launch = (env->E + chains - 1) / chains; in.chains = chains;
     in.f32 = key.f32 != 0; in.order = key.order != nullptr; in.obs = j0.obs != nullptr; in.n_steps = j0.n_steps;
     in.fast_profile = ssd::fast_profile(env->p, env->game); in.pair_profile = ssd::pair_profile(env->p, env->game);
     in.aql_coherent = env_coh; in.aql_split = env_split; in.aql_alternate = env_alternate; in.aql_pairs = env_pairs; in.aql_run = env_run;
-    const plan::Form form = plan::choose_form(in);
+    in.long_profile = ssd::long_profile(env->p, env->game);
+    plan::Form form = plan::choose_form(in);
+    if (form.key_long && !aql_long_buffers(env)) form.key_long = form.long_cap = 0;
     const bool coherent = form.coherent != 0, split = form.split;
-    key.coherent = form.coherent; key.split = form.key_split; key.pairs = form.pairs;
+    key.coherent = form.coherent; key.split = form.key_split; key.pairs = form.pairs; key.long_cap = form.key_long;
     key.world = key.split ? nullptr : env->p.world;
     AqlState::Set *st = aql_set(env, key, chains, jobs);
     if (!st) return 1;
@@ -481,21 +539,19 @@
     const int kAcq = env_acq >= 0 ? env_acq : (coherent ? 0 : 1), kRel = env_rel >= 0 ? env_rel : (coherent ? 0 : 1);
     const bool obs_wb = !key.f32 && plan::ring_past_cache(j0.obs, j0.ring, obs_bytes(env, false));
     const int o = plan::start_orientation(key.split, A.world_buf[1] && env->p.world == A.world_buf[1]);
-    plan::Schedule sched(j0.n_steps, j0.step0, j0.reset_every, j0.ring, key.slots, split, form.run_cap, coherent, obs_wb, kAcq, kRel, o);
+    plan::Schedule sched(j0.n_steps, j0.step0, j0.reset_every, j0.ring, key.slots, split, form.run_cap, coherent, obs_wb, kAcq, kRel, o, form.long_cap);
     plan::Group g;
     while (sched.next(g))
         for (int c = 0; c < chains; ++c) {
             for (int j = 0; j < g.n_packets; ++j) {
                 const plan::Packet &pk = g.packet[j];
                 const AqlState::Geo &geo = st->geo[c][pk.kind];
-                ssd::aql::dispatch(A.q[c], geo.k, geo.grid_x, geo.block_x, geo.lds,
-                                   st->dev + (((size_t)c * key.slots + pk.block) * st->kinds.n_dense + st->kinds.dense[pk.kind]) * AqlState::kBlock,
-                                   true, pk.acquire, pk.release);
+                ssd::aql::dispatch(A.q[c], geo.k, geo.grid_x, geo.block_x, geo.lds, st->block_of(c, pk.block, pk.kind), true, pk.acquire, pk.release);
             }
             if (g.ring) ssd::aql::ring(A.q[c]);
         }
     if (sched.longest() > 1) env->last_path |= SSD_PATH_PAIRS;
-    env->last_path = (env->last_path & ~(7 << SSD_PATH_RUN_SHIFT)) | (sched.longest() << SSD_PATH_RUN_SHIFT);
+    env->last_path = (env->last_path & ~(15 << SSD_PATH_RUN_SHIFT)) | (sched.longest() << SSD_PATH_RUN_SHIFT);
     if (split) {
         env->p.world = A.world_buf[sched.orientation()]; env->p.agents = A.agents_buf[sched.orientation()];
     }
@@ -549,7 +605,7 @@
             const int rc = rollout_aql(env, chains, jobs, s);
             env->last_path |= ssd::aql::pool_report(env->device);
             if (rc <= 0) return rc;
-            env->last_path &= ~(SSD_PATH_AQL | SSD_PATH_COHERENT | SSD_PATH_SPLIT | SSD_PATH_PAIRS | SSD_PATH_SYNC | SSD_PATH_FORKED | (7 << SSD_PATH_RUN_SHIFT));
+            env->last_path &= ~(SSD_PATH_AQL | SSD_PATH_COHERENT | SSD_PATH_SPLIT | SSD_PATH_PAIRS | SSD_PATH_SYNC | SSD_PATH_FORKED | (15 << SSD_PATH_RUN_SHIFT));
             if (!automatic || ssd::aql::pool_size(env->device) >= pool_before) break;
             chains = by_size();
             clamp_chains();
diff --git a/sequential_social_dilemma_games_amd/csrc/ssd_rollout_plan.hpp b/sequential_social_dilemma_games_amd/csrc/ssd_rollout_plan.hpp
--- a/sequential_social_dilemma_games_amd/csrc/ssd_rollout_plan.hpp
+++ b/sequential_social_dilemma_games_amd/csrc/ssd_rollout_plan.hpp
@@ -34,6 +34,28 @@
     return t;
 }
 
+constexpr int kLongLens = 5;
+constexpr int kLongLen[kLongLens] = {0, 1, 2, 4, kLongRun};
+constexpr int kLongPerO = 2 * kLongLens - 1, kLongKinds = 2 * kLongPerO, kAllKinds = kKinds + kLongKinds;
+constexpr int long_len_index(int n) { return n == 0 ? 0 : n == 1 ? 1 : n == 2 ? 2 : n == 4 ? 3 : n == kLongRun ? 4 : -1; }
+constexpr bool is_long_kind(int kind) { return kind >= kKinds; }
+constexpr bool long_counts(int n, int rendered) {
+    return (n == kLongRun && long_len_index(rendered) >= 0) || (rendered == kLongRun && long_len_index(n) >= 0);
+}
+constexpr int long_kind(int o, int n, int rendered) {
+    return kKinds + o * kLongPerO + (n == kLongRun ? long_len_index(rendered) : kLongLens + long_len_index(n));
+}
+constexpr int long_kind_o(int kind) { return (kind - kKinds) / kLongPerO; }
+constexpr int long_kind_n(int kind) { return (kind - kKinds) % kLongPerO < kLongLens ? kLongRun : kLongLen[(kind - kKinds) % kLongPerO - kLongLens]; }
+constexpr int long_kind_rendered(int kind) { return (kind - kKinds) % kLongPerO < kLongLens ? kLongLen[(kind - kKinds) % kLongPerO] : kLongRun; }
+struct LongKindTable { int8_t dense[kLongKinds]; int n_dense; };
+inline LongKindTable long_kind_table(int long_cap) {
+    LongKindTable t;
+    t.n_dense = 0;
+    for (int k = 0; k < kLongKinds; ++k) t.dense[k] = long_cap == kLongRun ? (int8_t)t.n_dense++ : (int8_t)-1;
+    return t;
+}
+
 struct Key {
     const void *obs = nullptr, *rew = nullptr, *done = nullptr;
     int32_t ring = 0, f32 = 0, num_actions = 0, chains = 0, horizon = 0, coherent = 0, split = 0, pairs = 0;
@@ -41,8 +63,9 @@
     int32_t slots = 0;
     const void *stamps = nullptr; uint32_t dbg_skip = 0;
     const void *world = nullptr;
+    int32_t long_cap = 0;
     bool operator==(const Key &o) const {
-        return stamps == o.stamps && dbg_skip == o.dbg_skip && world == o.world && obs == o.obs && rew == o.rew && done == o.done && ring == o.ring && f32 == o.f32 && num_actions == o.num_actions &&
+        return long_cap == o.long_cap && stamps == o.stamps && dbg_skip == o.dbg_skip && world == o.world && obs == o.obs && rew == o.rew && done == o.done && ring == o.ring && f32 == o.f32 && num_actions == o.num_actions &&
                chains == o.chains && horizon == o.horizon && coherent == o.coherent && split == o.split && pairs == o.pairs && actions == o.actions && order == o.order &&
                action_ring == o.action_ring && slots == o.slots;
     }
@@ -63,6 +86,7 @@
     int n_steps;
     int fast_profile, pair_profile;
     int aql_coherent, aql_split, aql_alternate, aql_pairs, aql_run;
+    int long_profile;
 };
 struct Form {
     int coherent;
@@ -70,7 +94,10 @@
     bool split;
     int pairs;
     int run_cap;
-};
+    int long_cap;
+    int key_long;
+};
+constexpr int kLongCallSteps = 256;
 inline Form choose_form(const FormIn &in) {
     Form f;
     const bool coherent = in.aql_coherent != 0 && !in.f32 && !in.order && in.fast_profile > 0 && in.per_launch <= 4096;
@@ -82,6 +109,8 @@
     if (in.aql_run >= 1 && in.aql_run < cap) cap = in.aql_run;
     f.pairs = cap >= 2 ? cap : 0;
     f.run_cap = f.split ? f.pairs : 0;
+    f.key_long = (f.key_split && f.pairs == kMaxRun && in.long_profile >= kLongRun && (in.aql_run < 1 || in.aql_run >= kLongRun)) ? kLongRun : 0;
+    f.long_cap = (f.key_long && f.split && in.n_steps >= kLongCallSteps) ? kLongRun : 0;
     return f;
 }
 
@@ -100,7 +129,7 @@
     } else { p.actions = nullptr; p.order = nullptr; p.num_actions_random = c.num_actions; }
 }
 
-constexpr int kMids = kMaxRun - 1;
+constexpr int kMids = kMaxRun - 1, kLongMids = kLongRun - 1;
 struct SplitBuffers {
     uint8_t *world_buf[2] = {};
     uint32_t *agents_buf[2] = {};
@@ -108,7 +137,45 @@
     uint8_t *snap_grid[2] = {};
     uint8_t *mid_world[kMids][2] = {}, *mid_snap[kMids][2] = {};
     uint32_t *mid_agents[kMids][2] = {}, *mid_list[kMids][2] = {};
-};
+    uint8_t *long_world[kLongMids - kMids][2] = {}, *long_snap[kLongMids - kMids][2] = {};
+    uint32_t *long_agents[kLongMids - kMids][2] = {}, *long_list[kLongMids - kMids][2] = {};
+    struct MidSet { uint8_t *world; uint32_t *agents; uint32_t *list; uint8_t *snap; };
+    MidSet mid_set(int k, int o) const {
+        if (k < kMids) return MidSet{mid_world[k][o], mid_agents[k][o], mid_list[k][o], mid_snap[k][o]};
+        return MidSet{long_world[k - kMids][o], long_agents[k - kMids][o], long_list[k - kMids][o], long_snap[k - kMids][o]};
+    }
+};
+
+template <int kMax, class Q>
+inline void fill_run(const ChainRings &cur, const Key &key, const SplitBuffers &A, int o, int n, int rd, int i, int r, int mode, Params &p, Q &q) {
+    auto ring_slot = [&](int d) { return ((r + d) % key.ring + key.ring) % key.ring; };
+    auto slot_obs = [&](int sl) { return cur.obs ? cur.obs + (size_t)sl * cur.ob : nullptr; };
+    p.mode = mode;
+    p.obs = nullptr;
+    p.snap_mode = (n == 0 ? 4 : 1) | (rd > 0 ? 2 : 0);
+    p.world_out = A.world_buf[1 - o]; p.agents_out = A.agents_buf[1 - o];
+    p.beam_list = A.beam_list[o]; p.snap = A.snap_grid[o];
+    p.beam_list_in = A.beam_list[1 - o]; p.snap_in = A.snap_grid[1 - o];
+    q.n_pass = n; q.n_render = rd;
+    for (int k = 0; k < n; ++k) {
+        const int rk = ring_slot(k);
+        PassRec &rec = q.pass[k];
+        const SplitBuffers::MidSet m = k + 1 < n ? A.mid_set(k, o) : SplitBuffers::MidSet{p.world_out, p.agents_out, p.beam_list, p.snap};
+        rec = PassRec{m.world, m.agents, m.list, m.snap, nullptr, nullptr, nullptr};
+        rec.rew = cur.rew ? cur.rew + (size_t)rk * cur.en : nullptr;
+        rec.done = cur.done ? cur.done + (size_t)rk * cur.en : nullptr;
+        rec.actions = cur.actions ? cur.actions + ((size_t)(i + k) % (size_t)cur.action_ring) * cur.en : nullptr;
+    }
+    const int first = n == 0 ? 0 : -rd;
+    for (int t = kMax - rd; t < kMax - 1; ++t) {
+        if (t < 0) continue;
+        const int j = t - (kMax - rd);
+        const SplitBuffers::MidSet m = A.mid_set(j, 1 - o);
+        q.mid_in[t] = MidIn{m.world, m.agents, m.list, m.snap};
+        q.obs_b0[t] = slot_obs(ring_slot(first + j));
+    }
+    p.obs_b = slot_obs(ring_slot(first + rd - 1));
+}
 
 inline void fill_block(const Params &base, const ChainRings &cur, const Key &key, const SplitBuffers &A, int kind, int i, Params &p, PairParams &q) {
     const int r = i % key.ring;
@@ -128,34 +195,7 @@
     cursor_actions(cur, p, (size_t)i);
     p.rew = cur.rew ? cur.rew + (size_t)r * cur.en : nullptr; p.done = cur.done ? cur.done + (size_t)r * cur.en : nullptr;
     if (pair_kind) {
-        constexpr int kMax = kMaxRun;
-        const int n = (kb - kRun) / (kMax + 1), rd = (kb - kRun) % (kMax + 1);
-        auto ring_slot = [&](int d) { return ((r + d) % key.ring + key.ring) % key.ring; };
-        auto slot_obs = [&](int sl) { return cur.obs ? cur.obs + (size_t)sl * cur.ob : nullptr; };
-        p.mode = kModeStepPair;
-        p.obs = nullptr;
-        p.snap_mode = (n == 0 ? 4 : 1) | (rd > 0 ? 2 : 0);
-        p.world_out = A.world_buf[1 - o]; p.agents_out = A.agents_buf[1 - o];
-        p.beam_list = A.beam_list[o]; p.snap = A.snap_grid[o];
-        p.beam_list_in = A.beam_list[1 - o]; p.snap_in = A.snap_grid[1 - o];
-        q.n_pass = n; q.n_render = rd;
-        for (int k = 0; k < n; ++k) {
-            const int rk = ring_slot(k);
-            PassRec &rec = q.pass[k];
-            if (k + 1 < n) rec = PassRec{A.mid_world[k][o], A.mid_agents[k][o], A.mid_list[k][o], A.mid_snap[k][o], nullptr, nullptr, nullptr};
-            else rec = PassRec{p.world_out, p.agents_out, p.beam_list, p.snap, nullptr, nullptr, nullptr};
-            rec.rew = cur.rew ? cur.rew + (size_t)rk * cur.en : nullptr;
-            rec.done = cur.done ? cur.done + (size_t)rk * cur.en : nullptr;
-            rec.actions = cur.actions ? cur.actions + ((size_t)(i + k) % (size_t)cur.action_ring) * cur.en : nullptr;
-        }
-        const int first = n == 0 ? 0 : -rd;
-        for (int t = kMax - rd; t < kMax - 1; ++t) {
-            if (t < 0) continue;
-            const int j = t - (kMax - rd);
-            q.mid_in[t] = MidIn{A.mid_world[j][1 - o], A.mid_agents[j][1 - o], A.mid_list[j][1 - o], A.mid_snap[j][1 - o]};
-            q.obs_b0[t] = slot_obs(ring_slot(first + j));
-        }
-        p.obs_b = slot_obs(ring_slot(first + rd - 1));
+        fill_run<kMaxRun>(cur, key, A, o, (kb - kRun) / (kMaxRun + 1), (kb - kRun) % (kMaxRun + 1), i, r, kModeStepPair, p, q);
     } else if (kb >= kA) {
         uint8_t *obs_r = p.obs;
         uint8_t *obs_prev = cur.obs ? cur.obs + (size_t)((r + key.ring - 1) % key.ring) * cur.ob : nullptr;
@@ -171,6 +211,18 @@
     }
 }
 
+inline void fill_long_block(const Params &base, const ChainRings &cur, const Key &key, const SplitBuffers &A, int kind, int i, Params &p, LongParams &q) {
+    const int r = i % key.ring, o = long_kind_o(kind);
+    p = base;
+    q = LongParams{};
+    p.world = A.world_buf[o]; p.agents = A.agents_buf[o];
+    p.coherent = key.coherent ? ((key.coherent == 2 && o == 1) ? 2u : 1u) : 0u;
+    p.rotate = 1;
+    cursor_actions(cur, p, (size_t)i);
+    p.rew = cur.rew ? cur.rew + (size_t)r * cur.en : nullptr; p.done = cur.done ? cur.done + (size_t)r * cur.en : nullptr;
+    fill_run<kLongRun>(cur, key, A, o, long_kind_n(kind), long_kind_rendered(kind), i, r, kModeStepLong, p, q);
+}
+
 inline int start_orientation(int key_split, bool state_in_second_buffer) { return key_split && state_in_second_buffer ? 1 : 0; }
 
 struct Packet {
@@ -186,9 +238,10 @@
 };
 class Schedule {
 public:
-    Schedule(int n_steps, int step0, int reset_every, int ring, int slots, bool split, int run_cap, bool coherent, bool obs_wb, int acq, int rel, int o)
+    Schedule(int n_steps, int step0, int reset_every, int ring, int slots, bool split, int run_cap, bool coherent, bool obs_wb, int acq, int rel, int o,
+             int long_cap = 0)
         : n_steps_(n_steps), step0_(step0), reset_every_(reset_every), ring_(ring), slots_(slots), split_(split), run_cap_(split ? run_cap : 0),
-          coherent_(coherent), obs_wb_(obs_wb), kAcq(acq), kRel(rel), o_(o) {}
+          long_cap_((split && run_cap == kMaxRun && long_cap == kLongRun) ? kLongRun : 0), coherent_(coherent), obs_wb_(obs_wb), kAcq(acq), kRel(rel), o_(o) {}
     __attribute__((always_inline)) bool next(Group &g) {
         const int k = k_;
         if (k >= n_steps_) return false;
@@ -197,12 +250,12 @@
         const bool reset = reset_every_ > 0 && (step0_ + k) % reset_every_ == 0;
         int avail = n_steps_ - k;
         if (reset_every_ > 0) { const int to_reset = reset_every_ - (step0_ + k) % reset_every_; if (to_reset < avail) avail = to_reset; }
-        const int n = (run_cap_ > 2 && avail >= run_cap_) ? run_cap_ : (run_cap_ >= 2 && avail >= 2) ? 2 : 1;
+        const int n = (long_cap_ > 0 && avail >= long_cap_) ? long_cap_ : (run_cap_ > 2 && avail >= run_cap_) ? run_cap_ : (run_cap_ >= 2 && avail >= 2) ? 2 : 1;
         const bool last = k + n >= n_steps_;
         const int acq = k == 0 ? 1 : kAcq;
         Packet *pk = g.packet;
         if (reset) {
-            if (split_ && pending_) *pk++ = Packet{i_prev_, o_ * KO + render_only(pending_), kAcq, kRel};
+            if (split_ && pending_) *pk++ = Packet{i_prev_, render_kind(o_, pending_), kAcq, kRel};
             *pk++ = Packet{i, o_ * KO + (split_ ? kRn : kR), acq, kRel};
         }
         const int rendered = reset ? 0 : pending_;
@@ -212,8 +265,9 @@
         bool round = false;
         for (int j = 0; j < n; ++j) round = round || (step0_ + k + j) % ring_ == 0;
         const int rel = (obs_wb_ && round) ? 1 : kRel;
-        *pk++ = Packet{i, o_ * KO + base, reset ? kAcq : acq, rel};
-        if (split_ && last) *pk++ = Packet{i, (1 - o_) * KO + render_only(n), kAcq, kRel};
+        const int kind = (n == kLongRun || rendered == kLongRun) ? long_kind(o_, n, rendered) : o_ * KO + base;
+        *pk++ = Packet{i, kind, reset ? kAcq : acq, rel};
+        if (split_ && last) *pk++ = Packet{i, render_kind(1 - o_, n), kAcq, kRel};
         g.n_packets = (int)(pk - g.packet);
         g.step = k; g.steps = n; g.reset = reset;
 #if SSD_RING_EVERY > 1
@@ -230,10 +284,11 @@
     int orientation() const { return o_; }
     int longest() const { return longest_; }
     static constexpr int render_only(int rendered) { return rendered == 1 ? (int)kB : run_kind(0, rendered); }
+    static constexpr int render_kind(int o, int rendered) { return rendered == kLongRun ? long_kind(o, 0, rendered) : o * kKindsPerO + render_only(rendered); }
 
 private:
     int n_steps_, step0_, reset_every_, ring_, slots_;
-    bool split_; int run_cap_; bool coherent_, obs_wb_;
+    bool split_; int run_cap_, long_cap_; bool coherent_, obs_wb_;
     int kAcq, kRel;
     int o_;
     int k_ = 0;
diff --git a/sequential_social_dilemma_games_amd/engine.py b/sequential_social_dilemma_games_amd/engine.py
--- a/sequential_social_dilemma_games_amd/engine.py
+++ b/sequential_social_dilemma_games_amd/engine.py
@@ -479,7 +479,7 @@
                 "pairs": bool(m & _capi.SSD_PATH_PAIRS),
                 "fused": bool(m & _capi.SSD_PATH_FUSED), "sync": bool(m & _capi.SSD_PATH_SYNC), "forked": bool(m & _capi.SSD_PATH_FORKED),
                 "queue_dropped": bool(m & _capi.SSD_PATH_QUEUE_DROPPED), "chains": (m >> 8) & 15, "pool": (m >> 12) & 7,
-                "agent_match": ("none", "pci", "uuid", "ordinal")[(m >> 16) & 3], "run": (m >> _capi.SSD_PATH_RUN_SHIFT) & 7}
+                "agent_match": ("none", "pci", "uuid", "ordinal")[(m >> 16) & 3], "run": (m >> _capi.SSD_PATH_RUN_SHIFT) & 15}
 
     def observe(self, rotate=True, obs=None):
         torch, dev = self._torch()
```

After: 5.554 billion, median of 6. 1.04x the previous value.
